# cryscan/bevy-hikari

Hardware: AMD Instinct MI355X
Metric: Mray/s (Cornell 1080p 2-bounce, whole job) + frame ms (higher is better)
Workload: dtype f32

## Files before the change

### bevy-hikari_amd/_ffi.py

```python
import ctypes as C
import os

HERE = os.path.dirname(os.path.abspath(__file__))
LIB_PATH = os.environ.get("HIKARI_HIP_LIB", os.path.join(HERE, "libhikari_hip.so"))

HK_OK = 0
HK_E_INVALID, HK_E_NO_DEVICE, HK_E_HIP, HK_E_NOT_READY, HK_E_NOMEM, HK_E_UNSUPPORTED = -1, -2, -3, -4, -5, -6

BUF_POSITION, BUF_NORMAL, BUF_DEPTH_GRADIENT, BUF_INSTANCE_MATERIAL, BUF_VELOCITY_UV, BUF_ALBEDO = range(6)
BUF_VARIANCE0, BUF_RENDER0, BUF_RESERVOIR0 = 6, 9, 12
BUF_DENOISE_INTERNAL0, BUF_DENOISE_INTERNAL_VARIANCE, BUF_DENOISE_RENDER0, BUF_TONE_MAPPED = 22, 26, 27, 30
(BUF_PREVIOUS_POSITION, BUF_PREVIOUS_VELOCITY_UV, BUF_PREVIOUS_TONE_MAPPED, BUF_UPSCALE_OUTPUT, BUF_TAA_OUTPUT, BUF_PREVIOUS_TAA_OUTPUT,
 BUF_UPSCALE_SHARPENED) = range(31, 38)
BUF_PARKED_TO0, BUF_PARKED_RECORD0, BUF_COUNT = 38, 41, 44
HISTORY_AUTO = 0xFFFF
(PASS_PREPASS, PASS_FULL_SCREEN_ALBEDO, PASS_DIRECT_LIT, PASS_DIRECT_EMISSIVE, PASS_INDIRECT, PASS_EMISSIVE_SPATIAL_REUSE,
 PASS_INDIRECT_SPATIAL_REUSE, PASS_DEMODULATION, PASS_DENOISE_L0, PASS_DENOISE_L1, PASS_DENOISE_L2, PASS_DENOISE_L3,
 PASS_TONE_MAPPING, PASS_SMAA_TU4X, PASS_SMAA_TU4X_EXTRAPOLATE, PASS_TAA_JASMINE, PASS_FSR_EASU, PASS_FSR_RCAS, PASS_COUNT) = range(19)
PASS_NAMES = ["prepass", "full_screen_albedo", "direct_lit", "direct_emissive", "indirect_lit_ambient", "emissive_spatial_reuse",
              "indirect_spatial_reuse", "demodulation", "denoise_l0", "denoise_l1", "denoise_l2", "denoise_l3", "tone_mapping",
              "smaa_tu4x", "smaa_tu4x_extrapolate", "taa_jasmine", "fsr_easu", "fsr_rcas"]
STAGE_TEMPORAL, STAGE_SPATIAL, STAGE_POST_PROCESS, STAGE_ANTIALIAS, STAGE_UPSCALE, STAGE_COUNT = range(6)
DEFAULT_CTX_FLAGS = int(os.environ.get("HIKARI_HIP_DEFAULT_CTX_FLAGS", "0"))
CTX_COUNT_RAYS, CTX_TIME_PASSES, CTX_PLAIN_DIVISION, CTX_SINGLE_STREAM, CTX_DETERMINISTIC_SCATTER, CTX_EXACT_TRAVERSAL = 1, 2, 4, 8, 16, 32
TREE_SAH, TREE_LBVH = 0, 1
CTX_WAVEFRONT, CTX_FUSED_INDIRECT = 64, 128
CTX_NO_WIDE_WALK = 256
CTX_COUNT_WALKS = 512
CTX_RACING_SCATTER = 1024
DEBUG_OPT_SPATIAL_WINDOW, DEBUG_OPT_FRAME_PIPELINE, DEBUG_OPT_WF_TIMELINE, DEBUG_OPT_FLAT_WALK, DEBUG_OPT_FLAT_ORDERINGS, DEBUG_OPT_TRACE_UPDATE = 0, 1, 2, 3, 4, 5
DEBUG_OPT_MAIN_PRIORITY, DEBUG_OPT_PREPASS_PIPELINE, DEBUG_OPT_MESH_REBUILD_ONE_WORKGROUP = 9, 10, 11
DEBUG_OPT_LOAD_DEVICE_LIMIT = 12
TIMING_TRACE_STAGES = 18
TRAVERSAL_WIDE = 0x100
FRAME_EXTERNAL_GBUFFER, FRAME_ANTIALIAS, FRAME_BALANCE_BANDS, FRAME_GATHER, FRAME_TIME_BAND = 1, 2, 4, 8, 16
TOPOLOGY_TRIANGLE_LIST, TOPOLOGY_TRIANGLE_STRIP = 0, 1
TAA_JASMINE, TAA_NONE = 0, 1
UPSCALE_FSR1, UPSCALE_SMAA_TU4X = 0, 1
NO_TEXTURE = 0xFFFFFFFF
ADDRESS_CLAMP_TO_EDGE, ADDRESS_REPEAT, ADDRESS_MIRROR_REPEAT = 0, 1, 2
TIMING_SLOTS = 24
FORMAT_RGBA16F, FORMAT_RGBA32F, FORMAT_RGBA8_UNORM_SRGB, FORMAT_BGRA8_UNORM_SRGB = range(4)
PRESENT_HDR, PRESENT_CLEAR = 1, 2
RAYS_CLOSEST, RAYS_ANY, RAYS_ATTRIBUTES, RAYS_STACKLESS = 0, 1, 2, 4
RAY_MISS, RAY_HIT, RAY_INVALID = 0, 1, 2
NO_INSTANCE = 0xFFFFFFFF

f32, u32, u64 = C.c_float, C.c_uint32, C.c_uint64


class HkVertex(C.Structure):
    _fields_ = [("position", f32 * 3), ("u", f32), ("normal", f32 * 3), ("v", f32)]


class HkPrimitiveVertex(C.Structure):
    _fields_ = [("position", f32 * 3), ("index", u32)]


class HkPrimitive(C.Structure):
    _fields_ = [("vertices", HkPrimitiveVertex * 3)]


class HkNode(C.Structure):
    _fields_ = [("min", f32 * 3), ("entry_index", u32), ("max", f32 * 3), ("exit_index", u32)]


class HkMeshIndex(C.Structure):
    _fields_ = [("vertex", u32), ("primitive", u32), ("node_offset", u32), ("node_count", u32)]


class HkInstance(C.Structure):
    _fields_ = [("min", f32 * 3), ("material", u32), ("max", f32 * 3), ("node_index", u32), ("model", f32 * 16),
                ("inverse_transpose_model", f32 * 16), ("mesh", HkMeshIndex)]


class HkMaterial(C.Structure):
    _fields_ = [("base_color", f32 * 4), ("base_color_texture", u32), ("_pad0", u32 * 3), ("emissive", f32 * 4),
                ("emissive_texture", u32), ("perceptual_roughness", f32), ("metallic", f32), ("metallic_roughness_texture", u32),
                ("reflectance", f32), ("normal_map_texture", u32), ("occlusion_texture", u32), ("_pad1", u32)]


class HkAliasEntry(C.Structure):
    _fields_ = [("prob", f32), ("index", u32)]


class HkEmissive(C.Structure):
    _fields_ = [("emissive", f32 * 4), ("position", f32 * 3), ("radius", f32), ("instance", u32), ("_pad0", u32),
                ("alias_table", u32 * 2), ("surface_area", f32), ("node_index", u32), ("_pad1", u32 * 2)]


class HkFrame(C.Structure):
    _fields_ = [("kernel", (f32 * 4) * 3), ("halton", (f32 * 4) * 8), ("clear_color", f32 * 4), ("number", u32),
                ("direct_validate_interval", u32), ("emissive_validate_interval", u32), ("indirect_bounces", u32),
                ("temporal_reuse", u32), ("emissive_spatial_reuse", u32), ("indirect_spatial_reuse", u32),
                ("max_temporal_reuse_count", u32), ("max_spatial_reuse_count", u32), ("max_reservoir_lifetime", f32),
                ("solar_angle", f32), ("max_indirect_luminance", f32), ("upscale_ratio", f32), ("_pad", u32 * 3)]


class HkView(C.Structure):
    _fields_ = [("view_proj", f32 * 16), ("inverse_view_proj", f32 * 16), ("view", f32 * 16), ("inverse_view", f32 * 16),
                ("projection", f32 * 16), ("inverse_projection", f32 * 16), ("world_position", f32 * 3), ("_pad0", f32),
                ("viewport", f32 * 4)]


class HkPreviousView(C.Structure):
    _fields_ = [("view_proj", f32 * 16), ("inverse_view_proj", f32 * 16)]


class HkLights(C.Structure):
    _fields_ = [("directional_color", f32 * 4), ("direction_to_light", f32 * 3), ("n_directional_lights", u32),
                ("ambient_color", f32 * 4)]


class HkSettings(C.Structure):
    _fields_ = [("direct_validate_interval", u32), ("emissive_validate_interval", u32), ("max_temporal_reuse_count", u32),
# ... 19 lines not shown
class HkRayHit(C.Structure):
    _fields_ = [("distance", f32), ("instance", u32), ("primitive", u32), ("material", u32), ("barycentric", f32 * 2), ("uv", f32 * 2),
                ("normal", f32 * 3), ("status", u32)]


class HkHaloOp(C.Structure):
    _fields_ = [("buffer", u32), ("peer", u32), ("row_begin", u32), ("row_end", u32), ("row_bytes", u64)]


class HkTransfer(C.Structure):
    _fields_ = [("buffer", u32), ("peer", u32), ("is_recv", u32), ("_pad", u32), ("offset", C.c_uint64), ("bytes", C.c_uint64)]


class HkMovedBox(C.Structure):
    _fields_ = [("min", f32 * 3), ("_pad0", f32), ("max", f32 * 3), ("_pad1", f32), ("previous_from_current", f32 * 16)]


class HkStats(C.Structure):
    _fields_ = [("rays_primary", u64), ("rays_tlas", u64), ("rays_blas", u64), ("frames", u64),
                ("pass_ms_total", C.c_double * TIMING_SLOTS), ("pass_launches", u64 * TIMING_SLOTS), ("last_frame_ms", f32),
                ("_pad", u32), ("scene_mesh_builds", u64), ("scene_instance_builds", u64),
                ("scene_async_instance_uploads", u64), ("scene_device_refits", u64), ("scene_device_tree_builds", u64),
                ("walk_node_steps", u64), ("walk_triangle_tests", u64), ("walk_instance_entries", u64), ("walk_closest_hits", u64), ("walk_top_node_steps", u64),
                ("wide_stack_lost", u64)]


assert C.sizeof(HkVertex) == 32 and C.sizeof(HkPrimitive) == 48 and C.sizeof(HkNode) == 32 and C.sizeof(HkInstance) == 176
assert C.sizeof(HkMaterial) == 80 and C.sizeof(HkEmissive) == 64 and C.sizeof(HkFrame) == 256 and C.sizeof(HkView) == 416
assert C.sizeof(HkPreviousView) == 128 and C.sizeof(HkAliasEntry) == 8
assert C.sizeof(HkRay) == 32 and C.sizeof(HkRayHit) == 48


class HikariError(RuntimeError):
    def __init__(self, code, fn, message):
        super().__init__(f"{fn} failed with code {code}: {message}")
        self.code = code


P = C.POINTER
_vp = C.c_void_p

_SIGNATURES = {
    "create": [C.c_int, u32, P(_vp)],
    "upload_meshes": [_vp, P(HkVertex), u32, P(HkPrimitive), u32, P(HkNode), u32],
    "upload_materials": [_vp, P(HkMaterial), u32],
    "upload_instances": [_vp, P(HkInstance), u32, P(HkNode), u32, P(HkEmissive), u32, P(HkNode), u32, P(HkAliasEntry), u32],
    "upload_previous_transforms": [_vp, P(f32), u32],
    "upload_noise": [_vp, _vp, C.c_size_t],
    "upload_textures": [_vp, P(HkImageDesc), u32],
    "resize": [_vp, u32, u32, f32],
    "set_view_options": [_vp, u32, u32, f32],
    "frame_begin": [_vp, P(HkFrame), P(HkView), P(HkPreviousView), P(HkLights)],
    "pass_run": [_vp, u32, u32, u32, u32],
    "frame_stage": [_vp, u32, P(HkSettings), u32],
    "frame_render": [_vp, P(HkFrame), P(HkView), P(HkPreviousView), P(HkLights), P(HkSettings), u32],
    "frame_wait": [_vp],
    "set_band": [_vp, u32, u32],
    "set_history_rows": [_vp, u32],
    "history_rows": [_vp, P(u32)],
    "scene_bounds": [_vp, P(f32), P(f32)],
    "set_band_bounds": [_vp, P(u32), u32],
    "row_costs": [_vp, P(u32), u32],
    "buffer_info": [_vp, u32, P(u32), P(u32), P(u32)],
    "read_buffer": [_vp, u32, _vp, C.c_size_t],
    "write_buffer": [_vp, u32, _vp, C.c_size_t],
    "device_ptr": [_vp, u32, P(_vp), P(C.c_size_t)],
    "get_stats": [_vp, P(HkStats)],
    "reset_stats": [_vp],
}
_DEBUG = {
    "debug_math": [_vp, u32, P(f32), P(f32), P(f32), C.c_size_t],
    "debug_read_trees": [_vp, P(HkNode), u32, P(HkNode), u32],
    "debug_read_mesh_nodes": [_vp, P(HkNode), u32, P(u32), P(u32)],
    "debug_last_load": [_vp, P(u32)],
    "debug_last_load_times": [_vp, P(C.c_double)],
    "debug_read_emitters": [_vp, P(f32), u32, P(u32), P(f32), u32, P(u32)],
    "debug_read_mesh_geometry": [_vp, P(HkMeshIndex), P(f32), P(f32), u32, P(f32), u32, P(f32), P(u32), P(u32)],
    "debug_comm_loopback": [_vp, u32, u32, u32, u32, u32],
    "debug_read_wf_timeline": [_vp, P(C.c_uint64), u32],
    "debug_set_option": [_vp, u32, C.c_int64],
    "debug_comm_lanes": [_vp, P(u32)],
    "debug_multi_serial": [C.c_int],
    "debug_spatial_windowed_launches": [_vp, P(C.c_uint64)],
    "debug_main_stream_priority": [_vp, P(u32)],
    "measure_hbm": [_vp, C.c_size_t, u32, P(C.c_double), P(C.c_double)],
    "measure_valu": [_vp, u32, P(C.c_double)],
    "measure_gather": [_vp, C.c_size_t, u32, u32, u32, u32, P(C.c_double), P(C.c_double)],
}
_PRODUCT_ONLY = {
    "device_count": [P(C.c_int)],
    "settings_default": [P(HkSettings)],
    "frame_from_settings": [P(HkSettings), u32, P(HkFrame)],
    "scaled_size": [u32, u32, f32, P(u32), P(u32)],
    "scene_builder_create": [P(_vp)],
    "scene_builder_add_mesh": [_vp, P(f32), P(f32), P(f32), u32, P(u32), u32, u32, P(u32)],
    "scene_builder_add_mesh_deferred": [_vp, P(f32), P(f32), P(f32), u32, P(u32), u32, u32, P(u32)],
    "scene_builder_pending_mesh_trees": [_vp, P(u32)],
    "scene_builder_build_pending_mesh_trees": [_vp],
    "scene_builder_add_material": [_vp, P(HkMaterial), P(u32)],
    "scene_builder_add_instance": [_vp, u32, u32, P(f32), P(u32)],
    "scene_builder_finish": [_vp],
    "scene_builder_finish_instances": [_vp],
    "scene_builder_remove_instance": [_vp, u32],
    "scene_builder_set_instance_material": [_vp, u32, u32],
    "scene_builder_set_instance_transform": [_vp, u32, P(f32)],
    "scene_builder_previous_transforms": [_vp, P(P(f32)), P(u32)],
    "scene_builder_vertices": [_vp, P(P(HkVertex)), P(u32)],
    "scene_builder_primitives": [_vp, P(P(HkPrimitive)), P(u32)],
    "scene_builder_asset_nodes": [_vp, P(P(HkNode)), P(u32)],
    "scene_builder_materials": [_vp, P(P(HkMaterial)), P(u32)],
    "scene_builder_instances": [_vp, P(P(HkInstance)), P(u32)],
    "scene_builder_instance_nodes": [_vp, P(P(HkNode)), P(u32)],
    "scene_builder_emissives": [_vp, P(P(HkEmissive)), P(u32)],
    "scene_builder_emissive_nodes": [_vp, P(P(HkNode)), P(u32)],
    "scene_builder_alias_table": [_vp, P(P(HkAliasEntry)), P(u32)],
    "scene_builder_set_mesh_vertices": [_vp, u32, P(f32), P(f32)],
    "scene_builder_rebuild_mesh_tree": [_vp, u32],
    "scene_builder_mesh_index": [_vp, u32, P(HkMeshIndex)],
    "upload_scene": [_vp, _vp],
    "upload_scene_instances": [_vp, _vp],
    "load_scene": [_vp, _vp, u32],
    "refit_scene_instances": [_vp, _vp, P(u32)],
    "rebuild_scene_trees": [_vp, u32],
    "update_scene_instances": [_vp, _vp, u32],
    "update_mesh_vertices": [_vp, P(HkMeshIndex), u32, P(f32), P(f32)],
    "set_mesh_skin": [_vp, P(HkMeshIndex), u32, P(f32), P(f32), P(C.c_uint16), P(f32)],
    "skin_mesh": [_vp, P(HkMeshIndex), P(f32), u32],
    "rebuild_mesh_tree": [_vp, P(HkMeshIndex), u32],
    "present": [_vp, P(HkSettings), u32, P(HkPresentTarget), u32, u32],
    "cast_rays": [_vp, P(HkRay), u32, u32, P(HkRayHit)],
    "cast_rays_device": [_vp, _vp, u32, u32, _vp],
    "band_rows": [u32, u32, u32, P(u32), P(u32)],
    "balanced_band_bounds": [P(u32), u32, u32, u32, u32, u32, f32, P(u32)],
    "balance_bands": [_vp, u32, P(u32), u32],
    "rebalanced_band_bounds": [P(u32), P(f32), u32, u32, P(f32), u32, u32, f32, P(u32)],
    "band_migration_plan": [u32, u32, f32, P(u32), P(u32), u32, u32, u32, P(HkSettings), P(HkHaloOp), P(u32)],
    "band_migration_schedule": [u32, u32, f32, P(u32), P(u32), u32, u32, u32, P(HkSettings), P(HkTransfer), P(u32)],
    "migrate_bands": [_vp, P(u32), u32, u32, P(HkSettings)],
    "band_time_ms": [_vp, P(f32)],
    "multi_migrate_bands": [_vp, P(u32), u32, u32, P(HkSettings)],
    "band_gather_schedule": [u32, u32, f32, u32, P(u32), u32, u32, u32, u32, P(HkTransfer), P(u32)],
    "comm_gather": [_vp, u32, u32],
    "multi_gather": [_vp, u32, u32],
    "get_band_bounds": [_vp, P(u32), u32],
    "get_band": [_vp, P(u32), P(u32)],
    "band_plan_bounds": [u32, u32, f32, P(u32), u32, u32, u32, u32, P(HkSettings), P(HkHaloOp), P(u32)],
    "band_schedule_bounds": [u32, u32, f32, P(u32), u32, u32, u32, u32, P(HkSettings), P(HkTransfer), P(u32)],
    "band_plan": [_vp, u32, P(HkSettings), P(HkHaloOp), P(u32)],
    "band_plan_for": [u32, u32, f32, u32, u32, u32, u32, P(HkSettings), P(HkHaloOp), P(u32)],
    "stream": [_vp, P(_vp)],
    "set_stream": [_vp, _vp],
    "set_timing_mask": [_vp, u32],
    "indirect_schedule": [_vp, P(u32)],
    "traversal_mode": [_vp, P(u32), P(u32)],
    "bvh_rethread": [P(HkNode), u32, u32, P(HkNode)],
    "band_schedule": [u32, u32, f32, u32, u32, u32, u32, P(HkSettings), P(HkTransfer), P(u32)],
    "comm_unique_id": [P(C.c_uint8)],
    "comm_available": [_vp],
    "comm_init": [_vp, u32, u32, P(C.c_uint8)],
    "comm_destroy": [_vp],
    "comm_set_history_rows": [_vp, u32],
    "history_rows_bound": [P(HkView), P(HkPreviousView), u32, P(f32), P(f32), P(HkMovedBox), u32, P(u32)],
    "comm_exchange": [_vp, u32, P(HkSettings)],
    "multi_create": [u32, P(C.c_int), u32, P(_vp)],
    "multi_context": [_vp, u32, P(_vp)],
    "multi_upload_scene": [_vp, _vp],
# ... 82 lines not shown
```

### bevy-hikari_amd/csrc/context.hip

```cpp
#include "hk_context.hpp"

using namespace hk;
using namespace hkd;

namespace hk {

void buffer_dims(const hk_ctx* c, uint32_t b, int* w, int* h) {
  if (buffer_is_full_size(b)) { *w = c->W; *h = c->H; return; }
  if (buffer_is_upscaled(b) && c->upscale_kind == HK_UPSCALE_SMAA_TU4X) { *w = c->UW; *h = c->UH; return; }
  if (b == HK_BUF_UPSCALE_OUTPUT) { *w = c->W; *h = c->H; return; }
  *w = c->RW;
  *h = c->RH;
}
size_t buffer_logical_bytes(const hk_ctx* c, uint32_t b) {
  int w, h;
  buffer_dims(c, b, &w, &h);
  return (size_t)w * h * buffer_bpp(b);
}

bool certify_uv_division(int size) {
  const float b = (float)size, c = 1.0f / b;
  for (int k = -64; k < size + 64; ++k) {
    const float x = (float)k + 0.5f, want = x / b, q = x * c, got = fmaf(fmaf(-q, b, x), c, q);
    if (memcmp(&want, &got, 4) != 0) return false;
  }
  return true;
}

#ifndef HK_PRE_BANDS
#define HK_PRE_BANDS 1
#endif
#ifndef HK_PRE_STREAM_HIGH
#define HK_PRE_STREAM_HIGH 0
#endif
#ifndef HK_MAIN_HIGH_PRIORITY_PIXELS
#define HK_MAIN_HIGH_PRIORITY_PIXELS ((size_t)6 << 20)
#endif
int pick_main_stream(hk_ctx* c, bool forced) {
  if (!c->own_stream || c->post_forked) return HK_OK;
  if (!forced && c->main_priority_decided) return HK_OK;
  const size_t px = (size_t)c->RW * (size_t)c->RH / (size_t)(c->band_count > 0 ? c->band_count : 1);
  if (px == 0) return HK_OK;
  c->main_priority_decided = true;
  const bool high = c->main_priority < 0 ? px <= HK_MAIN_HIGH_PRIORITY_PIXELS : c->main_priority != 0;
  if (high == c->own_stream_high) return HK_OK;
  const bool in_use = c->stream == c->own_stream;
  { const int rc = sync_all(c); if (rc) return rc; }
  HK_HIP(hipStreamSynchronize(c->own_stream));
  int least = 0, greatest = 0;
  hipStream_t fresh = nullptr;
  if (hipDeviceGetStreamPriorityRange(&least, &greatest) != hipSuccess || least == greatest ||
      hipStreamCreateWithPriority(&fresh, hipStreamNonBlocking, high ? greatest : least) != hipSuccess || !fresh) {
    (void)hipGetLastError();
    return HK_OK;
  }
  (void)hipStreamDestroy(c->own_stream);
  c->own_stream = fresh;
  c->own_stream_high = high;
  if (in_use) c->stream = fresh;
  if (high && c->side_stream && c->post_stream && !c->pre_stream) {
    if (hipStreamCreateWithPriority(&c->pre_stream, hipStreamNonBlocking, (HK_PRE_STREAM_HIGH || c->band_count > 1) ? greatest : least) != hipSuccess || hipEventCreateWithFlags(&c->pre_done, hipEventDisableTiming) != hipSuccess ||
        hipEventCreateWithFlags(&c->pre_scene_mark, hipEventDisableTiming) != hipSuccess) {
      (void)hipGetLastError();
      if (c->pre_stream) (void)hipStreamDestroy(c->pre_stream);
      c->pre_stream = nullptr;
    }
  }
  return HK_OK;
}
#ifndef HK_PREPASS_PIPELINE_RULE
#ifndef HK_PREPASS_PIPELINE_LDS_BANDS
#define HK_PREPASS_PIPELINE_LDS_BANDS 0
#endif
#define HK_PREPASS_PIPELINE_RULE                                                                                                     \
  ((size_t)c->scene.blob_f4 * 16 > HK_LDS_SCENE_BYTES ? (size_t)c->RW * (size_t)c->RH / (size_t)(c->band_count > 0 ? c->band_count : 1) <= ((size_t)3 << 20) \
                                                        : (HK_PREPASS_PIPELINE_LDS_BANDS && c->band_count > 1 && (size_t)c->RW * (size_t)c->RH / (size_t)c->band_count <= ((size_t)3 << 18)))
#endif
int free_screen(hk_ctx* c) {
  for (int k = 0; k < 3; ++k) {
    if (c->det_winner[k]) (void)hipFree(c->det_winner[k]);
    c->det_winner[k] = nullptr;
    c->det_lite_clean[k] = false;
  }
  for (uint32_t b = 0; b < HK_BUF_COUNT; ++b) {
    if (c->buf[b]) (void)hipFree(c->buf[b]);
    c->buf[b] = nullptr;
    c->buf_bytes[b] = 0;
  }
  for (int k = 0; k < 10; ++k) {
    if (c->tile_meta[k]) (void)hipFree(c->tile_meta[k]);
    c->tile_meta[k] = nullptr;
    c->tile_meta_zero[k] = false;
  }
  if (c->wf_mem) (void)hipFree(c->wf_mem);
  c->wf_mem = nullptr;
  if (c->wf.timeline) (void)hipFree(c->wf.timeline);
  c->wf = hkd::WfBuffers{};
  if (c->depth_plane) (void)hipFree(c->depth_plane);
  if (c->prev_depth_plane) (void)hipFree(c->prev_depth_plane);
  c->prev_depth_plane = nullptr;
  if (c->dn_g) (void)hipFree(c->dn_g);
  c->depth_plane = nullptr;
  c->dn_g = nullptr;
  for (void** q : {&c->albedo_twin, &c->depth_gradient_twin, &c->dn_g_twin, &c->normal_twin, &c->instance_material_twin, &c->render_twin[0], &c->render_twin[1], &c->render_twin[2], &c->variance_twin[0],
                   &c->variance_twin[1], &c->variance_twin[2]}) {
    if (*q) (void)hipFree(*q);
    *q = nullptr;
  }
  c->post_pending[0] = c->post_pending[1] = false;
  for (int k = 0; k < 2; ++k) {
    for (int l = 0; l < 4; ++l) {
      if (c->dn_extra[k][l]) (void)hipFree(c->dn_extra[k][l]);
      c->dn_extra[k][l] = nullptr;
    }
    if (c->dn_extra_var[k]) (void)hipFree(c->dn_extra_var[k]);
    c->dn_extra_var[k] = nullptr;
  }
  return HK_OK;
}

hipEvent_t get_event(hk_ctx* c) {
  if (!c->event_pool.empty()) {
    hipEvent_t e = c->event_pool.back();
    c->event_pool.pop_back();
    return e;
  }
  hipEvent_t e = nullptr;
  (void)hipEventCreate(&e);
  return e;
}

void drain_timers(hk_ctx* c) {
  for (TimedLaunch& t : c->pending) {
    float ms = 0.0f;
    if (hipEventElapsedTime(&ms, t.start, t.stop) == hipSuccess) {
      c->slot_ms[t.slot] += (double)ms;
      c->slot_launches[t.slot] += 1;
    }
    c->event_pool.push_back(t.start);
    c->event_pool.push_back(t.stop);
  }
  c->pending.clear();
  if (c->frame_timed) {
    float ms = 0.0f;
    if (hipEventElapsedTime(&ms, c->frame_start, c->frame_stop) == hipSuccess) c->last_frame_ms = ms;
    c->frame_timed = false;
  }
}

struct ScopedTimer {
  hk_ctx* c;
  bool on;
  TimedLaunch t{};
  bool attached;
  ScopedTimer(hk_ctx* ctx, uint32_t slot, bool attach = false) : c(ctx), on((ctx->timing_mask >> slot) & 1u), attached(attach) {
    if (on) {
      t.slot = slot;
      t.start = get_event(c);
      t.stop = get_event(c);
      if (!attached) (void)hipEventRecord(t.start, c->stream);
    }
  }
  ~ScopedTimer() {
    if (on) {
      if (!attached) (void)hipEventRecord(t.stop, c->stream);
      c->pending.push_back(t);
    }
  }
};

DFrame make_dframe(const hk_ctx* c) {
  DFrame f;
  memset(&f, 0, sizeof(f));
  const HkFrame& h = c->frame;
  for (int col = 0; col < 3; ++col)
    for (int row = 0; row < 3; ++row) f.kernel[col * 3 + row] = h.kernel[col][row];
  f.number = h.number;
  f.direct_validate_interval = h.direct_validate_interval;
  f.emissive_validate_interval = h.emissive_validate_interval;
  f.indirect_bounces = h.indirect_bounces;
  f.temporal_reuse = h.temporal_reuse;
  f.max_temporal_reuse_count = h.max_temporal_reuse_count;
  f.max_spatial_reuse_count = h.max_spatial_reuse_count;
  f.max_reservoir_lifetime = h.max_reservoir_lifetime;
  f.solar_angle = h.solar_angle;
  f.max_indirect_luminance = h.max_indirect_luminance;
  f.upscale_ratio = h.upscale_ratio;
  f.random_float_number = (float)hash_u32(h.number) / 4294967295.0f;
  f.number_golden = (float)h.number * 1.618033989f;
  f.cam_x = c->view.world_position[0]; f.cam_y = c->view.world_position[1]; f.cam_z = c->view.world_position[2];
  f.ortho_x = c->view.view_proj[2]; f.ortho_y = c->view.view_proj[6]; f.ortho_z = c->view.view_proj[10];
  f.is_ortho = c->view.projection[15] == 1.0f ? 1u : 0u;
  f.sun_r = c->lights.directional_color[0]; f.sun_g = c->lights.directional_color[1]; f.sun_b = c->lights.directional_color[2];
  f.sun_dx = c->lights.direction_to_light[0]; f.sun_dy = c->lights.direction_to_light[1]; f.sun_dz = c->lights.direction_to_light[2];
  f.amb_r = c->lights.ambient_color[0]; f.amb_g = c->lights.ambient_color[1]; f.amb_b = c->lights.ambient_color[2];
  f.clear_r = h.clear_color[0]; f.clear_g = h.clear_color[1]; f.clear_b = h.clear_color[2]; f.clear_a = h.clear_color[3];
  f.dw = c->W; f.dh = c->H; f.rw = c->RW; f.rh = c->RH;
  f.inv_dw = 1.0f / (float)c->W; f.inv_dh = 1.0f / (float)c->H; f.inv_rw = 1.0f / (float)c->RW; f.inv_rh = 1.0f / (float)c->RH;
  f.rcp_rw = 1.0 / (double)c->RW; f.rcp_rh = 1.0 / (double)c->RH;
  f.uv_fast = c->uv_fast ? 1u : 0u;
  return f;
}
GBuffer make_gbuffer(const hk_ctx* c) {
  GBuffer g;
  g.position = (float4*)c->buf[HK_BUF_POSITION];
  g.normal = (uint32_t*)c->buf[HK_BUF_NORMAL];
  g.depth_gradient = (float2*)c->buf[HK_BUF_DEPTH_GRADIENT];
  g.instance_material = (float2*)c->buf[HK_BUF_INSTANCE_MATERIAL];
  g.velocity_uv = (float4*)c->buf[HK_BUF_VELOCITY_UV];
  g.depth = c->depth_plane;
  g.dn_g = (float4*)c->dn_g;
  g.albedo_out = nullptr;
  return g;
}
bool parks_across_bands(const hk_ctx* c) { return c->band_count > 1 && c->history_now > 0; }
bool scatter_lite(const hk_ctx* c, int channel) {
  if (c->band_count > 1 || (c->flags & HK_CTX_RACING_SCATTER)) return false;
  if (c->flags & HK_CTX_DETERMINISTIC_SCATTER) return true;
  return channel == 2 ? c->frame.indirect_spatial_reuse != 0u : c->frame.emissive_spatial_reuse != 0u;
}
int ensure_parked(hk_ctx* c, uint32_t channels) {
  const size_t nr = (size_t)c->RW * c->RH;
  for (int k = 0; k < 3; ++k) {
    if (!((channels >> k) & 1u) || c->det_winner[k]) continue;
    int* winner = nullptr;
    void* plane[2] = {nullptr, nullptr};
    size_t plane_bytes[2] = {0, 0};
    hipError_t e = hipMalloc((void**)&winner, nr * sizeof(int));
    for (int j = 0; j < 2 && e == hipSuccess; ++j) {
      const uint32_t b = (j == 0 ? (uint32_t)HK_BUF_PARKED_TO0 : (uint32_t)HK_BUF_PARKED_RECORD0) + (uint32_t)k;
      plane_bytes[j] = nr * buffer_bpp(b);
      e = hipMalloc(&plane[j], plane_bytes[j]);
      if (e == hipSuccess) e = hipMemset(plane[j], j == 0 ? 0xFF : 0, plane_bytes[j]);
    }
    if (e == hipSuccess) e = hipDeviceSynchronize();
    if (e != hipSuccess) {
      if (winner) (void)hipFree(winner);
      for (void* q : plane)
        if (q) (void)hipFree(q);
      set_error("allocating the parked-store planes failed: %s", hipGetErrorString(e));
      return HK_E_HIP;
    }
    c->det_winner[k] = winner;
    for (int j = 0; j < 2; ++j) {
      const uint32_t b = (j == 0 ? (uint32_t)HK_BUF_PARKED_TO0 : (uint32_t)HK_BUF_PARKED_RECORD0) + (uint32_t)k;
      c->buf[b] = plane[j];
      c->buf_bytes[b] = plane_bytes[j];
    }
  }
  return HK_OK;
}
void scene_bounds(const hk_ctx* c, float mn[3], float mx[3]) {
  for (int k = 0; k < 3; ++k) { mn[k] = INFINITY; mx[k] = -INFINITY; }
  for (const HkInstance& in : c->instances)
    for (int k = 0; k < 3; ++k) {
      mn[k] = std::min(mn[k], in.min[k]);
      mx[k] = std::max(mx[k], in.max[k]);
    }
}
int derive_history_rows(const hk_ctx* c, uint32_t* rows) {
  *rows = 0;
  if (c->instances.empty()) return HK_OK;
  std::vector<HkMovedBox> moved;
  const size_t ni = c->instances.size();
  if (c->prev_models.size() == 16 * ni)
    for (size_t i = 0; i < ni; ++i) {
      const HkInstance& in = c->instances[i];
      const float* pm = &c->prev_models[16 * i];
      if (memcmp(pm, in.model, 64) == 0) continue;
      HkMovedBox b{};
      memcpy(b.min, in.min, 12);
      memcpy(b.max, in.max, 12);
      for (int col = 0; col < 4; ++col)
        for (int row = 0; row < 4; ++row) {
          double s = 0.0;
          for (int k = 0; k < 4; ++k) s += (double)pm[4 * k + row] * (double)in.inverse_transpose_model[4 * k + col];
          b.previous_from_current[4 * col + row] = (float)s;
        }
      moved.push_back(b);
    }
  if (moved.empty() && memcmp(c->view.view_proj, c->pview.view_proj, 64) == 0) return HK_OK;
  float mn[3], mx[3];
  scene_bounds(c, mn, mx);
  return hk_history_rows_bound(&c->view, &c->pview, (uint32_t)c->RH, mn, mx, moved.empty() ? nullptr : moved.data(), (uint32_t)moved.size(), rows);
}
LightTargets make_light_targets(const hk_ctx* c, int channel) {
  static const int T[3] = {0, 2, 6}, S[3] = {4, 4, 8};
  const uint32_t cur = c->frame.number % 2u, prev = 1u - cur;
  LightTargets t;
  t.previous = (const PackedReservoir*)c->buf[HK_BUF_RESERVOIR0 + cur + T[channel]];
  t.current = (PackedReservoir*)c->buf[HK_BUF_RESERVOIR0 + prev + T[channel]];
  t.previous_spatial = (PackedReservoir*)c->buf[HK_BUF_RESERVOIR0 + cur + S[channel]];
  t.spatial = (PackedReservoir*)c->buf[HK_BUF_RESERVOIR0 + prev + S[channel]];
  t.variance = (float*)c->buf[HK_BUF_VARIANCE0 + channel];
  t.render = (uint2*)c->buf[HK_BUF_RENDER0 + channel];
  const bool parked = c->det_winner[channel] && (scatter_lite(c, channel) || parks_across_bands(c));
  t.det_lite = parked && !parks_across_bands(c) ? 1 : 0;
// ... 2 lines not shown
  t.det_pending = parked ? (PackedReservoir*)c->buf[HK_BUF_PARKED_RECORD0 + channel] : nullptr;
  t.m_current = t.m_spatial = t.m_previous_spatial = nullptr;
  t.serial = 0;
  t.tiles_x = c->tiles_x;
  t.rw = c->RW;
  return t;
}
int attach_tile_meta(hk_ctx* c, LightTargets& t, int channel, bool spatial_pass, int y0, int y1) {
  if (!c->tile_meta[0]) return HK_OK;
  static const int T[3] = {0, 2, 6}, S[3] = {4, 4, 8};
  const int cur = (int)(c->frame.number % 2u), prev = 1 - cur;
  const int k_current = prev + T[channel], k_spatial = prev + S[channel], k_previous_spatial = cur + S[channel];
  const bool maintain = c->band_count == 1 && (y0 % 8) == 0 && ((y1 % 8) == 0 || y1 == c->RH);
  const size_t mb = (size_t)c->tiles_x * c->tiles_y * sizeof(TileMeta);
  const int written[3] = {spatial_pass ? -1 : k_current, k_spatial, spatial_pass ? -1 : k_previous_spatial};
  for (int k : written) {
    if (k < 0) continue;
    if (maintain) {
      c->tile_meta_zero[k] = false;
    } else if (!c->tile_meta_zero[k]) {
      HK_HIP(hipMemsetAsync(c->tile_meta[k], 0, mb, c->stream));
      c->tile_meta_zero[k] = true;
    }
  }
  if (!maintain) return HK_OK;
  t.m_current = c->tile_meta[k_current];
  t.m_spatial = c->tile_meta[k_spatial];
  t.m_previous_spatial = c->tile_meta[k_previous_spatial];
  t.serial = ++c->elide_serial;
  return HK_OK;
}

int ready(hk_ctx* c) {
  HK_REQUIRE(c, HK_E_INVALID, "ctx is NULL");
  HK_REQUIRE(c->W > 0, HK_E_NOT_READY, "hk_resize has not been called");
  HK_REQUIRE(c->have_frame, HK_E_NOT_READY, "hk_frame_begin has not been called");
  HK_REQUIRE(c->have_noise, HK_E_NOT_READY, "noise textures not uploaded");
  HK_HIP(hipSetDevice(c->device));
  const int rc = finalize_scene(c);
  return rc ? rc : flush_deform(c);
}

struct Jitter { float x, y; };
Jitter prepass_jitter(const hk_ctx* c) {
  Jitter j{0.0f, 0.0f};
  if (c->taa == HK_TAA_NONE) return j;
  const uint32_t n = c->frame.number;
  const uint32_t index = (c->upscale_kind == HK_UPSCALE_SMAA_TU4X) ? ((n >> 1u) & 15u) : (n & 15u);
  const float* h = c->frame.halton[index >> 1u];
  const float hx = (index & 1u) == 0u ? h[0] : h[2], hy = (index & 1u) == 0u ? h[1] : h[3];
  j.x = 2.0f * hx * (1.0f / c->view.viewport[2]);
  j.y = -(2.0f * hy * (1.0f / c->view.viewport[3]));
  return j;
}

void full_rows_for(const hk_ctx* c, int ry0, int ry1, int* fy0, int* fy1) {
  if (c->RH == c->H) {
    *fy0 = ry0;
    *fy1 = ry1;
    return;
  }
  *fy0 = std::max(0, (int)floorf((float)ry0 * (float)c->H / (float)c->RH) - 1);
  *fy1 = std::min(c->H, (int)ceilf((float)ry1 * (float)c->H / (float)c->RH) + 1);
}

void* dn_internal(hk_ctx* c, uint32_t nch, uint32_t ch, int level) {
  return ch + 1 == nch ? c->buf[HK_BUF_DENOISE_INTERNAL0 + level] : c->dn_extra[ch][level];
}
float* dn_variance(hk_ctx* c, uint32_t nch, uint32_t ch) {
  return ch + 1 == nch ? (float*)c->buf[HK_BUF_DENOISE_INTERNAL_VARIANCE] : c->dn_extra_var[ch];
}
int run_demodulation_fused(hk_ctx* c, uint32_t nch, int y0, int y1) {
  if (y1 <= y0) return HK_OK;
  const DFrame fr = make_dframe(c);
  ScopedTimer timer(c, HK_PASS_DEMODULATION);
  DemodTargets d{};
  d.albedo = (const uint2*)c->buf[HK_BUF_ALBEDO];
  for (uint32_t ch = 0; ch < nch; ++ch) {
    d.variance[ch] = (const float*)c->buf[HK_BUF_VARIANCE0 + ch];
    d.render[ch] = (const uint2*)c->buf[HK_BUF_RENDER0 + ch];
    d.output[ch] = (uint2*)dn_internal(c, nch, ch, 0);
    d.internal_variance[ch] = dn_variance(c, nch, ch);
  }
  launch_demodulation(c->stream, (int)nch, fr, d, y0, y1);
  HK_HIP(hipGetLastError());
  return HK_OK;
}
int run_denoise_fused(hk_ctx* c, uint32_t nch, int level, int y0, int y1, bool with_tone_mapping = false) {
  if (y1 <= y0) return HK_OK;
  const DFrame fr = make_dframe(c);
  ScopedTimer timer(c, HK_PASS_DENOISE_L0 + (uint32_t)level);
  DenoiseTargets d{};
  d.albedo = (const uint2*)c->buf[HK_BUF_ALBEDO];
  d.dn_g = (const float4*)c->dn_g;
  d.depth = c->depth_plane;
  d.depth_gradient = (const float2*)c->buf[HK_BUF_DEPTH_GRADIENT];
  for (uint32_t ch = 0; ch < nch; ++ch) {
    d.input[ch] = (const uint2*)dn_internal(c, nch, ch, level);
    d.output[ch] = level == 3 ? (uint2*)c->buf[HK_BUF_DENOISE_RENDER0 + ch] : (uint2*)dn_internal(c, nch, ch, level + 1);
    d.internal_variance[ch] = dn_variance(c, nch, ch);
  }
  if (with_tone_mapping && level == 3 && nch == (c->frame.indirect_bounces != 0u ? 3u : 2u)) {
    d.tone_mapped = (uint2*)c->buf[HK_BUF_TONE_MAPPED];
    memcpy(d.clear_color, c->frame.clear_color, sizeof(d.clear_color));
  }
  launch_denoise(c->stream, level, (int)nch, 0, fr, d, y0, y1);
  HK_HIP(hipGetLastError());
  return HK_OK;
}

bool use_wavefront(const hk_ctx* c) {
  if (c->frame.indirect_bounces < 2u || c->frame.indirect_bounces > 60u || (c->flags & HK_CTX_COUNT_RAYS)) return false;
  if (c->flags & HK_CTX_FUSED_INDIRECT) return false;
  if (c->flags & HK_CTX_WAVEFRONT) return true;
  return (size_t)c->scene.blob_f4 * 16 > HK_LDS_SCENE_BYTES;
}
static bool wide_allowed(const hk_ctx* c) {
  return !(c->flags & HK_CTX_NO_WIDE_WALK) && c->threaded && !c->scene.flat_mode && (size_t)c->scene.blob_f4 * 16 > HK_LDS_SCENE_BYTES;
}
bool use_wide(const hk_ctx* c) { return wide_allowed(c); }
int ensure_wide(hk_ctx* c, bool with_spill) {
  const size_t tlas_slots = c->instance_nodes.size(), blas_slots = c->asset_nodes.size();
  if (tlas_slots == 0 || blas_slots == 0) return HK_OK;
  if (tlas_slots > c->wide_tlas_slots) {
    if (c->wide_tlas) { HK_HIP(hipStreamSynchronize(c->stream)); (void)hipFree(c->wide_tlas); c->wide_tlas = nullptr; }
    HK_HIP(hipMalloc((void**)&c->wide_tlas, (tlas_slots + tlas_slots / 2 + 16) * 128));
    c->wide_tlas_slots = tlas_slots + tlas_slots / 2 + 16;
    c->wide_tlas_dirty = true;
  }
  if (blas_slots > c->wide_blas_slots) {
    if (c->wide_blas) { HK_HIP(hipStreamSynchronize(c->stream)); (void)hipFree(c->wide_blas); c->wide_blas = nullptr; }
    HK_HIP(hipMalloc((void**)&c->wide_blas, blas_slots * 128));
    c->wide_blas_slots = blas_slots;
    c->wide_blas_dirty = true;
  }
  const size_t n_inst = c->instances.size(), n_prim = c->primitives.size();
  if (n_inst > c->wide_rank_instances) {
    if (c->wide_tlas_rank) { HK_HIP(hipStreamSynchronize(c->stream)); (void)hipFree(c->wide_tlas_rank); c->wide_tlas_rank = nullptr; }
    HK_HIP(hipMalloc((void**)&c->wide_tlas_rank, (n_inst + n_inst / 2 + 16) * sizeof(uint32_t)));
    HK_HIP(hipMemsetAsync(c->wide_tlas_rank, 0xFF, (n_inst + n_inst / 2 + 16) * sizeof(uint32_t), c->stream));
    c->wide_rank_instances = n_inst + n_inst / 2 + 16;
    c->wide_tlas_dirty = true;
  }
  if (n_prim > c->wide_rank_primitives) {
    if (c->wide_blas_rank) { HK_HIP(hipStreamSynchronize(c->stream)); (void)hipFree(c->wide_blas_rank); c->wide_blas_rank = nullptr; }
    HK_HIP(hipMalloc((void**)&c->wide_blas_rank, std::max<size_t>(n_prim, 1) * sizeof(uint32_t)));
    HK_HIP(hipMemsetAsync(c->wide_blas_rank, 0xFF, std::max<size_t>(n_prim, 1) * sizeof(uint32_t), c->stream));
    c->wide_rank_primitives = n_prim;
    c->wide_blas_dirty = true;
  }
  if (!c->compute_units) {
    hipDeviceProp_t prop;
    HK_HIP(hipGetDeviceProperties(&prop, c->device));
    c->compute_units = prop.multiProcessorCount;
  }
  const size_t lanes = with_spill ? wide_trace_lanes(c->compute_units) : 0;
  if (lanes > c->wide_spill_lanes) {
    if (c->wide_spill) { HK_HIP(hipStreamSynchronize(c->stream)); (void)hipFree(c->wide_spill); c->wide_spill = nullptr; }
    HK_HIP(hipMalloc((void**)&c->wide_spill, lanes * wide_spill_entries() * sizeof(uint32_t)));
    c->wide_spill_lanes = lanes;
  }
  if (c->wide_blas_dirty || c->wide_mesh_check) {
    if (c->wide_blas_dirty) c->wide_meshes.clear();
    std::vector<std::pair<uint32_t, uint32_t>> meshes;
    std::vector<std::pair<std::pair<uint32_t, uint32_t>, uint32_t>> first_primitive;
    for (const HkInstance& in : c->instances) {
      meshes.emplace_back(in.mesh.node_offset, in.mesh.node_count);
      first_primitive.emplace_back(std::make_pair(in.mesh.node_offset, in.mesh.node_count), in.mesh.primitive);
    }
    std::sort(meshes.begin(), meshes.end());
    meshes.erase(std::unique(meshes.begin(), meshes.end()), meshes.end());
    std::sort(first_primitive.begin(), first_primitive.end());
    first_primitive.erase(std::unique(first_primitive.begin(), first_primitive.end()), first_primitive.end());
    for (size_t k = 0; k + 1 < first_primitive.size(); ++k)
      HK_REQUIRE(first_primitive[k].first != first_primitive[k + 1].first, HK_E_INVALID, "two instances share the mesh nodes [%u, +%u) but not the mesh primitives (%u / %u)",
                 first_primitive[k].first.first, first_primitive[k].first.second, first_primitive[k].second, first_primitive[k + 1].second);
    for (const auto& m : meshes) {
      if (std::binary_search(c->wide_meshes.begin(), c->wide_meshes.end(), m)) continue;
      HK_REQUIRE((size_t)m.first + m.second <= blas_slots, HK_E_INVALID, "an instance's mesh nodes lie outside the uploaded mesh nodes");
      const uint32_t prim0 = std::lower_bound(first_primitive.begin(), first_primitive.end(), std::make_pair(m, 0u))->second;
      HK_REQUIRE((size_t)prim0 + (m.second + 2u) / 3u <= n_prim, HK_E_INVALID, "an instance's mesh primitives lie outside the uploaded primitives");
      launch_build_wide(c->stream, c->scene.nodes + 2u * ((size_t)c->scene.blas_base + m.first), m.second, c->wide_blas + 8u * (size_t)m.first, c->wide_blas_rank + prim0);
    }
    HK_HIP(hipGetLastError());
    std::vector<std::pair<uint32_t, uint32_t>> all;
    std::set_union(c->wide_meshes.begin(), c->wide_meshes.end(), meshes.begin(), meshes.end(), std::back_inserter(all));
    c->wide_meshes.swap(all);
    c->wide_blas_dirty = c->wide_mesh_check = false;
// ... 51 lines not shown
  if ((tl_twin || count_twin) && !w.timeline) HK_HIP(hipMalloc((void**)&w.timeline, 64 * 32 * sizeof(unsigned long long)));
  w.timeline_mode = count_twin ? 2u : (tl_twin ? 1u : 0u);
  return HK_OK;
}

int join_side(hk_ctx* c) {
  if (!c->forked) return HK_OK;
  HK_HIP(hipEventRecord(c->join_event, c->side_stream));
  HK_HIP(hipStreamWaitEvent(c->stream, c->join_event, 0));
  c->forked = false;
  c->side_state[0] = c->side_state[1] = 0;
  return HK_OK;
}
int join_post(hk_ctx* c) {
  for (int k = 0; k < 2; ++k)
    if (c->post_pending[k]) {
      HK_HIP(hipStreamWaitEvent(c->stream, c->post_done[k], 0));
      c->post_pending[k] = false;
    }
  return HK_OK;
}
int join_post_parity(hk_ctx* c, uint32_t parity) {
  if (!c->post_pending[parity & 1u]) return HK_OK;
  HK_HIP(hipStreamWaitEvent(c->stream, c->post_done[parity & 1u], 0));
  c->post_pending[parity & 1u] = false;
  return HK_OK;
}
int join_all(hk_ctx* c) {
  int rc = join_side(c);
  if (!rc) rc = join_post(c);
  if (!rc && c->comm) rc = comm_join(c, -1);
  return rc;
}
#define HK_FRAME_INTERNAL_LATE_JOIN 0x80000000u
int post_begin(hk_ctx* c, const HkSettings* st, bool* pipelined) {
  *pipelined = false;
  int rc;
  if (st->denoise && c->derived_dirty) {
    launch_derive_planes(c->stream, make_gbuffer(c), c->depth_plane, c->dn_g, c->W, 0, c->H);
    c->derived_dirty = false;
  }
  const uint32_t post_bits = (1u << HK_PASS_DEMODULATION) | (1u << HK_PASS_DENOISE_L0) | (1u << HK_PASS_DENOISE_L1) | (1u << HK_PASS_DENOISE_L2) | (1u << HK_PASS_DENOISE_L3);
  if (!(st->denoise && c->post_stream && c->frame_pipeline && !(c->timing_mask & post_bits) && c->albedo_twin && c->render_twin[0])) {
    if ((rc = join_side(c))) return rc;
    return join_post(c);
  }
  if (c->forked) {
    HK_HIP(hipEventRecord(c->side_done, c->side_stream));
    HK_HIP(hipStreamWaitEvent(c->post_stream, c->side_done, 0));
    for (int k = 0; k < 2; ++k)
      if (c->side_state[k] == 1) {
        c->side_state[k] = 2;
        c->side_cover[k] = (uint8_t)(c->mapped_parity & 1u);
      }
  }
  HK_HIP(hipEventRecord(c->post_fork, c->stream));
  HK_HIP(hipStreamWaitEvent(c->post_stream, c->post_fork, 0));
  c->post_saved_main = c->stream;
  c->stream = c->post_stream;
  *pipelined = true;
  return HK_OK;
}
int post_end(hk_ctx* c, bool pipelined) {
  c->post_forked = false;
  if (!pipelined) return HK_OK;
  const uint32_t parity = c->mapped_parity & 1u;
  const hipError_t e = hipEventRecord(c->post_done[parity], c->post_stream);
  c->stream = c->post_saved_main;
  HK_REQUIRE(e == hipSuccess, HK_E_HIP, "hipEventRecord failed: %s", hipGetErrorString(e));
  c->post_pending[parity] = true;
  return HK_OK;
}
int run_pass(hk_ctx* c, uint32_t pass, uint32_t arg, int y0, int y1);
int run_pass_on_side(hk_ctx* c, uint32_t pass, uint32_t arg, int y0, int y1) {
  hipStream_t main_stream = c->stream;
  c->stream = c->side_stream;
  const int rc = (y1 > y0) ? run_pass(c, pass, arg, y0, y1) : HK_OK;
  c->stream = main_stream;
  return rc;
}

int run_pass(hk_ctx* c, uint32_t pass, uint32_t arg, int y0, int y1) {
  const DFrame fr = make_dframe(c);
  const GBuffer g = make_gbuffer(c);
  unsigned long long* counters = (c->flags & HK_CTX_COUNT_RAYS) ? c->d_counters : nullptr;
  if (c->derived_dirty && pass != HK_PASS_PREPASS) {
    launch_derive_planes(c->stream, g, c->depth_plane, c->dn_g, c->W, 0, c->H);
    c->derived_dirty = false;
  }
  ScopedTimer timer(c, pass, pass == HK_PASS_INDIRECT || pass == HK_PASS_INDIRECT_SPATIAL_REUSE || pass == HK_PASS_EMISSIVE_SPATIAL_REUSE);
  switch (pass) {
    case HK_PASS_PREPASS: {
      Jitter j = prepass_jitter(c);
      hkd::WideTrees wide{};
      { const int rc_ = wide_for_fused(c, &wide); if (rc_) return rc_; }
      launch_prepass(c->stream, c->scene, fr, c->view.inverse_view_proj, c->view.view_proj, c->pview.view_proj, c->d_prev_models, j.x, j.y, g, y0, y1, counters, &wide);
      break;
    }
    case HK_PASS_FULL_SCREEN_ALBEDO: launch_albedo(c->stream, c->scene, fr, g, c->buf[HK_BUF_ALBEDO], y0, y1); break;
    case HK_PASS_DIRECT_LIT:
    case HK_PASS_DIRECT_EMISSIVE:
    case HK_PASS_INDIRECT: {
      const int channel = pass == HK_PASS_DIRECT_LIT ? 0 : (pass == HK_PASS_DIRECT_EMISSIVE ? 1 : 2);
      const bool across = parks_across_bands(c);
      if (across || scatter_lite(c, channel)) { const int rc_ = ensure_parked(c, across ? 7u : 1u << channel); if (rc_) return rc_; }
      LightTargets t = make_light_targets(c, channel);
      { const int rc_ = attach_tile_meta(c, t, channel, false, y0, y1); if (rc_) return rc_; }
      const size_t px = (size_t)c->RW * c->RH;
      if (t.det_winner && t.det_lite) {
        if (!c->det_lite_clean[channel]) {
          HK_HIP(hipMemsetAsync(t.det_winner, 0xFF, px * sizeof(int), c->stream));
          HK_HIP(hipMemsetAsync(t.det_to, 0xFF, px * sizeof(int), c->stream));
          c->det_lite_clean[channel] = true;
        }
      } else {
        c->det_lite_clean[channel] = false;
        if (t.det_winner) {
          HK_HIP(hipMemsetAsync(t.det_winner, 0xFF, px * sizeof(int), c->stream));
          if (across) HK_HIP(hipMemsetAsync(t.det_to + (size_t)y0 * c->RW, 0xFF, (size_t)(y1 - y0) * c->RW * sizeof(int), c->stream));
          else HK_HIP(hipMemsetAsync(t.det_to, 0xFF, px * sizeof(int), c->stream));
        }
      }
      if (pass == HK_PASS_INDIRECT && use_wavefront(c)) {
        { const int rc_ = ensure_wavefront(c); if (rc_) return rc_; }
        hkd::WideTrees wide{};
        if (use_wide(c)) {
          { const int rc_ = ensure_wide(c, true); if (rc_) return rc_; }
          wide.tlas = c->wide_tlas;
          wide.blas = c->wide_blas;
          wide.tlas_rank = c->wide_tlas_rank;
          wide.blas_rank = c->wide_blas_rank;
          wide.tlas_count = c->scene.tlas_count;
          wide.spill = c->wide_spill;
          wide.lost = c->d_counters + 8;
        }
        std::vector<hipEvent_t> trace_events;
        if ((c->timing_mask >> HK_TIMING_TRACE_STAGES) & 1u)
          for (uint32_t k = 0; k < 2u * (c->frame.indirect_bounces + 1u); ++k) trace_events.push_back(get_event(c));
        launch_indirect_wavefront(c->stream, c->scene, fr, g, t, c->wf, y0, y1, c->compute_units, timer.on ? timer.t.start : nullptr,
                                  timer.on ? timer.t.stop : nullptr, &wide, trace_events.empty() ? nullptr : trace_events.data());
        for (size_t k = 0; k + 1 < trace_events.size(); k += 2) c->pending.push_back(TimedLaunch{HK_TIMING_TRACE_STAGES, trace_events[k], trace_events[k + 1]});
      } else if (pass == HK_PASS_INDIRECT)
        launch_indirect(c->stream, c->frame.indirect_bounces >= 2u, c->scene, fr, g, t, y0, y1, counters, timer.on ? timer.t.start : nullptr,
                        timer.on ? timer.t.stop : nullptr);
      else
        launch_direct(c->stream, pass == HK_PASS_DIRECT_EMISSIVE, c->scene, fr, g, t, y0, y1, counters);
      if (t.det_winner && t.det_lite) launch_resolve_scatter_lite(c->stream, t, fr, c->depth_plane, pass == HK_PASS_INDIRECT, y0, y1);
      else if (t.det_winner && !across) launch_resolve_scatter(c->stream, t, 0, (int)px, 0, 0);
      break;
    }
    case HK_PASS_EMISSIVE_SPATIAL_REUSE:
    case HK_PASS_INDIRECT_SPATIAL_REUSE: {
      const int channel = pass == HK_PASS_EMISSIVE_SPATIAL_REUSE ? 1 : 2;
      LightTargets t = make_light_targets(c, channel);
      { const int rc_ = attach_tile_meta(c, t, channel, true, y0, y1); if (rc_) return rc_; }
      if (launch_spatial(c->stream, channel == 1, c->scene, fr, g, t, y0, y1, c->spatial_window, timer.on ? timer.t.start : nullptr, timer.on ? timer.t.stop : nullptr))
        c->spatial_windowed_launches += 1;
      break;
    }
    case HK_PASS_DEMODULATION: {
      HK_REQUIRE(arg < 3, HK_E_INVALID, "channel out of range");
      DemodTargets d{};
      d.albedo = (const uint2*)c->buf[HK_BUF_ALBEDO];
      d.variance[0] = (const float*)c->buf[HK_BUF_VARIANCE0 + arg];
      d.render[0] = (const uint2*)c->buf[HK_BUF_RENDER0 + arg];
      d.output[0] = (uint2*)c->buf[HK_BUF_DENOISE_INTERNAL0];
      d.internal_variance[0] = (float*)c->buf[HK_BUF_DENOISE_INTERNAL_VARIANCE];
      launch_demodulation(c->stream, 1, fr, d, y0, y1);
      break;
    }
    case HK_PASS_DENOISE_L0: case HK_PASS_DENOISE_L1: case HK_PASS_DENOISE_L2: case HK_PASS_DENOISE_L3: {
      HK_REQUIRE(arg < 3, HK_E_INVALID, "channel out of range");
// ... 134 lines not shown
    if (!(flags & (HK_CTX_DETERMINISTIC_SCATTER | HK_CTX_COUNT_RAYS | HK_CTX_TIME_PASSES))) {
      if (hipStreamCreateWithFlags(&c->post_stream, hipStreamNonBlocking) != hipSuccess || hipEventCreateWithFlags(&c->post_fork, hipEventDisableTiming) != hipSuccess ||
          hipEventCreateWithFlags(&c->post_done[0], hipEventDisableTiming) != hipSuccess || hipEventCreateWithFlags(&c->post_done[1], hipEventDisableTiming) != hipSuccess) {
        set_error("cannot create the post-process stream");
        hk_destroy(c);
        return HK_E_HIP;
      }
    }
  }
  *out = c;
  return HK_OK;
}

void hk_destroy(hk_ctx* c) {
  if (!c) return;
  (void)hipSetDevice(c->device);
  (void)join_all(c);
  if (c->stream) (void)hipStreamSynchronize(c->stream);
  comm_release(c);
  drain_timers(c);
  for (hipEvent_t e : c->event_pool) (void)hipEventDestroy(e);
  for (hipEvent_t e : c->band_ev)
    if (e) (void)hipEventDestroy(e);
  if (c->frame_start) (void)hipEventDestroy(c->frame_start);
  if (c->frame_stop) (void)hipEventDestroy(c->frame_stop);
  free_screen(c);
  if (c->scene_mem) (void)hipFree(c->scene_mem);
  for (int k = 0; k < 2; ++k) {
    if (c->staging[k]) (void)hipHostFree(c->staging[k]);
    if (c->staging_done[k]) (void)hipEventDestroy(c->staging_done[k]);
  }
  if (c->query_staging) (void)hipHostFree(c->query_staging);
  if (c->query_device) (void)hipFree(c->query_device);
  free_refit(c);
  free_deform(c);
  for (void* q : {(void*)c->wide_tlas, (void*)c->wide_blas, (void*)c->wide_spill, (void*)c->wide_tlas_rank, (void*)c->wide_blas_rank})
    if (q) (void)hipFree(q);
  c->d_tex_data.release();
  c->d_noise.release();
  if (c->d_counters) (void)hipFree(c->d_counters);
  if (c->side_stream) (void)hipStreamDestroy(c->side_stream);
  if (c->post_stream) (void)hipStreamDestroy(c->post_stream);
  if (c->post_fork) (void)hipEventDestroy(c->post_fork);
  for (int k = 0; k < 2; ++k)
    if (c->post_done[k]) (void)hipEventDestroy(c->post_done[k]);
  if (c->fork_event) (void)hipEventDestroy(c->fork_event);
  if (c->join_event) (void)hipEventDestroy(c->join_event);
  if (c->side_done) (void)hipEventDestroy(c->side_done);
  if (c->pre_stream) { (void)hipStreamSynchronize(c->pre_stream); (void)hipStreamDestroy(c->pre_stream); }
  if (c->pre_done) (void)hipEventDestroy(c->pre_done);
  if (c->pre_scene_mark) (void)hipEventDestroy(c->pre_scene_mark);
  if (c->own_stream) (void)hipStreamDestroy(c->own_stream);
  delete c;
}
int hk_debug_read_wf_timeline(hk_ctx* c, unsigned long long* out, uint32_t n) {
  HK_REQUIRE(c && out && n == 64u * 32u, HK_E_INVALID, "bad argument");
  HK_REQUIRE(c->wf.timeline, HK_E_NOT_READY, "no timeline: set HK_WF_TIMELINE=1 (or create the context with HK_CTX_COUNT_WALKS) before the first frame of a scene beyond the LDS copy");
  HK_HIP(hipSetDevice(c->device));
  { const int rc = sync_all(c); if (rc) return rc; }
  HK_HIP(hipMemcpy(out, c->wf.timeline, n * sizeof(unsigned long long), hipMemcpyDeviceToHost));
  int khz = 0;
  HK_HIP(hipDeviceGetAttribute(&khz, hipDeviceAttributeWallClockRate, c->device));
  out[n - 1] = (unsigned long long)khz;
  return HK_OK;
}

int hk_debug_set_option(hk_ctx* c, uint32_t option, int64_t value) {
  HK_REQUIRE(c, HK_E_INVALID, "ctx is NULL");
  HK_HIP(hipSetDevice(c->device));
  { const int rc = sync_all(c); if (rc) return rc; }
  switch (option) {
    case HK_DEBUG_OPT_SPATIAL_WINDOW: c->spatial_window = value < 0 ? -1 : (value ? 1 : 0); break;
    case HK_DEBUG_OPT_FRAME_PIPELINE: c->frame_pipeline = value != 0; break;
    case HK_DEBUG_OPT_WF_TIMELINE:
      c->wf_timeline = value != 0;
      if (c->wf_mem) { (void)hipFree(c->wf_mem); c->wf_mem = nullptr; }
      break;
    case HK_DEBUG_OPT_FLAT_WALK: c->flat_walk = value != 0; c->dynamic_dirty = true; break;
    case HK_DEBUG_OPT_FLAT_ORDERINGS: c->flat_orderings = (int)std::max<int64_t>(0, std::min<int64_t>(8, value)); c->dynamic_dirty = true; break;
    case HK_DEBUG_OPT_TRACE_UPDATE: c->trace_update = value != 0; break;
    case HK_DEBUG_OPT_MESH_REBUILD_ONE_WORKGROUP: c->mesh_rebuild_one_workgroup = value != 0; break;
    case HK_DEBUG_OPT_LOAD_DEVICE_LIMIT: c->load_device_limit = value <= 0 ? HK_MESH_REBUILD_MAX_TRIANGLES : (uint32_t)std::min<int64_t>(value, HK_MESH_REBUILD_MAX_TRIANGLES); break;
    case HK_DEBUG_OPT_PREPASS_PIPELINE: c->prepass_pipeline = value < 0 ? -1 : (value ? 1 : 0); break;
    case HK_DEBUG_OPT_MAIN_PRIORITY: c->main_priority = value < 0 ? -1 : (value ? 1 : 0); return pick_main_stream(c, true);
    default: HK_REQUIRE(false, HK_E_INVALID, "unknown option %u", option);
  }
  return HK_OK;
}

int hk_debug_main_stream_priority(hk_ctx* c, uint32_t* out) {
  HK_REQUIRE(c && out, HK_E_INVALID, "bad argument");
  *out = (c->own_stream_high ? 1u : 0u) | (c->main_priority_decided ? 2u : 0u) | (c->pre_stream ? 4u : 0u) | ((uint32_t)std::min<uint64_t>(c->prepasses_pipelined, 0xFFFFFu) << 8);
  return HK_OK;
}

int hk_debug_spatial_windowed_launches(hk_ctx* c, uint64_t* out) {
  HK_REQUIRE(c && out, HK_E_INVALID, "bad argument");
  *out = c->spatial_windowed_launches;
  return HK_OK;
}

static int resize_resources(hk_ctx* c, uint32_t width, uint32_t height, float upscale_ratio);

int hk_resize(hk_ctx* c, uint32_t width, uint32_t height, float upscale_ratio) {
  HK_REQUIRE(c && width && height && width <= 16384u && height <= 16384u, HK_E_INVALID, "bad size %u x %u (1..16384)", width, height);
  const int rc = resize_resources(c, width, height, upscale_ratio);
  if (rc) {
    free_screen(c);
    c->W = c->H = c->RW = c->RH = c->UW = c->UH = 0;
  }
  return rc;
}

static int resize_resources(hk_ctx* c, uint32_t width, uint32_t height, float upscale_ratio) {
  HK_HIP(hipSetDevice(c->device));
  { const int rc_ = sync_all(c); if (rc_) return rc_; }
  free_screen(c);
  if (!c->band_bounds.empty()) {
    c->band_bounds.clear();
    c->bounds_generation += 1;
  }
  uint32_t rw, rh;
  int rc = hk_scaled_size(width, height, upscale_ratio, &rw, &rh);
  if (rc) return rc;
  c->W = (int)width; c->H = (int)height; c->RW = (int)rw; c->RH = (int)rh;
  c->ratio = upscale_ratio < 1.0f ? 1.0f : (upscale_ratio > 2.0f ? 2.0f : upscale_ratio);
  {
    const float scale2 = (1.0f / c->ratio) * 2.0f;
    c->UW = (int)ceilf((float)width * scale2);
    c->UH = (int)ceilf((float)height * scale2);
    c->mapped_parity = 0;
    c->pre_chain_ok = false;
  }
  for (uint32_t b = 0; b < HK_BUF_PARKED_TO0; ++b) {
    size_t n = buffer_is_full_size(b) ? (size_t)c->W * c->H : (buffer_is_upscaled(b) ? (size_t)c->UW * c->UH : (size_t)c->RW * c->RH);
    size_t bytes = n * buffer_bpp(b);
    HK_HIP(hipMalloc(&c->buf[b], bytes));
    HK_HIP(hipMemset(c->buf[b], 0, bytes));
    c->buf_bytes[b] = bytes;
  }
  const size_t nf = (size_t)c->W * c->H, nr = (size_t)c->RW * c->RH;
  {
    c->tiles_x = (c->RW + 7) / 8;
    c->tiles_y = (c->RH + 7) / 8;
    const size_t mb = (size_t)c->tiles_x * c->tiles_y * sizeof(TileMeta);
    for (int k = 0; k < 10; ++k) {
      HK_HIP(hipMalloc((void**)&c->tile_meta[k], mb));
      HK_HIP(hipMemset(c->tile_meta[k], 0, mb));
      c->tile_meta_zero[k] = true;
    }
  }
  HK_HIP(hipMalloc((void**)&c->depth_plane, nf * 4));
  HK_HIP(hipMemset(c->depth_plane, 0, nf * 4));
  HK_HIP(hipMalloc((void**)&c->prev_depth_plane, nf * 4));
  HK_HIP(hipMemset(c->prev_depth_plane, 0, nf * 4));
  HK_HIP(hipMalloc(&c->dn_g, nf * 16));
  HK_HIP(hipMemset(c->dn_g, 0, nf * 16));
  if (c->post_stream) {
    HK_HIP(hipMalloc(&c->albedo_twin, c->buf_bytes[HK_BUF_ALBEDO]));
    HK_HIP(hipMemset(c->albedo_twin, 0, c->buf_bytes[HK_BUF_ALBEDO]));
    HK_HIP(hipMalloc(&c->depth_gradient_twin, c->buf_bytes[HK_BUF_DEPTH_GRADIENT]));
    HK_HIP(hipMemset(c->depth_gradient_twin, 0, c->buf_bytes[HK_BUF_DEPTH_GRADIENT]));
    HK_HIP(hipMalloc(&c->dn_g_twin, nf * 16));
    HK_HIP(hipMemset(c->dn_g_twin, 0, nf * 16));
    HK_HIP(hipMalloc(&c->normal_twin, c->buf_bytes[HK_BUF_NORMAL]));
    HK_HIP(hipMemset(c->normal_twin, 0, c->buf_bytes[HK_BUF_NORMAL]));
    HK_HIP(hipMalloc(&c->instance_material_twin, c->buf_bytes[HK_BUF_INSTANCE_MATERIAL]));
    HK_HIP(hipMemset(c->instance_material_twin, 0, c->buf_bytes[HK_BUF_INSTANCE_MATERIAL]));
    for (int ch = 0; ch < 3; ++ch) {
      HK_HIP(hipMalloc(&c->render_twin[ch], c->buf_bytes[HK_BUF_RENDER0 + ch]));
      HK_HIP(hipMemset(c->render_twin[ch], 0, c->buf_bytes[HK_BUF_RENDER0 + ch]));
      HK_HIP(hipMalloc(&c->variance_twin[ch], c->buf_bytes[HK_BUF_VARIANCE0 + ch]));
      HK_HIP(hipMemset(c->variance_twin[ch], 0, c->buf_bytes[HK_BUF_VARIANCE0 + ch]));
    }
  }
  for (int k = 0; k < 2; ++k) {
    for (int l = 0; l < 4; ++l) {
      HK_HIP(hipMalloc(&c->dn_extra[k][l], nr * 8));
      HK_HIP(hipMemset(c->dn_extra[k][l], 0, nr * 8));
    }
    HK_HIP(hipMalloc((void**)&c->dn_extra_var[k], nr * 4));
    HK_HIP(hipMemset(c->dn_extra_var[k], 0, nr * 4));
  }
  c->derived_dirty = false;
  c->uv_fast = !(c->flags & HK_CTX_PLAIN_DIVISION) && certify_uv_division(c->W) && certify_uv_division(c->H) && certify_uv_division(c->RW) && certify_uv_division(c->RH);
  HK_HIP(hipDeviceSynchronize());
  return HK_OK;
}

int hk_set_view_options(hk_ctx* c, uint32_t taa, uint32_t upscale_kind, float upscale_sharpness) {
  HK_REQUIRE(c && taa <= HK_TAA_NONE && upscale_kind <= HK_UPSCALE_SMAA_TU4X, HK_E_INVALID, "bad argument");
  c->upscale_sharpness = upscale_sharpness;
  c->taa = taa;
  c->upscale_kind = upscale_kind;
  return HK_OK;
}

int hk_frame_begin(hk_ctx* c, const HkFrame* f, const HkView* v, const HkPreviousView* pv, const HkLights* l) {
  HK_REQUIRE(c && f && v && pv && l, HK_E_INVALID, "NULL argument");
  HK_REQUIRE(f->direct_validate_interval > 0 && f->emissive_validate_interval > 0, HK_E_INVALID, "validate intervals must be > 0");
  if (!c->main_priority_decided) { const int rc = pick_main_stream(c, false); if (rc) return rc; }
  c->frame = *f;
  c->view = *v;
  c->pview = *pv;
  c->lights = *l;
  c->have_frame = true;
  if ((f->number & 1u) != c->mapped_parity) {
    std::swap(c->buf[HK_BUF_POSITION], c->buf[HK_BUF_PREVIOUS_POSITION]);
    std::swap(c->depth_plane, c->prev_depth_plane);
    std::swap(c->buf[HK_BUF_VELOCITY_UV], c->buf[HK_BUF_PREVIOUS_VELOCITY_UV]);
    std::swap(c->buf[HK_BUF_TONE_MAPPED], c->buf[HK_BUF_PREVIOUS_TONE_MAPPED]);
    std::swap(c->buf[HK_BUF_TAA_OUTPUT], c->buf[HK_BUF_PREVIOUS_TAA_OUTPUT]);
    if (c->albedo_twin) {
      std::swap(c->buf[HK_BUF_ALBEDO], c->albedo_twin);
      std::swap(c->buf[HK_BUF_DEPTH_GRADIENT], c->depth_gradient_twin);
      std::swap(c->dn_g, c->dn_g_twin);
      std::swap(c->buf[HK_BUF_NORMAL], c->normal_twin);
      std::swap(c->buf[HK_BUF_INSTANCE_MATERIAL], c->instance_material_twin);
      for (int ch = 0; ch < 3; ++ch) {
        std::swap(c->buf[HK_BUF_RENDER0 + ch], c->render_twin[ch]);
        std::swap(c->buf[HK_BUF_VARIANCE0 + ch], c->variance_twin[ch]);
      }
    }
    c->mapped_parity = f->number & 1u;
  }
  if (c->comm) { const int rc = comm_join(c, (int)(f->number & 1u)); if (rc) return rc; }
  c->history_now = 0;
  if (c->band_count > 1 && c->RH > 0) {
    if (c->history_rows != HK_HISTORY_AUTO) {
      c->history_now = std::min(c->history_rows, (uint32_t)c->RH);
    } else {
      const int rc = derive_history_rows(c, &c->history_now);
      if (rc) return rc;
    }
    if (parks_across_bands(c)) { const int rc = ensure_parked(c, 7u); if (rc) return rc; }
  }
  return HK_OK;
}

int hk_set_history_rows(hk_ctx* c, uint32_t rows) {
  HK_REQUIRE(c && rows <= HK_HISTORY_AUTO, HK_E_INVALID, "bad argument");
  c->history_rows = rows;
  return HK_OK;
}
int hk_history_rows(hk_ctx* c, uint32_t* rows) {
  HK_REQUIRE(c && rows, HK_E_INVALID, "bad argument");
  *rows = c->history_now;
  return HK_OK;
}
int hk_scene_bounds(hk_ctx* c, float mn[3], float mx[3]) {
  HK_REQUIRE(c && mn && mx, HK_E_INVALID, "bad argument");
  HK_REQUIRE(c->have_instances, HK_E_NOT_READY, "no scene uploaded");
  scene_bounds(c, mn, mx);
  return HK_OK;
}

int hk_pass_run(hk_ctx* c, uint32_t pass, uint32_t arg, uint32_t row_begin, uint32_t row_end) {
  int rc = ready(c);
  if (rc) return rc;
  if ((rc = join_all(c))) return rc;
  const bool full_grid = pass == HK_PASS_PREPASS || pass == HK_PASS_FULL_SCREEN_ALBEDO;
  int rows = full_grid ? c->H : c->RH;
  if (pass == HK_PASS_TAA_JASMINE) { int w; buffer_dims(c, HK_BUF_TAA_OUTPUT, &w, &rows); }
  if (pass == HK_PASS_FSR_EASU || pass == HK_PASS_FSR_RCAS) rows = c->H;
  const int y0 = (int)row_begin, y1 = row_end == 0 ? rows : (int)row_end;
  HK_REQUIRE(y0 >= 0 && y1 <= rows && y0 <= y1, HK_E_INVALID, "row range [%d,%d) outside 0..%d", y0, y1, rows);
  return run_pass(c, pass, arg, y0, y1);
}

int hk_set_band(hk_ctx* c, uint32_t band_index, uint32_t band_count) {
  HK_REQUIRE(c && band_count > 0 && band_index < band_count, HK_E_INVALID, "bad band");
  if (band_count != c->band_count && !c->band_bounds.empty()) {
    c->band_bounds.clear();
    c->bounds_generation += 1;
  }
  c->band_index = band_index;
  c->band_count = band_count;
  return HK_OK;
}

int hk_set_band_bounds(hk_ctx* c, const uint32_t* bounds, uint32_t n_bounds) {
  HK_REQUIRE(c, HK_E_INVALID, "ctx is NULL");
  if (!bounds || n_bounds == 0) {
    if (!c->band_bounds.empty()) c->bounds_generation += 1;
    c->band_bounds.clear();
    return HK_OK;
  }
  HK_REQUIRE(c->RH > 0, HK_E_NOT_READY, "hk_resize has not been called");
  HK_REQUIRE(n_bounds == c->band_count + 1, HK_E_INVALID, "need band_count + 1 = %u boundaries (hk_set_band first), got %u", c->band_count + 1, n_bounds);
  HK_REQUIRE(band_bounds_valid(bounds, c->band_count, (uint32_t)c->RH), HK_E_INVALID,
             "band bounds must run 0 = b[0] < b[1] < ... < b[%u] = %d (scaled render rows)", c->band_count, c->RH);
  c->band_bounds.assign(bounds, bounds + n_bounds);
  c->bounds_generation += 1;
  return HK_OK;
}

int hk_get_band(hk_ctx* c, uint32_t* band_index, uint32_t* band_count) {
  HK_REQUIRE(c, HK_E_INVALID, "ctx is NULL");
  if (band_index) *band_index = c->band_index;
  if (band_count) *band_count = c->band_count;
  return HK_OK;
}
int hk_get_band_bounds(hk_ctx* c, uint32_t* bounds, uint32_t n_bounds) {
  HK_REQUIRE(c && bounds, HK_E_INVALID, "NULL argument");
  HK_REQUIRE(c->RH > 0, HK_E_NOT_READY, "hk_resize has not been called");
  HK_REQUIRE(n_bounds == c->band_count + 1, HK_E_INVALID, "need band_count + 1 = %u entries", c->band_count + 1);
  const uint32_t* explicit_split = c->band_bounds.size() == (size_t)c->band_count + 1 ? c->band_bounds.data() : nullptr;
  for (uint32_t i = 0; i < c->band_count; ++i) {
    uint32_t b0, b1;
    band_rows_in(explicit_split, (uint32_t)c->RH, (uint32_t)c->RH, i, c->band_count, &b0, &b1);
    bounds[i] = b0;
    bounds[i + 1] = b1;
  }
  return HK_OK;
}

int hk_row_costs(hk_ctx* c, uint32_t* out, uint32_t n_rows) {
  HK_REQUIRE(c && out, HK_E_INVALID, "NULL argument");
  HK_REQUIRE(c->H > 0 && c->depth_plane, HK_E_NOT_READY, "hk_resize has not been called");
  HK_REQUIRE(n_rows == (uint32_t)c->H, HK_E_INVALID, "need one counter per full-size row: %d", c->H);
  HK_HIP(hipSetDevice(c->device));
  { const int rc_ = sync_all(c); if (rc_) return rc_; }
  uint32_t* d = nullptr;
  HK_HIP(hipMalloc((void**)&d, (size_t)n_rows * 4));
  launch_count_geometry_rows(c->stream, c->depth_plane, c->W, c->H, d);
  hipError_t e = hipStreamSynchronize(c->stream);
  if (e == hipSuccess) e = hipMemcpy(out, d, (size_t)n_rows * 4, hipMemcpyDeviceToHost);
  (void)hipFree(d);
  HK_REQUIRE(e == hipSuccess, HK_E_HIP, "hk_row_costs failed: %s", hipGetErrorString(e));
  return HK_OK;
}

int hk_balance_bands(hk_ctx* c, uint32_t min_rows, uint32_t* bounds_out, uint32_t n_bounds) {
  int rc = ready(c);
  if (rc) return rc;
  HK_REQUIRE(c->have_frame, HK_E_NOT_READY, "hk_frame_begin has not been called");
  HK_REQUIRE(!bounds_out || n_bounds == c->band_count + 1, HK_E_INVALID, "need band_count + 1 = %u boundaries", c->band_count + 1);
  std::vector<uint32_t> bounds(c->band_count + 1);
  if (c->band_count > 1) {
    if ((rc = hk_pass_run(c, HK_PASS_PREPASS, 0, 0, 0))) return rc;
    std::vector<uint32_t> cost((size_t)c->H);
    if ((rc = hk_row_costs(c, cost.data(), (uint32_t)c->H))) return rc;
    if ((rc = hk_balanced_band_bounds(cost.data(), (uint32_t)c->H, (uint32_t)c->W, (uint32_t)c->RH, c->band_count,
                                      std::max(1u, std::min(min_rows ? min_rows : 8u, (uint32_t)c->RH / c->band_count)) ,
                                      (size_t)c->scene.blob_f4 * 16 > HK_LDS_SCENE_BYTES ? 1.0f / 16.0f : 0.25f, bounds.data()))) return rc;
    if ((rc = hk_set_band_bounds(c, bounds.data(), c->band_count + 1))) return rc;
  } else {
    bounds[0] = 0u;
    bounds[1] = (uint32_t)c->RH;
  }
  if (bounds_out) std::copy(bounds.begin(), bounds.end(), bounds_out);
  return HK_OK;
}

int hk_band_time_ms(hk_ctx* c, float* ms) {
  HK_REQUIRE(c && ms, HK_E_INVALID, "bad argument");
  HK_REQUIRE(c->band_timed, HK_E_NOT_READY, "no frame has been rendered with HK_FRAME_TIME_BAND");
  HK_HIP(hipSetDevice(c->device));
  HK_HIP(hipEventSynchronize(c->band_ev[3]));
  float a = 0.0f, b = 0.0f;
  HK_HIP(hipEventElapsedTime(&a, c->band_ev[0], c->band_ev[1]));
  HK_HIP(hipEventElapsedTime(&b, c->band_ev[2], c->band_ev[3]));
  *ms = a + b;
  return HK_OK;
}

int hk_migrate_bands(hk_ctx* c, const uint32_t* new_bounds, uint32_t n_bounds, uint32_t next_frame_number, const HkSettings* st) {
  HK_REQUIRE(c && st, HK_E_INVALID, "NULL argument");
  HK_REQUIRE(c->RH > 0, HK_E_NOT_READY, "hk_resize has not been called");
  HK_REQUIRE(!new_bounds || n_bounds == c->band_count + 1, HK_E_INVALID, "need band_count + 1 = %u boundaries", c->band_count + 1);
  HK_REQUIRE(band_bounds_valid(new_bounds, c->band_count, (uint32_t)c->RH), HK_E_INVALID, "band bounds must run 0 = b[0] < b[1] < ... < b[%u] = %d", c->band_count, c->RH);
  HK_HIP(hipSetDevice(c->device));
  int rc = join_all(c);
  if (rc) return rc;
  const uint32_t* old_bounds = c->band_bounds.size() == (size_t)c->band_count + 1 ? c->band_bounds.data() : nullptr;
  if (c->band_count > 1 && (rc = comm_migrate(c, old_bounds, new_bounds, next_frame_number, st))) return rc;
  return hk_set_band_bounds(c, new_bounds, new_bounds ? n_bounds : 0u);
}

int hk_band_plan(hk_ctx* c, uint32_t stage, const HkSettings* st, HkHaloOp* ops, uint32_t* n_ops) {
  HK_REQUIRE(c && c->W > 0, HK_E_NOT_READY, "hk_resize has not been called");
  HK_REQUIRE(c->have_frame, HK_E_NOT_READY, "hk_frame_begin has not been called");
  const uint32_t* bounds = c->band_bounds.size() == (size_t)c->band_count + 1 ? c->band_bounds.data() : nullptr;
  return hk_band_plan_bounds((uint32_t)c->W, (uint32_t)c->H, c->ratio, bounds, c->band_index, c->band_count, stage, c->frame.number, st, ops, n_ops);
}

int hk_frame_stage(hk_ctx* c, uint32_t stage, const HkSettings* st, uint32_t flags) {
  int rc = ready(c);
  if (rc) return rc;
  HK_REQUIRE(st, HK_E_INVALID, "settings is NULL");
  HK_REQUIRE(c->band_count <= (uint32_t)c->RH, HK_E_INVALID, "more bands than rows");
  HK_REQUIRE(st->taa <= HK_TAA_NONE && st->upscale_kind <= HK_UPSCALE_SMAA_TU4X, HK_E_INVALID, "bad taa / upscale_kind in settings");
  HK_REQUIRE(!(flags & HK_FRAME_INTERNAL_LATE_JOIN) || c->in_frame_render, HK_E_INVALID, "unknown frame flag");
  HK_REQUIRE(st->indirect_bounces == c->frame.indirect_bounces && (st->temporal_reuse != 0u) == (c->frame.temporal_reuse != 0u) &&
                 (st->emissive_spatial_reuse != 0u) == (c->frame.emissive_spatial_reuse != 0u) &&
                 (st->indirect_spatial_reuse != 0u) == (c->frame.indirect_spatial_reuse != 0u),
             HK_E_INVALID, "HkSettings disagrees with the HkFrame given to hk_frame_begin (indirect_bounces / reuse flags)");
  c->taa = st->taa;
  c->upscale_kind = st->upscale_kind;
  c->upscale_sharpness = st->upscale_sharpness;
  uint32_t ub0, ub1;
  const uint32_t* bounds = c->band_bounds.size() == (size_t)c->band_count + 1 ? c->band_bounds.data() : nullptr;
  HK_REQUIRE(band_bounds_valid(bounds, c->band_count, (uint32_t)c->RH), HK_E_INVALID, "the band boundaries do not fit the current render size (hk_set_band_bounds after hk_resize)");
  band_rows_in(bounds, (uint32_t)c->RH, (uint32_t)c->RH, c->band_index, c->band_count, &ub0, &ub1);
  const int b0 = (int)ub0, b1 = (int)ub1;
  auto clampr = [&](int v) { return std::min(std::max(v, 0), c->RH); };
  const Aprons ap = band_aprons(st);
  const int den = (int)ap.denoise, sp = (int)ap.spatial;
#define HK_RUN(pass, arg, y0, y1)                    \
  do {                                               \
    int a_ = (y0), b_ = (y1);                        \
    if (b_ > a_ && (rc = run_pass(c, pass, arg, a_, b_))) return rc; \
  } while (0)
  if (stage == HK_STAGE_TEMPORAL) {
    {
      const uint32_t p_ = c->mapped_parity & 1u;
      const bool covered = c->side_state[p_] == 2 && c->side_cover[p_] == p_;
      if (c->forked && (!c->normal_twin || (flags & HK_FRAME_EXTERNAL_GBUFFER) || (c->side_state[p_] != 0 && !covered)) && (rc = join_side(c))) return rc;
    }
    int f0, f1;
    full_rows_for(c, clampr(b0 - den - sp), clampr(b1 + den + sp), &f0, &f1);
    const uint32_t parity = c->mapped_parity & 1u;
    const bool wide_clean = !wide_allowed(c) || (!c->wide_tlas_dirty && !c->wide_blas_dirty && !c->wide_mesh_check);
    const bool pre_wanted = c->prepass_pipeline < 0 ? HK_PREPASS_PIPELINE_RULE : c->prepass_pipeline != 0;
    const bool pre_pipelined = pre_wanted && c->pre_stream && c->stream == c->own_stream && c->normal_twin && c->pre_chain_ok && c->pre_last_parity != parity &&
                               !(flags & (HK_FRAME_EXTERNAL_GBUFFER | HK_FRAME_ANTIALIAS | HK_FRAME_TIME_BAND)) && (c->band_count == 1 || HK_PRE_BANDS) && !c->timing_mask && !(c->flags & HK_CTX_COUNT_RAYS) &&
                               wide_clean && !c->derived_dirty && c->scene_epoch == c->pre_seen_epoch && c->post_pending[parity] && f1 > f0 &&
                               (c->side_state[parity] == 0 || (c->side_state[parity] == 2 && c->side_cover[parity] == parity));
    const bool scene_written = c->scene_epoch != c->pre_seen_epoch || !wide_clean;
    c->pre_seen_epoch = c->scene_epoch;
    if (pre_pipelined) {
      if (c->pre_scene_marked) HK_HIP(hipStreamWaitEvent(c->pre_stream, c->pre_scene_mark, 0));
      HK_HIP(hipStreamWaitEvent(c->pre_stream, c->post_done[parity], 0));
      c->post_pending[parity] = false;
    } else if ((flags & HK_FRAME_EXTERNAL_GBUFFER) ? (rc = join_post(c)) : (rc = join_post_parity(c, c->mapped_parity))) {
      return rc;
    }
    bool albedo_done = false;
    if (c->timing_mask) (void)hipEventRecord(c->frame_start, c->stream);
    if (!(flags & HK_FRAME_EXTERNAL_GBUFFER)) {
      if (f1 > f0) {
        const DFrame fr = make_dframe(c);
        GBuffer g = make_gbuffer(c);
        g.albedo_out = (uint2*)c->buf[HK_BUF_ALBEDO];
        unsigned long long* counters = (c->flags & HK_CTX_COUNT_RAYS) ? c->d_counters : nullptr;
        const Jitter j = prepass_jitter(c);
        hkd::WideTrees wide{};
        if ((rc = wide_for_fused(c, &wide))) return rc;
        {
          ScopedTimer timer(c, HK_PASS_PREPASS);
          launch_prepass(pre_pipelined ? c->pre_stream : c->stream, c->scene, fr, c->view.inverse_view_proj, c->view.view_proj, c->pview.view_proj, c->d_prev_models, j.x, j.y, g, f0, f1,
                         counters, &wide);
        }
        HK_HIP(hipGetLastError());
        if (pre_pipelined) {
          HK_HIP(hipEventRecord(c->pre_done, c->pre_stream));
          HK_HIP(hipStreamWaitEvent(c->stream, c->pre_done, 0));
          c->prepasses_pipelined += 1;
        } else if (c->pre_stream && scene_written) {
          HK_HIP(hipEventRecord(c->pre_scene_mark, c->stream));
          c->pre_scene_marked = true;
        }
        albedo_done = true;
      }
    } else if (f1 > f0) {
      launch_derive_planes(c->stream, make_gbuffer(c), c->depth_plane, c->dn_g, c->W, f0, f1);
      c->derived_dirty = false;
    }
    int a0, a1;
    full_rows_for(c, clampr(b0 - den), clampr(b1 + den), &a0, &a1);
    if (!albedo_done) HK_RUN(HK_PASS_FULL_SCREEN_ALBEDO, 0, a0, a1);
    if (c->side_stream && b1 > b0) {
      HK_HIP(hipEventRecord(c->fork_event, c->stream));
      HK_HIP(hipStreamWaitEvent(c->side_stream, c->fork_event, 0));
      c->forked = true;
      c->side_state[c->mapped_parity & 1u] = 1;
      if ((rc = run_pass_on_side(c, HK_PASS_DIRECT_LIT, 0, b0, b1))) return rc;
      if ((rc = run_pass_on_side(c, HK_PASS_DIRECT_EMISSIVE, 0, b0, b1))) return rc;
      HK_RUN(HK_PASS_INDIRECT, 0, b0, b1);
      if (c->band_count > 1 && st->emissive_spatial_reuse && (rc = join_side(c))) return rc;
    } else {
      HK_RUN(HK_PASS_DIRECT_LIT, 0, b0, b1);
      HK_RUN(HK_PASS_DIRECT_EMISSIVE, 0, b0, b1);
      HK_RUN(HK_PASS_INDIRECT, 0, b0, b1);
    }
    c->pre_chain_ok = !(flags & (HK_FRAME_EXTERNAL_GBUFFER | HK_FRAME_ANTIALIAS));
    c->pre_last_parity = parity;
  } else if (stage == HK_STAGE_SPATIAL) {
    if (parks_across_bands(c) && c->det_winner[0]) {
      const int reach = 2 * (int)c->history_now, r0 = clampr(b0 - reach), r1 = clampr(b1 + reach);
      if ((rc = join_side(c))) return rc;
      for (int channel = 0; channel < 3; ++channel) {
        const bool exchanged = channel == 2 ? st->indirect_spatial_reuse != 0 : st->emissive_spatial_reuse != 0;
        const LightTargets t = make_light_targets(c, channel);
        if (!t.det_winner) continue;
        if (exchanged) launch_resolve_scatter(c->stream, t, r0 * c->RW, r1 * c->RW, b0 * c->RW, b1 * c->RW);
        else launch_resolve_scatter(c->stream, t, b0 * c->RW, b1 * c->RW, 0, 0);
      }
      HK_HIP(hipGetLastError());
    }
    if (st->emissive_spatial_reuse) {
      if (c->forked) {
        if ((rc = run_pass_on_side(c, HK_PASS_EMISSIVE_SPATIAL_REUSE, 0, b0, b1))) return rc;
      } else {
        HK_RUN(HK_PASS_EMISSIVE_SPATIAL_REUSE, 0, b0, b1);
      }
    }
    if (st->indirect_spatial_reuse) HK_RUN(HK_PASS_INDIRECT_SPATIAL_REUSE, 0, b0, b1);
    if ((c->band_count > 1 && !(flags & HK_FRAME_INTERNAL_LATE_JOIN)) && (rc = join_side(c))) return rc;
  } else if (stage == HK_STAGE_POST_PROCESS) {
    bool pipelined = c->post_forked;
    if (!pipelined && (rc = post_begin(c, st, &pipelined))) return rc;
    if (st->denoise) {
      const uint32_t nch = st->indirect_bounces == 0 ? 2u : 3u;
      rc = run_demodulation_fused(c, nch, clampr(b0 - 15), clampr(b1 + 15));
      if (!rc) rc = run_denoise_fused(c, nch, 0, clampr(b0 - 7), clampr(b1 + 7));
      if (!rc) rc = run_denoise_fused(c, nch, 1, clampr(b0 - 3), clampr(b1 + 3));
      if (!rc) rc = run_denoise_fused(c, nch, 2, clampr(b0 - 1), clampr(b1 + 1));
      if (!rc) rc = run_denoise_fused(c, nch, 3, b0, b1, true);
      if (c->timing_mask) {
        (void)hipEventRecord(c->frame_stop, c->stream);
        c->frame_timed = true;
      }
      const int rc2 = post_end(c, pipelined);
      if (rc) return rc;
      if (rc2) return rc2;
    } else {
      if ((rc = join_side(c))) return rc;
      HK_RUN(HK_PASS_TONE_MAPPING, 0u, b0, b1);
      if (c->timing_mask) {
        (void)hipEventRecord(c->frame_stop, c->stream);
        c->frame_timed = true;
      }
    }
    c->frames += 1;
  } else if (stage == HK_STAGE_ANTIALIAS) {
    if ((rc = join_post(c))) return rc;
    const bool smaa = st->upscale_kind == HK_UPSCALE_SMAA_TU4X;
    if (smaa) {
      HK_RUN(HK_PASS_SMAA_TU4X, 0, clampr(b0 - 2), clampr(b1 + 2));
      HK_RUN(HK_PASS_SMAA_TU4X_EXTRAPOLATE, 0, clampr(b0 - 1), clampr(b1 + 1));
    }
    if (st->taa == HK_TAA_JASMINE) {
      int w, h;
      buffer_dims(c, HK_BUF_TAA_OUTPUT, &w, &h);
      const int scale = smaa ? 2 : 1;
      HK_RUN(HK_PASS_TAA_JASMINE, 0, std::min(h, scale * b0), b1 == c->RH ? h : std::min(h, scale * b1));
    }
  } else if (stage == HK_STAGE_UPSCALE) {
    if ((rc = join_post(c))) return rc;
    if (st->upscale_kind == HK_UPSCALE_FSR1) {
      uint32_t w0, w1;
      band_rows_in(bounds, (uint32_t)c->RH, (uint32_t)c->H, c->band_index, c->band_count, &w0, &w1);
      HK_RUN(HK_PASS_FSR_EASU, 0, std::max((int)w0 - 1, 0), std::min((int)w1 + 1, c->H));
      HK_RUN(HK_PASS_FSR_RCAS, 0, (int)w0, (int)w1);
    }
  } else {
    HK_REQUIRE(false, HK_E_INVALID, "unknown stage %u", stage);
  }
#undef HK_RUN
  return HK_OK;
}

int hk_frame_render(hk_ctx* c, const HkFrame* f, const HkView* v, const HkPreviousView* pv, const HkLights* l, const HkSettings* st, uint32_t flags) {
  int rc = hk_frame_begin(c, f, v, pv, l);
  if (rc) return rc;
  HK_REQUIRE(st, HK_E_INVALID, "settings is NULL");
// ... 113 lines not shown
    if (derives) c->scene_epoch += 1;
    wide.tlas = c->wide_tlas;
    wide.blas = c->wide_blas;
    wide.tlas_rank = c->wide_tlas_rank;
    wide.blas_rank = c->wide_blas_rank;
    wide.tlas_count = c->scene.tlas_count;
    wide.spill = c->wide_spill;
    wide.lost = c->d_counters + 8;
  }
  launch_cast_rays(c->stream, c->scene, &wide, c->wide_spill_lanes, d_rays, n, flags, d_hits);
  HK_HIP(hipGetLastError());
  return HK_OK;
}
int hk_cast_rays_device(hk_ctx* c, const void* d_rays, uint32_t n, uint32_t flags, void* d_hits) {
  int rc = cast_rays_checked(c, d_rays, n, flags, d_hits);
  if (rc || !n) return rc;
  HK_REQUIRE(((uintptr_t)d_rays % 16) == 0 && ((uintptr_t)d_hits % 16) == 0, HK_E_INVALID, "d_rays and d_hits must be aligned to 16 bytes");
  HK_HIP(hipSetDevice(c->device));
  return cast_rays_enqueue(c, d_rays, n, flags, d_hits);
}
int hk_cast_rays(hk_ctx* c, const HkRay* rays, uint32_t n, uint32_t flags, HkRayHit* hits) {
  int rc = cast_rays_checked(c, rays, n, flags, hits);
  if (rc || !n) return rc;
  HK_HIP(hipSetDevice(c->device));
  const size_t chunk = std::min<size_t>(n, (size_t)1 << 18);
  const size_t per_ray = sizeof(HkRay) + sizeof(HkRayHit);
  if (chunk > c->query_capacity) {
    HK_HIP(hipStreamSynchronize(c->stream));
    if (c->query_staging) (void)hipHostFree(c->query_staging);
    if (c->query_device) (void)hipFree(c->query_device);
    c->query_staging = c->query_device = nullptr;
    c->query_capacity = 0;
    HK_HIP(hipHostMalloc((void**)&c->query_staging, chunk * per_ray, hipHostMallocDefault));
    HK_HIP(hipMalloc((void**)&c->query_device, chunk * per_ray));
    c->query_capacity = chunk;
  }
  uint8_t* const h_rays = c->query_staging;
  uint8_t* const h_hits = c->query_staging + c->query_capacity * sizeof(HkRay);
  uint8_t* const d_rays = c->query_device;
  uint8_t* const d_hits = c->query_device + c->query_capacity * sizeof(HkRay);
  for (size_t done = 0; done < n; done += chunk) {
    const size_t m = std::min<size_t>(chunk, n - done);
    memcpy(h_rays, rays + done, m * sizeof(HkRay));
    HK_HIP(hipMemcpyAsync(d_rays, h_rays, m * sizeof(HkRay), hipMemcpyHostToDevice, c->stream));
    if ((rc = cast_rays_enqueue(c, d_rays, (uint32_t)m, flags, d_hits))) return rc;
    HK_HIP(hipMemcpyAsync(h_hits, d_hits, m * sizeof(HkRayHit), hipMemcpyDeviceToHost, c->stream));
    HK_HIP(hipStreamSynchronize(c->stream));
    memcpy(hits + done, h_hits, m * sizeof(HkRayHit));
  }
  return HK_OK;
}

int hk_buffer_info(hk_ctx* c, uint32_t buffer, uint32_t* w, uint32_t* h, uint32_t* bpp) {
  HK_REQUIRE(c && buffer < HK_BUF_COUNT && buffer_bpp(buffer), HK_E_INVALID, "bad buffer id");
  int bw, bh;
  buffer_dims(c, buffer, &bw, &bh);
  if (w) *w = (uint32_t)bw;
  if (h) *h = (uint32_t)bh;
  if (bpp) *bpp = buffer_bpp(buffer);
  return HK_OK;
}
int hk_read_buffer(hk_ctx* c, uint32_t buffer, void* dst, size_t bytes) {
  HK_REQUIRE(c && dst && buffer < HK_BUF_COUNT && c->buf[buffer], HK_E_INVALID, "bad argument");
  HK_REQUIRE(bytes == buffer_logical_bytes(c, buffer), HK_E_INVALID, "size mismatch: buffer has %zu bytes", buffer_logical_bytes(c, buffer));
  HK_HIP(hipSetDevice(c->device));
  { int rc_ = join_all(c); if (rc_) return rc_; }
  HK_HIP(hipStreamSynchronize(c->stream));
  HK_HIP(hipMemcpy(dst, c->buf[buffer], bytes, hipMemcpyDeviceToHost));
  return HK_OK;
}
int hk_write_buffer(hk_ctx* c, uint32_t buffer, const void* src, size_t bytes) {
  HK_REQUIRE(c && src && buffer < HK_BUF_COUNT && c->buf[buffer], HK_E_INVALID, "bad argument");
  HK_REQUIRE(bytes == buffer_logical_bytes(c, buffer), HK_E_INVALID, "size mismatch: buffer has %zu bytes", buffer_logical_bytes(c, buffer));
  HK_HIP(hipSetDevice(c->device));
  { int rc_ = join_all(c); if (rc_) return rc_; }
  HK_HIP(hipStreamSynchronize(c->stream));
  HK_HIP(hipMemcpy(c->buf[buffer], src, bytes, hipMemcpyHostToDevice));
  if (buffer >= HK_BUF_RESERVOIR0 && buffer < HK_BUF_RESERVOIR0 + 10 && c->tile_meta[buffer - HK_BUF_RESERVOIR0]) {
    const uint32_t k = buffer - HK_BUF_RESERVOIR0;
    HK_HIP(hipMemset(c->tile_meta[k], 0, (size_t)c->tiles_x * c->tiles_y * sizeof(TileMeta)));
    c->tile_meta_zero[k] = true;
  }
  if (buffer == HK_BUF_POSITION || buffer == HK_BUF_NORMAL || buffer == HK_BUF_INSTANCE_MATERIAL) c->derived_dirty = true;
  return HK_OK;
}
int hk_device_ptr(hk_ctx* c, uint32_t buffer, void** ptr, size_t* bytes) {
  HK_REQUIRE(c && ptr && buffer < HK_BUF_COUNT && c->buf[buffer], HK_E_INVALID, "bad argument");
  *ptr = c->buf[buffer];
  if (bytes) *bytes = c->buf_bytes[buffer];
  return HK_OK;
}
int hk_set_stream(hk_ctx* c, void* s) {
  HK_REQUIRE(c, HK_E_INVALID, "ctx is NULL");
  HK_HIP(hipSetDevice(c->device));
  { int rc = join_all(c); if (rc) return rc; }
  HK_HIP(hipStreamSynchronize(c->stream));
  drain_timers(c);
  c->stream = s ? (hipStream_t)s : c->own_stream;
  return HK_OK;
}
int hk_stream(hk_ctx* c, void** s) {
  HK_REQUIRE(c && s, HK_E_INVALID, "bad argument");
  *s = (void*)c->stream;
  return HK_OK;
}
int hk_set_timing_mask(hk_ctx* c, uint32_t mask) {
  HK_REQUIRE(c, HK_E_INVALID, "ctx is NULL");
  c->timing_mask = mask;
  return HK_OK;
}
int hk_get_stats(hk_ctx* c, HkStats* out) {
  HK_REQUIRE(c && out, HK_E_INVALID, "bad argument");
  HK_HIP(hipSetDevice(c->device));
  { int rc = join_all(c); if (rc) return rc; }
  HK_HIP(hipStreamSynchronize(c->stream));
  drain_timers(c);
  memset(out, 0, sizeof(*out));
  unsigned long long h[9] = {};
  HK_HIP(hipMemcpy(h, c->d_counters, sizeof(h), hipMemcpyDeviceToHost));
  out->rays_primary = h[0];
  out->rays_tlas = h[1];
  out->rays_blas = h[2];
  out->walk_node_steps = h[3];
  out->walk_triangle_tests = h[4];
  out->walk_instance_entries = h[5];
  out->walk_closest_hits = h[6];
  out->walk_top_node_steps = h[7];
  out->wide_stack_lost = h[8];
  out->frames = c->frames;
  out->last_frame_ms = c->last_frame_ms;
  out->scene_mesh_builds = c->static_rebuilds;
  out->scene_instance_builds = c->dynamic_rebuilds;
  out->scene_async_instance_uploads = c->async_instance_uploads;
  out->scene_device_refits = c->device_refits;
  out->scene_device_tree_builds = c->device_tree_builds;
  for (int i = 0; i < HK_TIMING_SLOTS; ++i) {
    out->pass_ms_total[i] = c->slot_ms[i];
    out->pass_launches[i] = c->slot_launches[i];
  }
  return HK_OK;
}
int hk_indirect_schedule(hk_ctx* c, uint32_t* out) {
  HK_REQUIRE(c && out, HK_E_INVALID, "NULL argument");
  HK_REQUIRE(c->have_frame, HK_E_NOT_READY, "hk_frame_begin has not been called");
  HK_HIP(hipSetDevice(c->device));
  { const int rc = finalize_scene(c); if (rc) return rc; }
  *out = use_wavefront(c) ? 1u : 0u;
  return HK_OK;
}

int hk_traversal_mode(hk_ctx* c, uint32_t* out, uint32_t* orderings) {
  HK_REQUIRE(c && out, HK_E_INVALID, "NULL argument");
  HK_HIP(hipSetDevice(c->device));
  { const int rc = finalize_scene(c); if (rc) return rc; }
  HK_REQUIRE(c->scene_mem, HK_E_NOT_READY, "no scene uploaded");
  *out = c->scene.flat_mode ? HK_TRAVERSAL_ONE_LEVEL : c->threaded ? (HK_TRAVERSAL_THREADED | (wide_allowed(c) ? HK_TRAVERSAL_WIDE : 0u)) : HK_TRAVERSAL_REFERENCE;
  if (orderings) *orderings = c->scene.flat_mode ? c->scene.flat_mask + 1u : c->threaded ? 8u : 1u;
  return HK_OK;
}

int hk_reset_stats(hk_ctx* c) {
  HK_REQUIRE(c, HK_E_INVALID, "ctx is NULL");
  HK_HIP(hipSetDevice(c->device));
  { const int rc_ = sync_all(c); if (rc_) return rc_; }
  drain_timers(c);
  HK_HIP(hipMemset(c->d_counters, 0, 9 * sizeof(unsigned long long)));
  c->frames = 0;
  for (int i = 0; i < HK_TIMING_SLOTS; ++i) {
    c->slot_ms[i] = 0.0;
    c->slot_launches[i] = 0;
  }
// ... 4 lines not shown
```

### bevy-hikari_amd/csrc/hk_context.hpp

```cpp
#pragma once
#include <hip/hip_runtime.h>
#include <math.h>
#include <stdlib.h>
#include <string.h>

#include <algorithm>
#include <iterator>
#include <chrono>
#include <new>
#include <thread>
#include <utility>
#include <vector>

#include "hk_internal.hpp"
#include "hk_kernels.hpp"

#define HK_HIP(expr)                                                                     \
  do {                                                                                   \
    hipError_t e_ = (expr);                                                              \
    if (e_ != hipSuccess) {                                                              \
      ::hk::set_error("%s failed: %s (%s:%d)", #expr, hipGetErrorString(e_), __FILE__, __LINE__); \
      return HK_E_HIP;                                                                   \
    }                                                                                    \
  } while (0)
// ... 68 lines not shown
struct DynOffsets { size_t tlas, instances, prev_models, light_lo, light_hi, emissives, alias, materials, tex_info, srgb_lut, flat; uint32_t flat_count, flat_orderings; };

struct hk_ctx {
  int device = 0;
  uint32_t flags = 0;
  hipStream_t stream = nullptr;
  hipStream_t own_stream = nullptr;
  bool own_stream_high = false;
  bool main_priority_decided = false;
  hipStream_t pre_stream = nullptr;
  hipEvent_t pre_done = nullptr, pre_scene_mark = nullptr;
  bool pre_scene_marked = false;
  int prepass_pipeline = -1;
  uint64_t scene_epoch = 0, pre_seen_epoch = 0;
  bool pre_chain_ok = false;
  uint32_t pre_last_parity = 0;
  uint64_t prepasses_pipelined = 0;
  int main_priority = -1;
  hipStream_t side_stream = nullptr;
  hipEvent_t fork_event = nullptr, join_event = nullptr;
  bool forked = false;
  hipEvent_t side_done = nullptr;
  uint8_t side_state[2] = {0, 0};
  uint8_t side_cover[2] = {0, 0};
  void* normal_twin = nullptr;
  void* instance_material_twin = nullptr;
  hipStream_t post_stream = nullptr;
  hipEvent_t post_fork = nullptr;
  hipEvent_t post_done[2] = {nullptr, nullptr};
  bool post_pending[2] = {false, false};
  bool post_forked = false;
  hipStream_t post_saved_main = nullptr;
  void* albedo_twin = nullptr;
  void* depth_gradient_twin = nullptr;
  void* dn_g_twin = nullptr;
  void* render_twin[3] = {nullptr, nullptr, nullptr};
  void* variance_twin[3] = {nullptr, nullptr, nullptr};
  int spatial_window = -1;
  uint64_t spatial_windowed_launches = 0;
  bool frame_pipeline = true;
  bool wf_timeline = false;
  bool flat_walk = true;
  int flat_orderings = 0;
  bool trace_update = false;
  bool in_frame_render = false;

  std::vector<HkVertex> vertices;
  std::vector<HkPrimitive> primitives;
  std::vector<HkNode> asset_nodes;
  std::vector<HkMaterial> materials;
  std::vector<HkInstance> instances;
  std::vector<HkNode> instance_nodes;
  std::vector<HkEmissive> emissives;
  std::vector<HkNode> emissive_nodes;
  std::vector<HkAliasEntry> alias_table;
  struct HostTexture { std::vector<uint32_t> texels; uint32_t w, h, flags; };
  std::vector<HostTexture> textures;
  bool have_meshes = false, have_materials = false, have_instances = false, have_noise = false;
  bool mesh_dirty = true, dynamic_dirty = true, textures_dirty = true;
  std::vector<float> prev_models;
  std::vector<int64_t> node_prim_offset;

  uint8_t* scene_mem = nullptr;
  size_t dyn_capacity = 0, static_bytes = 0;
  bool two_slots = false;
  int slot = 0;
  Blob dyn_blob;
  std::vector<float4> tlas_tmp;
  bool trees_pending_on_device = false;
  bool threaded = false;
  uint8_t* staging[2] = {nullptr, nullptr};
  size_t staging_bytes[2] = {0, 0};
  hipEvent_t staging_done[2] = {nullptr, nullptr};
  bool staging_pending[2] = {false, false};
  uint64_t async_instance_uploads = 0;
  size_t st_nodes = 0, st_v0 = 0, st_v1 = 0, st_v2 = 0, st_vn = 0, st_vuv = 0;
  uint64_t static_rebuilds = 0, dynamic_rebuilds = 0;
  int* det_winner[3] = {nullptr, nullptr, nullptr};
  bool det_lite_clean[3] = {false, false, false};
  TileMeta* tile_meta[10] = {};
  bool tile_meta_zero[10] = {};
  int tiles_x = 0, tiles_y = 0;
  uint32_t elide_serial = 0;
  DynOffsets dyn_off{};
  float4 *rf_inst_lo = nullptr, *rf_inst_hi = nullptr, *rf_prev_models = nullptr;
  uint32_t* rf_emissive_of_instance = nullptr;
  float* rf_alias_scratch = nullptr;
  size_t rf_instances = 0, rf_alias = 0;
  bool rf_ready = false;
  hkd::RefitUpdate* rf_updates[2] = {nullptr, nullptr};
  size_t rf_updates_cap[2] = {0, 0};
  hipEvent_t rf_done[2] = {nullptr, nullptr};
  bool rf_pending[2] = {false, false};
  int rf_k = 0;
  std::vector<uint32_t> rf_last_moved;
  bool mirrors_stale = false;
  std::vector<struct DeformMesh*> deform;
  struct DeformStage { uint8_t* p = nullptr; size_t cap = 0; hipEvent_t done = nullptr; bool pending = false; };
  std::vector<DeformStage> df_stage;
  bool deform_pending = false;
  bool meshes_deformed = false;
  uint64_t instances_generation = 0;
  uint64_t device_refits = 0, device_tree_builds = 0;
  void* lbvh_scratch = nullptr;
  size_t lbvh_scratch_cap = 0;
  std::vector<std::pair<uint32_t, uint32_t>> load_pending_ranges;
  uint32_t load_device_limit = HK_MESH_REBUILD_MAX_TRIANGLES;
  uint32_t last_load[4] = {0, 0, 0, 0};
  double last_load_ms[5] = {0, 0, 0, 0, 0};
  bool mesh_rebuild_one_workgroup = false;
  const float4* d_prev_models = nullptr;
  DevArray<uint32_t> d_noise;
  DevArray<uint32_t> d_tex_data;
  DScene scene{};

  int W = 0, H = 0, RW = 0, RH = 0;
  int UW = 0, UH = 0;
  bool uv_fast = false;
  uint32_t mapped_parity = 0;
  float ratio = 1.0f;
  void* buf[HK_BUF_COUNT] = {};
  size_t buf_bytes[HK_BUF_COUNT] = {};
  float* depth_plane = nullptr;
  float* prev_depth_plane = nullptr;
  void* dn_g = nullptr;
  void* dn_extra[2][4] = {};
  float* dn_extra_var[2] = {};
  bool derived_dirty = false;
  void* wf_mem = nullptr;
  hkd::WfBuffers wf{};
  float4* wide_tlas = nullptr;
  float4* wide_blas = nullptr;
  uint32_t* wide_spill = nullptr;
  uint32_t* wide_tlas_rank = nullptr;
  uint32_t* wide_blas_rank = nullptr;
  size_t wide_rank_instances = 0, wide_rank_primitives = 0;
  size_t wide_tlas_slots = 0, wide_blas_slots = 0, wide_spill_lanes = 0;
  bool wide_tlas_dirty = true, wide_blas_dirty = true;
  bool wide_mesh_check = true;
  std::vector<std::pair<uint32_t, uint32_t>> wide_meshes;
  int compute_units = 0;

  HkFrame frame{};
  HkView view{};
  HkPreviousView pview{};
  HkLights lights{};
  bool have_frame = false;
  uint32_t taa = HK_TAA_JASMINE, upscale_kind = HK_UPSCALE_SMAA_TU4X;
  float upscale_sharpness = 0.0f;

  uint32_t band_index = 0, band_count = 1;
  std::vector<uint32_t> band_bounds;
  uint32_t bounds_generation = 0;
  void* comm = nullptr;
  uint32_t history_rows = HK_HISTORY_AUTO;
  uint32_t history_now = 0;
  hipEvent_t band_ev[4] = {nullptr, nullptr, nullptr, nullptr};
  bool band_timed = false;

  uint8_t* query_staging = nullptr;
  uint8_t* query_device = nullptr;
  size_t query_capacity = 0;

  unsigned long long* d_counters = nullptr;
  uint64_t frames = 0;
  uint32_t timing_mask = 0;
// ... 26 lines not shown
```

### bevy-hikari_amd/csrc/hk_kernels.hpp

```cpp
#pragma once
#include <hip/hip_runtime.h>

#include "../../include/hikari_hip.h"
#include "hk_device.hpp"

namespace hkd {

struct GBuffer {
  float4* __restrict__ position;
  uint32_t* __restrict__ normal;
  float2* __restrict__ depth_gradient;
  float2* __restrict__ instance_material;
  float4* __restrict__ velocity_uv;
  float* __restrict__ depth;
  float4* __restrict__ dn_g;
  uint2* __restrict__ albedo_out;
};
struct TileMeta {
  unsigned long long id, src;
  uint32_t valid, poison, pad0, pad1;
};
struct LightTargets {
  const PackedReservoir* __restrict__ previous;
  PackedReservoir* current;
  PackedReservoir* previous_spatial;
  PackedReservoir* spatial;
  float* variance;
  uint2* render;
  int* det_winner;
  int* det_to;
  PackedReservoir* det_pending;
  int det_lite;
  TileMeta* m_current;
  TileMeta* m_spatial;
  TileMeta* m_previous_spatial;
  uint32_t serial;
  int tiles_x;
  int rw;
};
struct WfBuffers {
  uint32_t* ctr;
  uint32_t* pixel;
  float4* state;
  float4 *cr0, *cr1;
  float4 *sr0, *sr1;
  uint32_t* sr2;
  float4* ch0;
  uint32_t* ch1;
  uint32_t* sh;
  uint32_t* alive[2];
  uint32_t* shadow[2];
  uint32_t cap;
  unsigned long long* timeline;
  uint32_t timeline_mode;
};
struct WideTrees {
  const float4* tlas;
  const float4* blas;
  const uint32_t* tlas_rank;
  const uint32_t* blas_rank;
  uint32_t tlas_count;
  unsigned long long* lost;
  uint32_t* spill;
};
struct RefitUpdate {
  uint32_t instance;
  uint32_t moved;
  float model[16];
  float aabb_center[3], aabb_half[3];
};
struct MeshTree {
  uint32_t n;
  uint32_t *parent, *left, *right, *first, *last;
  uint32_t *leaf_parent, *leaf_shape;
  uint32_t* arrived;
  uint8_t* swap;
  float4 *node_lo, *node_hi;
  float4 *tri_lo, *tri_hi;
};
struct ForestMesh {
  uint32_t tri_begin, n_tris;
  uint32_t primitive;
  uint32_t node_offset;
};
struct RefitScene {
  DInstance* instances;
  float4* prev_models;
  float4 *inst_lo, *inst_hi;
  const uint32_t* emissive_of_instance;
  DEmissive* emissives;
  float2* alias;
  float* alias_scratch;
  const float4* materials;
  const float4 *tri_v0, *tri_v1, *tri_v2;
};
struct DemodTargets {
  const uint2* __restrict__ albedo;
  const float* variance[3];
  const uint2* render[3];
  uint2* output[3];
  float* internal_variance[3];
};
struct DenoiseTargets {
  const uint2* __restrict__ albedo;
  const float4* __restrict__ dn_g;
  const float* __restrict__ depth;
  const float2* __restrict__ depth_gradient;
  const uint2* input[3];
  uint2* output[3];
  const float* internal_variance[3];
  uint2* tone_mapped;
  float clear_color[4];
};

__device__ __forceinline__ float4 denoise_geometry(uint32_t packed_normal, float instance) {
  const f3 n = normalize(xyz(unpack4x8snorm(packed_normal)));
  return make_float4(n.x, n.y, n.z, instance);
}

struct Pixel { int x, y; bool valid; };

__device__ __forceinline__ unsigned long long record_id(const PackedReservoir& p) {
  const uint32_t w[16] = {p.radiance.x, p.radiance.y, p.random.x, p.random.y, f2u(p.visible_position.x), f2u(p.visible_position.y), f2u(p.visible_position.z),
                          f2u(p.visible_position.w), f2u(p.sample_position.x), f2u(p.sample_position.y), f2u(p.sample_position.z), f2u(p.sample_position.w),
                          p.visible_normal, p.sample_normal, p.reservoir.x, p.reservoir.y};
  unsigned long long h = 0x9E3779B97F4A7C15ull;
#pragma unroll
  for (int k = 0; k < 16; ++k) {
    h ^= (unsigned long long)w[k] + 0x9E3779B97F4A7C15ull + (h << 6) + (h >> 2);
    h *= 0xBF58476D1CE4E5B9ull;
    h ^= h >> 29;
  }
  return h | 1ull;
}
__device__ __forceinline__ bool wave_leader() { return (int)__lane_id() == __ffsll((long long)__ballot(1)) - 1; }
__device__ __forceinline__ int wave_tile(const Pixel& px, int tiles_x) {
  const int lane = threadIdx.x & 63;
  return ((px.y - (lane >> 3)) >> 3) * tiles_x + ((px.x - (lane & 7)) >> 3);
}
__device__ __forceinline__ bool tile_holds(const TileMeta* m, int tile, unsigned long long id) {
  const TileMeta v = m[tile];
  return v.valid > v.poison && v.id == id;
}
__device__ __forceinline__ void tile_mark(TileMeta* m, int tile, unsigned long long id, unsigned long long src, uint32_t serial) {
  if (wave_leader()) {
    m[tile].id = id;
    m[tile].src = src;
    m[tile].valid = serial;
  }
}
__device__ __forceinline__ void tile_unknown(TileMeta* m, int tile) {
  if (wave_leader()) m[tile].valid = 0u;
}

constexpr int HK_TILE_LDS_UINT4 = 4 * 65;
__device__ __forceinline__ void store_packed_tile(uint4* lds, PackedReservoir* __restrict__ buf, int width, const Pixel& px, const PackedReservoir& p, bool write) {
  const int lane = threadIdx.x & 63;
  const unsigned long long wmask = __ballot(write);
  if (wmask == 0ull) return;
  lds[0 * 65 + lane] = make_uint4(p.radiance.x, p.radiance.y, p.random.x, p.random.y);
  lds[1 * 65 + lane] = make_uint4(f2u(p.visible_position.x), f2u(p.visible_position.y), f2u(p.visible_position.z), f2u(p.visible_position.w));
  lds[2 * 65 + lane] = make_uint4(f2u(p.sample_position.x), f2u(p.sample_position.y), f2u(p.sample_position.z), f2u(p.sample_position.w));
  lds[3 * 65 + lane] = make_uint4(p.visible_normal, p.sample_normal, p.reservoir.x, p.reservoir.y);
  __builtin_amdgcn_wave_barrier();
  const int tile_x0 = px.x - (lane & 7), tile_y0 = px.y - (lane >> 3);
#pragma unroll
  for (int k = 0; k < 4; ++k) {
    const int m = k * 64 + lane, record = m >> 2, part = m & 3;
    const uint4 v = lds[part * 65 + record];
    if ((wmask >> record) & 1ull) {
      const int x = tile_x0 + (record & 7), y = tile_y0 + (record >> 3);
      reinterpret_cast<uint4*>(buf + (x + width * y))[part] = v;
    }
  }
  __builtin_amdgcn_wave_barrier();
}

template <bool XCD_BANDS = true>
__device__ __forceinline__ Pixel pixel_of_thread(int width, int row_begin, int row_end) {
  const int tiles_x = (width + 15) >> 4;
  const uint32_t nb = gridDim.x;
  uint32_t b = blockIdx.x;
  const uint32_t per = nb >> 3;
  if ((XCD_BANDS || nb < 2048u) && per > 0 && b < per * 8u) b = (b & 7u) * per + (b >> 3);
  const int tile_x = (int)(b % (uint32_t)tiles_x), tile_y = (int)(b / (uint32_t)tiles_x);
  const int wave = threadIdx.x >> 6, lane = threadIdx.x & 63;
  Pixel p;
  p.x = tile_x * 16 + (wave & 1) * 8 + (lane & 7);
  p.y = row_begin + tile_y * 16 + (wave >> 1) * 8 + (lane >> 3);
  p.valid = p.x < width && p.y < row_end;
  return p;
}

template <int W, bool XCD_BANDS>
__device__ __forceinline__ Pixel pixel_of_thread_rows(int width, int row_begin, int row_end) {
  constexpr int H = 64 / W;
  const int tiles_x = (width + W - 1) / W;
  uint32_t b = blockIdx.x;
  const uint32_t nb = gridDim.x, per = nb >> 3;
  if (XCD_BANDS && per > 0 && b < per * 8u) b = (b & 7u) * per + (b >> 3);
  const int tile_x = (int)(b % (uint32_t)tiles_x), tile_y = (int)(b / (uint32_t)tiles_x);
  const int wave = threadIdx.x >> 6, lane = threadIdx.x & 63;
  Pixel p;
  p.x = tile_x * W + (lane & (W - 1));
  p.y = row_begin + tile_y * (4 * H) + wave * H + (lane / W);
  p.valid = p.x < width && p.y < row_end;
  return p;
}

}

#define HK_LDS_SCENE_BYTES 32768u

namespace hk {
static inline dim3 grid_for_rows(int wave_width, int width, int rows) {
  int wg_rows = 4 * (64 / wave_width);
  int tiles_x = (width + wave_width - 1) / wave_width, tiles_y = (rows + wg_rows - 1) / wg_rows;
  return dim3((unsigned)(tiles_x * tiles_y), 1, 1);
}
static inline dim3 grid_for(int width, int rows) {
  int tiles_x = (width + 15) / 16, tiles_y = (rows + 15) / 16;
// ... 70 lines not shown
```

### bevy-hikari_amd/csrc/kernels.hip

```cpp
#include <hip/hip_runtime.h>
#include <hip/hip_ext.h>

#include <cmath>

#include "hk_device.hpp"
#include "hk_kernels.hpp"
#include "hk_light.hpp"
#include "hk_prepass.hpp"
#include "hk_wide.hpp"

namespace hkd {

__global__ __launch_bounds__(256) void k_join_winners(LightTargets t, int p0, int p1, int own0, int own1) {
  const int i = p0 + (int)(blockIdx.x * 256u + threadIdx.x);
  if (i >= p1 || (i >= own0 && i < own1)) return;
  const int to = t.det_to[i];
  if (to >= 0) atomicMax(&t.det_winner[to], i);
}
__global__ __launch_bounds__(256) void k_resolve_scatter(LightTargets t, int p0, int p1) {
  const int i = p0 + (int)(blockIdx.x * 256u + threadIdx.x);
  if (i >= p1) return;
  const int to = t.det_to[i];
  if (to >= 0 && t.det_winner[to] == i) store_packed(t.previous_spatial, to, load_packed(t.det_pending, i));
}

__device__ __forceinline__ bool lite_is_background(const DFrame& fr, const float* __restrict__ depth_plane, int pixel, bool indirect) {
  if (indirect && fr.indirect_bounces == 0u) return true;
  const int y = pixel / fr.rw, x = pixel - y * fr.rw;
  int dcx, dcy;
  jittered_deferred_coords(fr, coords_to_uv(fr, x, y), &dcx, &dcy);
  const float depth = in_bounds(dcx, dcy, fr.dw, fr.dh) ? depth_plane[dcx + fr.dw * dcy] : 0.0f;
  return depth < HK_F32_EPSILON;
}
__global__ __launch_bounds__(256) void k_resolve_scatter_lite(LightTargets t, DFrame fr, const float* __restrict__ depth_plane, int indirect, int p0, int p1) {
  const int p = p0 + (int)(blockIdx.x * 256u + threadIdx.x);
  if (p >= p1) return;
  const int to = t.det_to[p];
  if (to < 0 || to == p || t.det_winner[to] != p) return;
  if (lite_is_background(fr, depth_plane, p, indirect != 0)) return;
  t.det_winner[to] = -1;
  const bool owner_stored = lite_is_background(fr, depth_plane, to, indirect != 0) || t.det_to[to] == to;
  if (owner_stored && to > p) return;
  store_packed(t.previous_spatial, to, load_packed(t.det_pending, p));
  if (t.m_previous_spatial) {
    const int ty = to / t.rw, tx = to - ty * t.rw;
    atomicMax(&t.m_previous_spatial[(ty >> 3) * t.tiles_x + (tx >> 3)].poison, t.serial);
  }
}

#ifndef HK_PREPASS_WIDE_WAVES
#define HK_PREPASS_WIDE_WAVES 5
#endif
#ifndef HK_PREPASS_FLAT_WAVES
#define HK_PREPASS_FLAT_WAVES 5
#endif
template <bool COUNT, int LDS>
__global__ __launch_bounds__(256, (LDS == 4 ? HK_PREPASS_WIDE_WAVES : (LDS == 2 ? HK_PREPASS_FLAT_WAVES : 1))) void k_prepass(DScene gsc, DFrame fr, PrepassParams pp, GBuffer g, int row_begin, int row_end,
                                                  unsigned long long* counters) {
  const DScene sc = stage_scene<LDS>(gsc);
  const Pixel px = pixel_of_thread<false>(fr.dw, row_begin, row_end);
  RayCounters rc{0, 0};
  uint32_t primary = 0;
  __shared__ uint32_t wide_lds[LDS == 4 ? HK_WIDE_LDS_STACK * 256u : 1u];
  if (px.valid) {
    Ray ray = primary_ray(fr, pp, (float)px.x, (float)px.y);
    Hit hit;
#pragma unroll 1
    for (int attempt = 0;; ++attempt) {
      if (LDS == 4) {
        WideStackPrivate<HK_WIDE_LDS_STACK, 96u> stack;
        stack.lds = wide_lds;
        stack.lost = pp.wide.lost;
        hit = traverse_top_wide<COUNT>(sc, pp.wide, ray, HK_F32_MAX, 0.0f, HK_DONT_EXCLUDE, stack, rc);
      } else {
        hit = traverse_top(sc, ray, HK_F32_MAX, 0.0f, HK_DONT_EXCLUDE, rc);
      }
      if (attempt != 0 || !clip_at_near_plane(fr, pp, (float)px.x, (float)px.y, ray, hit)) break;
    }
    rc.tlas = 0;
    primary = 1;
    rc.hits += hit.instance_index != HK_U32_MAX ? 1u : 0u;
    prepass_store(sc, fr, pp, g, px.x, px.y, ray, hit);
  }
  flush_counters<COUNT>(rc, primary, counters);
}

__global__ __launch_bounds__(256) void k_full_screen_albedo(DScene sc, DFrame fr, GBuffer g, uint2* __restrict__ albedo, int row_begin, int row_end) {
  const Pixel px = pixel_of_thread(fr.dw, row_begin, row_end);
  if (!px.valid) return;
  const int idx = px.x + fr.dw * px.y;
  const float4 position_depth = g.position[idx];
  if (position_depth.w < HK_F32_EPSILON) {
    albedo[idx] = make_uint2(0u, 0u);
    return;
  }
  const f3 normal = xyz(unpack4x8snorm(g.normal[idx]));
  const uint32_t material = f32_to_u32(g.instance_material[idx].y);
  const float4 velocity_uv = g.velocity_uv[idx];
  Surface surface = retreive_surface(sc, material, F2(velocity_uv.z, velocity_uv.w));
  f3 view_direction = calculate_view(fr, xyz(position_depth));
  albedo[idx] = pack_f16x4(F4(env_brdf(view_direction, normal, surface), 1.0f));
}

#ifndef HK_DIRECT_GLOBAL_WAVES
#define HK_DIRECT_GLOBAL_WAVES 4
#endif
#ifndef HK_DIRECT_FLAT_WAVES
#define HK_DIRECT_FLAT_WAVES 4
#endif
template <bool EMISSIVE_LIT, bool COUNT, int LDS>
__global__ __launch_bounds__(256, (LDS == 0 ? HK_DIRECT_GLOBAL_WAVES : (LDS == 2 ? HK_DIRECT_FLAT_WAVES : 1))) void k_direct_lit(DScene gsc, DFrame fr, GBuffer g, LightTargets t, int row_begin, int row_end,
                                                     unsigned long long* counters) {
  const DScene sc = stage_scene<LDS>(gsc);
  const Pixel px = pixel_of_thread<false>(fr.rw, row_begin, row_end);
  RayCounters rc{0, 0};
  __shared__ uint4 tile_lds[4][HK_TILE_LDS_UINT4];
  PackedReservoir out = pack_reservoir(zero_reservoir());
  bool write_current = false, background = false;
  if (px.valid) {
    const int x = px.x, y = px.y;
    const int index = x + fr.rw * y;
    const f2 uv = coords_to_uv(fr, x, y);
    Sample s = zero_sample();
    int dcx, dcy;
    jittered_deferred_coords(fr, uv, &dcx, &dcy);
    const bool din = in_bounds(dcx, dcy, fr.dw, fr.dh);
    const int didx = dcx + fr.dw * dcy;
    const float4 position_depth = din ? g.position[didx] : make_float4(0, 0, 0, 0);
    const f3 position = xyz(position_depth);
    const float depth = position_depth.w;

    if (depth < HK_F32_EPSILON) {
      Reservoir r = zero_reservoir();
      set_reservoir(r, s, 0.0f);
      out = pack_reservoir(r);
      write_current = true;
      background = true;
      t.variance[index] = 0.0f;
      t.render[index] = make_uint2(0u, 0u);
    } else {
      const f3 normal = xyz(unpack4x8snorm(g.normal[didx]));
      const float2 imf = g.instance_material[didx];
      const uint32_t im_x = f32_to_u32(imf.x), im_y = f32_to_u32(imf.y);
      const float4 velocity_uv = g.velocity_uv[didx];

      s.random = noise_fetch(sc, x, y, fr.number);
      s.random = fract(s.random + fr.number_golden);
      s.visible_position = F4(position, depth);
      s.visible_normal = normal;
      s.visible_instance = im_x;

      Ray ray;
      ray.origin = F3(0, 0, 0); ray.direction = F3(0, 0, 0); ray.inv_direction = F3(0, 0, 0);
      HitInfo info = empty_hit_info(F3(0, 0, 0), F3(0, 0, 0));
      info.position = F4(0, 0, 0, 0); info.instance_index = 0u; info.material_index = 0u;

      const f2 previous_uv = jittered_deferred_uv(fr, uv, 0.25f) - F2(velocity_uv.x, velocity_uv.y);
      Reservoir r = load_reservoir_uv(t.previous, previous_uv, fr.rw, fr.rh);
      if (t.det_lite) t.det_to[index] = -1;
      const bool prev_on_screen = fabsf(previous_uv.x - 0.5f) <= 0.5f && fabsf(previous_uv.y - 0.5f) <= 0.5f;
      const int previous_index = f32_to_i32(previous_uv.x * (float)fr.rw) + fr.rw * f32_to_i32(previous_uv.y * (float)fr.rh);

      if (!check_previous_reservoir(r, s) && prev_on_screen) store_previous_spatial(t, index, previous_index, pack_reservoir(r));

      const uint32_t validate_interval = EMISSIVE_LIT ? fr.emissive_validate_interval : fr.direct_validate_interval;
      const uint32_t select_light_instance = EMISSIVE_LIT ? im_x : HK_DONT_SAMPLE_EMISSIVE;
      const bool validation_frame = (fr.number % validate_interval) == 0u;

      if (!validation_frame || r.count < 4.0f) {
        LightCandidate candidate = select_light_candidate(sc, fr, s.random, xyz(s.visible_position), s.visible_normal, select_light_instance, info, rc);
        ray.origin = position + normal * HK_RAY_BIAS;
        ray.direction = candidate.direction;
        ray.inv_direction = 1.0f / ray.direction;
        bool trace_condition = dot(candidate.direction, normal) > 0.0f;
        trace_condition = trace_condition && candidate.p > 0.0f;
        if (EMISSIVE_LIT) trace_condition = trace_condition && candidate.emissive_instance != HK_DONT_SAMPLE_EMISSIVE;
        if (trace_condition) {
          Hit hit = traverse_top<true>(sc, ray, candidate.max_distance, candidate.min_distance, candidate.emissive_instance, rc);
          occlude_hit_info(ray, hit, info);
          s.radiance = EMISSIVE_LIT ? input_radiance(sc, fr, ray, info, false, candidate.emissive_instance, false)
                                    : input_radiance(sc, fr, ray, info, true, HK_DONT_SAMPLE_EMISSIVE, false);
        }
        s.sample_position = info.position;
        s.sample_normal = info.normal;
        float w_new = (candidate.p > 0.0f) ? luminance(xyz(s.radiance)) / candidate.p : 0.0f;
        temporal_restir(r, s, w_new, fr.max_temporal_reuse_count);
      }

      if (validation_frame) {
        LightCandidate candidate = select_light_candidate(sc, fr, r.s.random, xyz(r.s.visible_position), r.s.visible_normal, select_light_instance, info, rc);
        ray.origin = xyz(s.visible_position) + s.visible_normal * HK_RAY_BIAS;
        ray.direction = normalize(xyz(r.s.sample_position) - xyz(s.visible_position));
        ray.inv_direction = 1.0f / ray.direction;
        f4 validate_radiance = F4(0, 0, 0, 0);
        bool trace_condition = dot(candidate.direction, r.s.visible_normal) > 0.0f;
        trace_condition = trace_condition && candidate.p > 0.0f;
        if (EMISSIVE_LIT) trace_condition = trace_condition && candidate.emissive_instance != HK_DONT_SAMPLE_EMISSIVE;
        if (trace_condition) {
          Hit hit = traverse_top<true>(sc, ray, candidate.max_distance, candidate.min_distance, candidate.emissive_instance, rc);
          occlude_hit_info(ray, hit, info);
          validate_radiance = EMISSIVE_LIT ? input_radiance(sc, fr, ray, info, false, candidate.emissive_instance, false)
                                           : input_radiance(sc, fr, ray, info, true, HK_DONT_SAMPLE_EMISSIVE, false);
        }
        if (r.count >= 4.0f) {
          s.random = r.s.random;
          s.sample_position = info.position;
          s.sample_normal = info.normal;
          s.radiance = validate_radiance;
        }
        float luminance_ratio = luminance(xyz(validate_radiance)) / fmax_(luminance(xyz(r.s.radiance)), 0.0001f);
        if (luminance_ratio > 1.25f || luminance_ratio < 0.8f) {
// ... 108 lines not shown
};
__device__ __forceinline__ bool bounce_step(const DScene& sc, const DFrame& fr, uint32_t n, PathState& p, RayCounters& rc, SecTimer& tm) {
  HK_SEC(tm, 1);
  f4 rand_sample = sample_cosine_hemisphere(F2(p.random.x, p.random.y));
  Ray ray;
  ray.origin = p.position + p.normal * HK_RAY_BIAS;
  ray.direction = mul(normal_basis(p.normal), xyz(rand_sample));
  ray.inv_direction = 1.0f / ray.direction;

  HK_SEC(tm, 2);
  HK_ABLATE_WALK(sc, ray, HK_F32_MAX, 0.0f, HK_DONT_EXCLUDE, rc);
  Hit hit = traverse_top(sc, ray, HK_F32_MAX, 0.0f, HK_DONT_EXCLUDE, rc);
  HK_SEC(tm, 3);
  rc.hits += hit.instance_index != HK_U32_MAX ? 1u : 0u;
  HitInfo info = hit_info(sc, ray, hit);
  if (n == 0u) {
    p.first_position = info.position;
    p.first_normal = info.normal;
    p.pdf = rand_sample.w;
  }
  const f3 sample_position = xyz(info.position);
  const f3 sample_normal = info.normal;

  if (hit.instance_index != HK_U32_MAX) {
    f3 out_radiance = F3(0, 0, 0);
    Surface surface = retreive_surface(sc, info.material_index, info.uv);
    surface.roughness = 1.0f;
    const uint32_t info_instance = info.instance_index;
    HK_SEC(tm, 4);
    LightCandidate candidate = select_light_candidate(sc, fr, p.random, sample_position, sample_normal, info_instance, info, rc);
    HK_SEC(tm, 5);
    const bool sample_directional = (candidate.emissive_instance == HK_DONT_SAMPLE_EMISSIVE);
    const f3 bounce_view_direction = normalize(p.position - sample_position);

    const f3 next_transport = p.transport * env_brdf(bounce_view_direction, sample_normal, surface);
    if (dot(candidate.direction, sample_normal) > 0.0f && candidate.p > 0.0f) {
      ray.origin = sample_position + sample_normal * HK_RAY_BIAS;
      ray.direction = candidate.direction;
      ray.inv_direction = 1.0f / ray.direction;
      const f4 in_clear = input_radiance(sc, fr, ray, info, sample_directional, candidate.emissive_instance, false);
      f3 add[2];
#pragma unroll
      for (int o = 0; o < 2; ++o) {
        const f4 in_radiance = o == 0 ? in_clear : F4(0.0f, 0.0f, 0.0f, 1.0f);
        out_radiance = shading(fr, bounce_view_direction, sample_normal, ray.direction, surface, in_radiance);
        out_radiance = out_radiance / candidate.p;
        if (n > 0u) out_radiance = (rand_sample.w < 0.01f) ? F3(0, 0, 0) : out_radiance / rand_sample.w;
        float out_luminance = luminance(out_radiance);
        if (out_luminance > fr.max_indirect_luminance) out_radiance = out_radiance * fr.max_indirect_luminance / out_luminance;
        add[o] = p.transport * out_radiance;
      }
      HK_SEC(tm, 6);
      HK_ABLATE_WALK(sc, ray, candidate.max_distance, candidate.min_distance, candidate.emissive_instance, rc);
      hit = traverse_top(sc, ray, candidate.max_distance, candidate.min_distance, candidate.emissive_instance, rc);
      HK_SEC(tm, 7);
      p.radiance = p.radiance + F4(hit.instance_index != HK_U32_MAX ? add[1] : add[0], 1.0f);
    }
    p.transport = next_transport;
    p.random = fract(p.random + fr.number_golden);
    p.position = sample_position;
    p.normal = sample_normal;
    return true;
  }
  f3 out_radiance = xyz(input_radiance(sc, fr, ray, info, false, HK_DONT_SAMPLE_EMISSIVE, true));
  p.radiance = p.radiance + F4(p.transport * out_radiance, 0.0f);
  return false;
}

#ifndef HK_INDIRECT_FLAT_WAVES
#define HK_INDIRECT_FLAT_WAVES 5
#endif
template <bool MULTIPLE_BOUNCES, bool COUNT, int LDS>
__global__ __launch_bounds__(256, (LDS == 2 && MULTIPLE_BOUNCES ? HK_INDIRECT_FLAT_WAVES : 4)) void k_indirect(DScene gsc, DFrame fr, GBuffer g, LightTargets t, int row_begin, int row_end,
                                                   unsigned long long* counters) {
  const DScene sc = stage_scene<LDS>(gsc);
  const Pixel px = pixel_of_thread<false>(fr.rw, row_begin, row_end);
  RayCounters rc{0, 0};
  SecTimer tm;
  tm.start();
  if (px.valid) {
    const int x = px.x, y = px.y;
    const int index = x + fr.rw * y;
    const f2 uv = coords_to_uv(fr, x, y);
    int dcx, dcy;
    jittered_deferred_coords(fr, uv, &dcx, &dcy);
    const bool din = in_bounds(dcx, dcy, fr.dw, fr.dh);
    const int didx = dcx + fr.dw * dcy;
    const float4 position_depth = din ? g.position[didx] : make_float4(0, 0, 0, 0);
    const f3 position = xyz(position_depth);
    const float depth = position_depth.w;

    Sample s = zero_sample();
    Reservoir r = zero_reservoir();

    const bool background = fr.indirect_bounces == 0u || depth < HK_F32_EPSILON;
    const bool all_background = __ballot(!background) == 0ull;
    const int tile = wave_tile(px, t.tiles_x);
    if (background) {
      const PackedReservoir pr = pack_reservoir(r);
      bool skip_current = false, skip_spatial = false, skip_previous_spatial = false;
      if (t.m_current && all_background) {
        const unsigned long long id = record_id(pr);
        skip_current = tile_holds(t.m_current, tile, id);
        skip_spatial = tile_holds(t.m_spatial, tile, id);
        skip_previous_spatial = tile_holds(t.m_previous_spatial, tile, id);
        if (!skip_current) tile_mark(t.m_current, tile, id, 0ull, t.serial);
        if (!skip_spatial) tile_mark(t.m_spatial, tile, id, 0ull, t.serial);
        if (!skip_previous_spatial) tile_mark(t.m_previous_spatial, tile, id, 0ull, t.serial);
      }
      if (!skip_current) store_packed(t.current, index, pr);
      if (!skip_spatial) store_packed(t.spatial, index, pr);
      if (!skip_previous_spatial) store_previous_spatial(t, index, index, pr);
      t.variance[index] = 0.0f;
      t.render[index] = make_uint2(0u, 0u);
    } else {
      const f3 normal = normalize(xyz(unpack4x8snorm(g.normal[didx])));
      const float2 imf = g.instance_material[didx];
      const uint32_t im_x = f32_to_u32(imf.x), im_y = f32_to_u32(imf.y);
      const float4 velocity_uv = g.velocity_uv[didx];

      s.random = noise_fetch(sc, x, y, fr.number);
      s.random = fract(s.random + fr.number_golden);
      s.visible_position = F4(position, depth);
      s.visible_normal = normal;
      s.visible_instance = im_x;

      Ray ray;
      float pdf = 0.0f;
      Surface surface;

      if (MULTIPLE_BOUNCES) {
        PathState p;
        p.random = s.random;
        p.position = xyz(s.visible_position);
        p.normal = s.visible_normal;
        p.transport = F3(1.0f, 1.0f, 1.0f);
        p.radiance = s.radiance;
        p.first_position = s.sample_position;
        p.first_normal = s.sample_normal;
        p.pdf = 0.0f;
        for (uint32_t n = 0u; n < fr.indirect_bounces && (p.transport.x > 0.01f || p.transport.y > 0.01f || p.transport.z > 0.01f); n += 1u) {
          if (!bounce_step(sc, fr, n, p, rc, tm)) break;
        }
        s.radiance = p.radiance;
        s.sample_position = p.first_position;
        s.sample_normal = p.first_normal;
        pdf = p.pdf;
        {
          int didx2 = didx, x2 = x, y2 = y;
          asm volatile("" : "+v"(didx2), "+v"(x2), "+v"(y2));
          const float4 pd2 = g.position[didx2];
          const float2 imf2 = g.instance_material[didx2];
          Sample s2 = zero_sample();
          s2.random = noise_fetch(sc, x2, y2, fr.number);
          s2.random = fract(s2.random + fr.number_golden);
          s2.visible_position = F4(pd2);
          s2.visible_normal = normalize(xyz(unpack4x8snorm(g.normal[didx2])));
          s2.visible_instance = f32_to_u32(imf2.x);
          s2.radiance = s.radiance;
          s2.sample_position = s.sample_position;
          s2.sample_normal = s.sample_normal;
          HK_SEC(tm, 8);
          indirect_temporal_tail(sc, fr, t, x2 + fr.rw * y2, coords_to_uv(fr, x2, y2), xyz(F4(pd2)), g.velocity_uv[didx2], f32_to_u32(imf2.y), s2, pdf);
        }
      } else {
        f4 rand_sample = sample_cosine_hemisphere(F2(s.random.x, s.random.y));
        ray.origin = xyz(s.visible_position) + s.visible_normal * HK_RAY_BIAS;
        ray.direction = mul(normal_basis(s.visible_normal), xyz(rand_sample));
        ray.inv_direction = 1.0f / ray.direction;
        Hit hit = traverse_top(sc, ray, HK_F32_MAX, 0.0f, HK_DONT_EXCLUDE, rc);
        rc.hits += hit.instance_index != HK_U32_MAX ? 1u : 0u;
// ... 61 lines not shown
    if constexpr (WINDOWED) {
      const unsigned lx = (unsigned)(x - x0), ly = (unsigned)(y - y0);
      if (lx < (unsigned)HK_SPATIAL_TILE_W && ly < (unsigned)HK_SPATIAL_TILE_W) return tile[ly * (unsigned)HK_SPATIAL_TILE_W + lx];
    }
    return plane[x + dw * y];
  }
};
template <bool WINDOWED>
HKD uint32_t spatial_tap_reaches(const DFrame& fr, const DepthWindow<WINDOWED>& g, const SpatialTaps& taps, const SpatialPixel& me, uint32_t i, int* out_x, int* out_y) {
  const float angle = HK_TAU * fract((float)i * HK_GOLDEN_RATIO + me.rot + fr.random_float_number);
  const float radius = taps.radius[i - 1u];
  float sn, cs;
  sincos_(angle, &sn, &cs);
  const f2 offset = radius * F2(cs, sn);

  const int scx = f32_to_i32(offset.x + (float)me.x), scy = f32_to_i32(offset.y + (float)me.y);
  *out_x = scx;
  *out_y = scy;
  const f2 sample_uv = coords_to_uv(fr, scx, scy);
  if (sample_uv.x < 0.0f || sample_uv.y < 0.0f || sample_uv.x > 1.0f || sample_uv.y > 1.0f) return 1u;
  int sdx, sdy;
  jittered_deferred_coords(fr, sample_uv, &sdx, &sdy);
  const float sample_depth = g.at(sdx, sdy);

  const float depth_ratio = me.depth / sample_depth;
  if (depth_ratio < 0.9f || depth_ratio > 1.1f) return 2u;

  const float tap_interval = taps.tap_interval[i - 1u];
  const uint32_t tap_count = taps.tap_count[i - 1u];
  bool occluded = false;
  const f2 dir = normalize(offset);
  float march_depth[6];
#pragma unroll
  for (uint32_t j = 1u; j <= 6u; j += 1u) {
    march_depth[j - 1u] = 0.0f;
    if (j <= tap_count) {
      const float tap_dist = (float)j * tap_interval;
      const f2 tap_offset = tap_dist * dir;
      const f2 tap_uv = me.uv + F2(quotient_by_reciprocal(tap_offset.x, fr.rcp_rw), quotient_by_reciprocal(tap_offset.y, fr.rcp_rh));
      int tdx, tdy;
      jittered_deferred_coords(fr, tap_uv, &tdx, &tdy);
      march_depth[j - 1u] = g.at(tdx, tdy);
    }
  }
#pragma unroll
  for (uint32_t j = 1u; j <= 6u; j += 1u) {
    if (j <= tap_count) {
      const float ref_depth = mix(me.depth, sample_depth, taps.march_frac[i - 1u][j - 1u]);
      if (march_depth[j - 1u] > ref_depth + 0.00001f) occluded = true;
    }
  }
  return occluded ? 5u : 0u;
}
template <bool EMISSIVE_LIT>
HKD uint32_t spatial_tap_merge(const ShadingSite& site, const Sample& s, Reservoir& r, const PackedReservoir& record) {
  const Reservoir q = unpack_reservoir(record);
  const bool normal_miss = dot(s.visible_normal, q.s.visible_normal) < 0.866f;
  if (q.count < HK_F32_EPSILON || normal_miss) return 3u;

  const f3 to_sample = xyz(q.s.sample_position) - xyz(s.visible_position);
  const float to_sample_length = sqrtf(dot(to_sample, to_sample));
  const f3 sample_direction = to_sample * (1.0f / to_sample_length);
  if (dot(sample_direction, s.visible_normal) < 0.0f) return 4u;

  const float jacobian = (q.s.sample_position.w > 0.5f) ? compute_jacobian_shared(q.s, sample_direction, to_sample_length) : 1.0f;
  if (EMISSIVE_LIT) {
    merge_reservoir(r, q, luminance(xyz(q.s.radiance)) / jacobian);
  } else {
    f3 out_radiance = shade(site, sample_direction, q.s.radiance);
    merge_reservoir(r, q, luminance(out_radiance) / jacobian);
  }
  return 0u;
}
#ifndef HK_SPATIAL_WGS
#define HK_SPATIAL_WGS 4
#endif
template <bool EMISSIVE_LIT, bool WINDOWED>
__global__ __launch_bounds__(256, HK_SPATIAL_WGS) void k_spatial_reuse(DScene sc, DFrame fr, GBuffer g, LightTargets t, SpatialTaps taps, int row_begin, int row_end) {
  const Pixel px = pixel_of_thread<false>(fr.rw, row_begin, row_end);
  if (!WINDOWED && !px.valid) return;
  constexpr uint32_t SPATIAL_REUSE_COUNT = EMISSIVE_LIT ? 8u : 16u;
  const int x = px.x, y = px.y;
  const int index = x + fr.rw * y;
  const f2 uv = coords_to_uv(fr, x, y);
  int dcx, dcy;
  jittered_deferred_coords(fr, uv, &dcx, &dcy);
  const bool din = in_bounds(dcx, dcy, fr.dw, fr.dh) && px.valid;
  const int didx = dcx + fr.dw * dcy;
  const float4 position_depth = din ? g.position[didx] : make_float4(0, 0, 0, 0);
  const f3 position = xyz(position_depth);
  const float depth = position_depth.w;
  __shared__ float depth_tile[WINDOWED ? HK_SPATIAL_TILE_W * HK_SPATIAL_TILE_W : 1];
  DepthWindow<WINDOWED> window{g.depth, depth_tile, 0, 0, fr.dw, fr.dh};
  if constexpr (WINDOWED) {
    const int lane = threadIdx.x & 63, wave = threadIdx.x >> 6;
    const int block_x0 = x - (lane & 7) - (wave & 1) * 8, block_y0 = y - (lane >> 3) - (wave >> 1) * 8;
    window.x0 = (int)floorf((float)(block_x0 - HK_SPATIAL_TILE_REACH) * (float)fr.dw / (float)fr.rw);
    window.y0 = (int)floorf((float)(block_y0 - HK_SPATIAL_TILE_REACH) * (float)fr.dh / (float)fr.rh);
    if (__syncthreads_or(px.valid && !(depth < HK_F32_EPSILON))) {
      for (int k = (int)threadIdx.x; k < HK_SPATIAL_TILE_W * HK_SPATIAL_TILE_W; k += 256) {
        const int ly = k / HK_SPATIAL_TILE_W, lx = k - ly * HK_SPATIAL_TILE_W;
        const int gx = window.x0 + lx, gy = window.y0 + ly;
        depth_tile[k] = in_bounds(gx, gy, fr.dw, fr.dh) ? g.depth[gx + fr.dw * gy] : 0.0f;
      }
      __syncthreads();
    }
    if (!px.valid) return;
  }

  const bool background = depth < HK_F32_EPSILON;
  const bool all_background = __ballot(!background) == 0ull;
  const int tile = wave_tile(px, t.tiles_x);
  unsigned long long input_id = 0ull;
  if (t.m_current && all_background) {
    const TileMeta in = t.m_current[tile];
    if (in.valid > in.poison) {
      input_id = in.id;
      const TileMeta have = t.m_spatial[tile];
      if (have.valid > have.poison && have.src == input_id) {
        t.render[index] = make_uint2(0u, 0u);
        return;
      }
    }
  }
  Reservoir r = unpack_reservoir(load_packed(t.current, index));
  if (background) {
    const PackedReservoir pr = pack_reservoir(r);
    store_packed(t.spatial, index, pr);
    if (t.m_spatial) {
      if (all_background && input_id != 0ull) tile_mark(t.m_spatial, tile, record_id(pr), input_id, t.serial);
      else tile_unknown(t.m_spatial, tile);
    }
    t.render[index] = make_uint2(0u, 0u);
    return;
  }
  const uint32_t im_y = f32_to_u32(g.instance_material[didx].y);
  const float4 velocity_uv = g.velocity_uv[didx];
  const Surface surface = retreive_surface(sc, im_y, F2(velocity_uv.z, velocity_uv.w));
  const bool use_spatial_variance = r.count <= 4.0f;
  const f2 previous_uv = jittered_deferred_uv(fr, uv, 0.25f) - F2(velocity_uv.x, velocity_uv.y);

  Reservoir q = r;
  const Sample s = q.s;
  const float max_lifetime = (fr.max_reservoir_lifetime <= 1.0f) ? HK_F32_MAX : fr.max_reservoir_lifetime;
  if (r.lifetime <= max_lifetime) r = load_reservoir_uv(t.previous_spatial, previous_uv, fr.rw, fr.rh);

  const f3 view_direction = calculate_view(fr, position);
  const ShadingSite site = make_site(fr, view_direction, s.visible_normal, surface);
  if (EMISSIVE_LIT) {
    merge_reservoir(r, q, luminance(xyz(q.s.radiance)));
  } else {
    f3 out_radiance = shade(site, normalize(xyz(s.sample_position) - xyz(s.visible_position)), s.radiance);
    merge_reservoir(r, q, luminance(out_radiance));
  }
  r.s.visible_position = s.visible_position;
  r.s.visible_normal = s.visible_normal;

  const float rot = dot(s.random, F4(1.0f, 1.0f, 1.0f, 1.0f));
#ifdef HK_PROFILE_SECTIONS
  struct TapStats {
    uint32_t n[6] = {0u, 0u, 0u, 0u, 0u, 0u};
    __device__ ~TapStats() {
      for (int k = 0; k < 6; ++k)
        if (n[k]) atomicAdd(&g_sections[10 + k], (unsigned long long)n[k]);
    }
  } taps_;
#define HK_TAP(k) (taps_.n[k] += 1u)
#else
#define HK_TAP(k) ((void)0)
#endif
  const SpatialPixel me{x, y, uv, depth, rot};
  __shared__ uint32_t kept[WINDOWED ? 16u * 256u : 1u];
// ... 266 lines not shown
```

### bevy-hikari_amd/csrc/kernels_denoise.hip

```cpp
#include <hip/hip_runtime.h>

#include "hk_device.hpp"
#include "hk_kernels.hpp"

#ifndef HK_DENOISE_W
#define HK_DENOISE_W 64
#endif

namespace hkd {

__global__ __launch_bounds__(256) void k_derive_planes(GBuffer g, float* __restrict__ depth_plane, float4* __restrict__ dn_g, int width, int row_begin,
                                                       int row_end) {
  const Pixel px = pixel_of_thread(width, row_begin, row_end);
  if (!px.valid) return;
  const int idx = px.x + width * px.y;
  const float depth = g.position[idx].w;
  depth_plane[idx] = depth;
  dn_g[idx] = denoise_geometry(g.normal[idx], g.instance_material[idx].x);
}

__global__ __launch_bounds__(256) void k_count_geometry_rows(const float* __restrict__ depth, int width, uint32_t* __restrict__ out) {
  __shared__ uint32_t partial[4];
  const int y = (int)blockIdx.x;
  uint32_t n = 0;
  for (int x = (int)threadIdx.x; x < width; x += 256) n += !(depth[(size_t)y * width + x] < HK_F32_EPSILON) ? 1u : 0u;
  for (int off = 32; off > 0; off >>= 1) n += __shfl_down(n, off);
  if ((threadIdx.x & 63) == 0) partial[threadIdx.x >> 6] = n;
  __syncthreads();
  if (threadIdx.x == 0) out[y] = partial[0] + partial[1] + partial[2] + partial[3];
}

template <int NCH>
__global__ __launch_bounds__(256) void k_demodulation(DFrame fr, DemodTargets d, int row_begin, int row_end) {
  const Pixel px = pixel_of_thread_rows<64, true>(fr.rw, row_begin, row_end);
  if (!px.valid) return;
  const int x = px.x, y = px.y, index = x + fr.rw * y;
  const f2 uv = coords_to_uv(fr, x, y);
  const f2 deferred_uv = jittered_deferred_uv(fr, uv, 0.5f);
  int ax, ay, rx, ry;
  nearest_coords(deferred_uv, fr.dw, fr.dh, &ax, &ay);
  const f3 albedo = xyz(unpack_f16x4(d.albedo[ax + fr.dw * ay]));
  nearest_coords(uv, fr.rw, fr.rh, &rx, &ry);
  uint2 render_in[NCH];
#pragma unroll
  for (int ch = 0; ch < NCH; ++ch) render_in[ch] = d.render[ch][rx + fr.rw * ry];
  float tap_variance[9][NCH];
  bool tap_inside[9];
#pragma unroll
  for (int ox = -1; ox <= 1; ++ox) {
#pragma unroll
    for (int oy = -1; oy <= 1; ++oy) {
      const int k = (ox + 1) * 3 + (oy + 1);
      const f2 sample_uv = uv + F2((float)ox * fr.inv_rw, (float)oy * fr.inv_rh);
      tap_inside[k] = !(sample_uv.x < 0.0f || sample_uv.y < 0.0f || sample_uv.x > 1.0f || sample_uv.y > 1.0f);
      int sx, sy;
      nearest_coords(sample_uv, fr.rw, fr.rh, &sx, &sy);
      const int at = tap_inside[k] ? sx + fr.rw * sy : index;
#pragma unroll
      for (int ch = 0; ch < NCH; ++ch) tap_variance[k][ch] = d.variance[ch][at];
    }
  }
#pragma unroll
  for (int ch = 0; ch < NCH; ++ch) {
    f3 irradiance = xyz(unpack_f16x4(render_in[ch]));
    const f3 qd = irradiance / albedo;
    irradiance = F3(albedo.x < 0.01f ? 0.0f : qd.x, albedo.y < 0.01f ? 0.0f : qd.y, albedo.z < 0.01f ? 0.0f : qd.z);
    d.output[ch][index] = pack_f16x4(F4(irradiance, 1.0f));
  }
  float sum_variance[NCH];
#pragma unroll
  for (int ch = 0; ch < NCH; ++ch) sum_variance[ch] = 0.0f;
#pragma unroll
  for (int ox = -1; ox <= 1; ++ox) {
#pragma unroll
    for (int oy = -1; oy <= 1; ++oy) {
      const int k = (ox + 1) * 3 + (oy + 1);
#pragma unroll
      for (int ch = 0; ch < NCH; ++ch) {
        const float variance = tap_variance[k][ch];
        const float with_tap = sum_variance[ch] + fr.kernel[(oy + 1) * 3 + (ox + 1)] * fmax_(variance, 0.0f);
        sum_variance[ch] = (tap_inside[k] && !(variance > HK_F32_MAX)) ? with_tap : sum_variance[ch];
      }
    }
  }
#pragma unroll
  for (int ch = 0; ch < NCH; ++ch) d.internal_variance[ch][index] = sum_variance[ch];
}

__device__ __forceinline__ bool nan_or_above_max(f3 v) { return !(v.x <= HK_F32_MAX) || !(v.y <= HK_F32_MAX) || !(v.z <= HK_F32_MAX); }

#ifndef HK_DENOISE_WAVES
#define HK_DENOISE_WAVES 8
#endif
template <int LEVEL, int NCH, int FFMASK>
__global__ __launch_bounds__(256, HK_DENOISE_WAVES) void k_denoise(DFrame fr, DenoiseTargets d, int row_begin, int row_end) {
  const Pixel px = pixel_of_thread_rows<HK_DENOISE_W, false>(fr.rw, row_begin, row_end);
  if (!px.valid) return;
  constexpr int STEP = 8 >> LEVEL;
  const int x = px.x, y = px.y, index = x + fr.rw * y;
  int col_texel[3], row_texel[3];
  bool col_inside[3], row_inside[3];
#pragma unroll
  for (int a = 0; a < 3; ++a) {
    const f2 tap_uv = coords_to_uv(fr, x + (a - 1) * STEP, y + (a - 1) * STEP);
    col_inside[a] = !(tap_uv.x < 0.0f || tap_uv.x > 1.0f);
    row_inside[a] = !(tap_uv.y < 0.0f || tap_uv.y > 1.0f);
    nearest_coords(jittered_deferred_uv(fr, tap_uv, 0.5f), fr.dw, fr.dh, &col_texel[a], &row_texel[a]);
  }
  const int dx = col_texel[1], dy = row_texel[1];
  const int didx = dx + fr.dw * dy;
  const float4 gc = d.dn_g[didx];
  const float depth = d.depth[didx];
  if (depth < HK_F32_EPSILON) {
#pragma unroll
    for (int ch = 0; ch < NCH; ++ch) d.output[ch][index] = make_uint2(0u, 0u);
    if (LEVEL == 3 && d.tone_mapped) d.tone_mapped[index] = pack_f16x4(F4(d.clear_color[0], d.clear_color[1], d.clear_color[2], d.clear_color[3]));
    return;
  }
  const float2 dg = d.depth_gradient[didx];
  const f2 depth_gradient = F2(dg.x, dg.y);
  const f3 normal = F3(gc.x, gc.y, gc.z);
  const float instance = gc.w;

  constexpr int OX[8] = {-1, 0, 1, -1, 1, -1, 0, 1};
  constexpr int OY[8] = {-1, -1, -1, 0, 0, 1, 1, 1};
  bool tap_inside[8];
  float w_geometry[8];
#pragma unroll
  for (int k = 0; k < 8; ++k) {
    const int ox = OX[k], oy = OY[k];
    tap_inside[k] = col_inside[ox + 1] && row_inside[oy + 1];
    w_geometry[k] = 0.0f;
    if (tap_inside[k]) {
      const int gx = col_texel[ox + 1], gy = row_texel[oy + 1];
      const float4 gs = d.dn_g[gx + fr.dw * gy];
      const float sample_depth = d.depth[gx + fr.dw * gy];
      const f3 sample_normal = F3(gs.x, gs.y, gs.z);
      const float w_normal = pow16_(fmax_(0.0f, dot(normal, sample_normal)));
      const float w_depth = exp_nonpositive_((-fabsf(depth - sample_depth)) / (fabsf(dot(depth_gradient, F2((float)ox, (float)oy))) + 0.01f));
      const float w_instance = fmax_(0.0f, 1.0f - fabsf(instance - gs.w));
      w_geometry[k] = w_normal * w_depth * w_instance;
    }
  }
  f4 albedo = F4(0, 0, 0, 0), tone_sum = F4(0, 0, 0, 0);
  if (LEVEL == 3) albedo = unpack_f16x4(d.albedo[didx]);
#pragma unroll
  for (int ch = 0; ch < NCH; ++ch) {
    const float variance = d.internal_variance[ch][index];
    const uint2 centre = d.input[ch][index];
    f3 irradiance = xyz(unpack_f16x4(centre));
    f3 sum_irradiance = irradiance * fr.kernel[4];
    float sum_w = fr.kernel[4];
    if (nan_or_above_max(irradiance)) {
      irradiance = F3(0, 0, 0);
      sum_irradiance = F3(0, 0, 0);
      sum_w = 0.0f;
    }
    const float lum = luminance(irradiance);
    const float lum_denominator = 4.0f * pow_quarter_(variance) + 0.001f;
    const double inv_lum_denominator = 1.0 / (double)lum_denominator;
    uint2 tap[8];
#pragma unroll
    for (int k = 0; k < 8; ++k) tap[k] = tap_inside[k] ? d.input[ch][index + OX[k] * STEP + fr.rw * (OY[k] * STEP)] : make_uint2(0u, 0u);
    float ff_moment_1 = 0.0f, ff_moment_2 = 0.0f, ff_count = 0.0f;
    bool black = (centre.x | (centre.y & 0xFFFFu)) == 0u && lum_denominator == lum_denominator;
#pragma unroll
    for (int k = 0; k < 8; ++k) black = black && (tap[k].x | (tap[k].y & 0xFFFFu)) == 0u;
    if (__ballot(!black) == 0ull) {
#pragma unroll
      for (int k = 0; k < 8; ++k) {
        if (!tap_inside[k]) continue;
        const float w = clamp_(w_geometry[k] * 1.0f, 0.0f, 1.0f) * fr.kernel[(OY[k] + 1) * 3 + (OX[k] + 1)];
        const float zw = 0.0f * w;
        sum_irradiance = sum_irradiance + F3(zw, zw, zw);
        sum_w += w;
      }
    } else {
#pragma unroll
      for (int k = 0; k < 8; ++k) {
        if (!tap_inside[k]) continue;
        const f3 irr = xyz(unpack_f16x4(tap[k]));
        if (nan_or_above_max(irr)) continue;
// ... 80 lines not shown
```

### bevy-hikari_amd/plugin.py

```python
import ctypes as C
import dataclasses
import json
import math
import os
from dataclasses import dataclass, field
from typing import Optional

import numpy as np

from . import _ffi as F

ASSETS = os.path.join(os.path.dirname(os.path.abspath(__file__)), "assets")

WORKGROUP_SIZE = 8
NOISE_TEXTURE_COUNT = 16


class graph:
    NAME = "hikari"

    class node:
        PREPASS = "hikari_prepass"
        LIGHT = "hikari_light"
        POST_PROCESS = "hikari_post_process"
# ... 740 lines not shown
            return False, repr(err)

    def comm_unique_id(self):
        ident = (C.c_uint8 * 128)()
        self.api.call("comm_unique_id", ident)
        return bytes(ident)

    def comm_init(self, rank, n_ranks, ident):
        buf = (C.c_uint8 * 128).from_buffer_copy(ident)
        self.api.call("comm_init", self.ctx, rank, n_ranks, buf)

    def comm_set_history_rows(self, rows):
        self.set_history_rows(rows)

    def set_history_rows(self, rows=F.HISTORY_AUTO):
        self.api.call("set_history_rows", self.ctx, int(rows))

    def history_rows(self):
        n = F.u32(0)
        self.api.call("history_rows", self.ctx, C.byref(n))
        return n.value

    def scene_bounds(self):
        mn, mx = (F.f32 * 3)(), (F.f32 * 3)()
        self.api.call("scene_bounds", self.ctx, mn, mx)
        return list(mn), list(mx)

    def comm_gather(self, buffer, root=0):
        self.api.call("comm_gather", self.ctx, buffer, root)

    def debug_comm_loopback(self, src_buffer, dst_buffer, row_begin, row_end, overlapped=False):
        self.api.call("debug_comm_loopback", self.ctx, src_buffer, dst_buffer, row_begin, row_end, 1 if overlapped else 0)

    def comm_destroy(self):
        self.api.call("comm_destroy", self.ctx)

    def stats(self):
        s = F.HkStats()
        self.api.call("get_stats", self.ctx, C.byref(s))
        return s

    def reset_stats(self):
        self.api.call("reset_stats", self.ctx)

    def stream(self):
        h = C.c_void_p()
        self.api.call("stream", self.ctx, C.byref(h))
        return h.value or 0

    def set_stream(self, hip_stream_ptr):
        self.api.call("set_stream", self.ctx, C.c_void_p(hip_stream_ptr))

    def set_timing_mask(self, mask):
        self.api.call("set_timing_mask", self.ctx, mask)

    def indirect_schedule(self):
        v = C.c_uint32()
        self.api.call("indirect_schedule", self.ctx, C.byref(v))
        return "wavefront" if v.value else "fused"

    def traversal_mode(self):
        v, n = C.c_uint32(), C.c_uint32()
        self.api.call("traversal_mode", self.ctx, C.byref(v), C.byref(n))
        return ("reference", "threaded", "one-level")[v.value & 0xFF], n.value

    def wide_walk(self):
        v = C.c_uint32()
        self.api.call("traversal_mode", self.ctx, C.byref(v), None)
        return bool(v.value & 0x100)

    def set_debug_option(self, option, value):
        self.api.call("debug_set_option", self.ctx, option, int(value))

    def main_stream_priority(self):
        v = F.u32()
        self.api.call("debug_main_stream_priority", self.ctx, C.byref(v))
        return bool(v.value & 1), bool(v.value & 2)

    def prepasses_pipelined(self):
        v = F.u32()
        self.api.call("debug_main_stream_priority", self.ctx, C.byref(v))
        return int(v.value >> 8)

    def spatial_windowed_launches(self):
        n = C.c_uint64()
        self.api.call("debug_spatial_windowed_launches", self.ctx, C.byref(n))
        return int(n.value)

    def measure_hbm(self, bytes_per_array=1 << 30, reps=8):
        cp, tr = C.c_double(), C.c_double()
        self.api.call("measure_hbm", self.ctx, bytes_per_array, reps, C.byref(cp), C.byref(tr))
        return cp.value, tr.value

    def measure_gather(self, footprint_bytes, bytes_per_step=32, waves_per_simd=7, steps=512, workgroups=0):
        a, b = C.c_double(), C.c_double()
        self.api.call("measure_gather", self.ctx, int(footprint_bytes), bytes_per_step, waves_per_simd, steps, workgroups, C.byref(a), C.byref(b))
        return a.value, b.value

    def measure_valu(self, iters=2048):
        r = (C.c_double * 4)()
        self.api.call("measure_valu", self.ctx, iters, r)
        return {1 << k: r[k] for k in range(4)}

    def debug_math(self, op, x, y=None):
        return debug_math_call(self.api, self.ctx, op, x, y)


def debug_math_call(api, ctx, op, x, y=None):
    op = int(op)
    x = np.ascontiguousarray(x, dtype=np.float32)
    width = 16 if 16 <= op <= 19 or 35 <= op <= 52 else 1
    n, rest = divmod(x.size, width)
    if rest:
        raise ValueError(f"debug_math op {op} reads {width} floats of x per item, got {x.size}")
    yy = None if y is None else np.ascontiguousarray(y, dtype=np.float32)
    ywidth = 4 if 46 <= op <= 49 else 1
    if ywidth == 4 and yy is None:
        raise ValueError(f"debug_math op {op} takes its vector in y")
    if yy is not None and yy.size != ywidth * n:
        raise ValueError(f"debug_math op {op} reads {ywidth} floats of y per item: {ywidth * n} for {n} items, got {yy.size}")
    out = np.empty(n, dtype=np.float32)
    fp = lambda a: a.ctypes.data_as(C.POINTER(F.f32))
    api.call("debug_math", ctx, op, fp(x), None if yy is None else fp(yy), fp(out), n)
    return out


class FrameCounter:
    def __init__(self, value=0):
        self.value = value

    def tick(self):
        self.value += 1
        return self.value


def frame_uniform(settings: HikariSettings, frame_number: int):
    f = F.HkFrame()
    s = settings.to_c()
    F.api().call("frame_from_settings", C.byref(s), frame_number, C.byref(f))
    return f


class _Node:
    IN_VIEW = "view"

    def __init__(self, engine: Engine):
        self.engine = engine


class PrepassNode(_Node):
    def run(self, settings: HikariSettings):
        self.engine.set_view_options(settings.taa, settings.upscale.kind, settings.upscale.sharpness_)
        self.engine.pass_run(F.PASS_PREPASS)


class LightNode(_Node):
    def run(self, settings: HikariSettings):
        e = self.engine
        e.pass_run(F.PASS_FULL_SCREEN_ALBEDO)
        e.pass_run(F.PASS_DIRECT_LIT)
        e.pass_run(F.PASS_DIRECT_EMISSIVE)
        if settings.emissive_spatial_reuse:
            e.pass_run(F.PASS_EMISSIVE_SPATIAL_REUSE)
        e.pass_run(F.PASS_INDIRECT)
        if settings.indirect_spatial_reuse:
            e.pass_run(F.PASS_INDIRECT_SPATIAL_REUSE)
# ... 88 lines not shown
```

### include/hikari_hip_debug.h

```cpp
#ifndef HIKARI_HIP_DEBUG_H
#define HIKARI_HIP_DEBUG_H

#include "hikari_hip.h"

#ifdef __cplusplus
extern "C" {
#endif
#if defined(__GNUC__)
#pragma GCC visibility push(default)
#endif

int hk_debug_read_trees(hk_ctx* ctx, HkNode* instance_nodes, uint32_t instance_cap, HkNode* emissive_nodes, uint32_t emissive_cap);
int hk_debug_read_mesh_nodes(hk_ctx* ctx, HkNode* out, uint32_t cap, uint32_t* count, uint32_t* orderings);
int hk_debug_last_load(hk_ctx* ctx, uint32_t out[4]);
int hk_debug_last_load_times(hk_ctx* ctx, double out[5]);
int hk_debug_read_mesh_geometry(hk_ctx* ctx, const HkMeshIndex* mesh, float* positions, float* normals, uint32_t vertex_cap, float* triangles,
                                uint32_t triangle_cap, float box[6], uint32_t* n_vertices, uint32_t* n_triangles);
int hk_debug_read_emitters(hk_ctx* ctx, float* records, uint32_t records_cap, uint32_t* n_records, float* alias, uint32_t alias_cap, uint32_t* n_alias);

int hk_measure_hbm(hk_ctx* ctx, size_t bytes_per_array, uint32_t reps, double* copy_gbs, double* triad_gbs);
int hk_measure_valu(hk_ctx* ctx, uint32_t iters, double ginstr_s[4]);

int hk_debug_math(hk_ctx* ctx, uint32_t op, const float* x, const float* y, float* out, size_t n);

int hk_measure_gather(hk_ctx* ctx, size_t footprint_bytes, uint32_t bytes_per_step, uint32_t waves_per_simd, uint32_t steps,
                      uint32_t workgroups , double* gloads_s, double* gbytes_s);

int hk_debug_read_wf_timeline(hk_ctx* ctx, unsigned long long* out, uint32_t n );

int hk_debug_comm_loopback(hk_ctx* ctx, uint32_t src_buffer, uint32_t dst_buffer, uint32_t row_begin, uint32_t row_end,
                           uint32_t mode );

int hk_debug_spatial_windowed_launches(hk_ctx* ctx, uint64_t* out);

int hk_debug_main_stream_priority(hk_ctx* ctx, uint32_t* out);

int hk_debug_comm_lanes(hk_ctx* ctx, uint32_t* lanes);

#define HK_DEBUG_OPT_SPATIAL_WINDOW 0u
#define HK_DEBUG_OPT_FRAME_PIPELINE 1u
#define HK_DEBUG_OPT_WF_TIMELINE 2u
#define HK_DEBUG_OPT_FLAT_WALK 3u
#define HK_DEBUG_OPT_FLAT_ORDERINGS 4u
#define HK_DEBUG_OPT_TRACE_UPDATE 5u
#define HK_DEBUG_OPT_MAIN_PRIORITY 9u
#define HK_DEBUG_OPT_PREPASS_PIPELINE 10u
#define HK_DEBUG_OPT_LOAD_DEVICE_LIMIT 12u
#define HK_DEBUG_OPT_MESH_REBUILD_ONE_WORKGROUP 11u
int hk_debug_set_option(hk_ctx* ctx, uint32_t option, int64_t value);
int hk_debug_multi_serial(int on);

#if defined(__GNUC__)
#pragma GCC visibility pop
#endif
#ifdef __cplusplus
}
#endif
#endif
```

Measured before the change: 7253.

## Skip lighting and denoise work on 8x8 tiles where all primary rays missed

The prepass now writes a per-8x8-tile flag plane that records when every primary ray in a wave missed geometry. The direct, emissive, indirect and spatial-reuse passes read this flag per wave and skip the G-buffer position fetch. Demodulation and the denoise levels write known constant outputs (zeros or the clear colour) for tiles whose neighbourhood is all empty. The plane is used only under conditions the host checks: full-resolution single band, no host writes, and a certified pixel-to-UV identity. The cost is extra bookkeeping and invalidation logic, with a risk of stale planes if a case is missed.

```diff
diff --git a/bevy-hikari_amd/_ffi.py b/bevy-hikari_amd/_ffi.py
--- a/bevy-hikari_amd/_ffi.py
+++ b/bevy-hikari_amd/_ffi.py
@@ -31,6 +31,7 @@
 DEBUG_OPT_SPATIAL_WINDOW, DEBUG_OPT_FRAME_PIPELINE, DEBUG_OPT_WF_TIMELINE, DEBUG_OPT_FLAT_WALK, DEBUG_OPT_FLAT_ORDERINGS, DEBUG_OPT_TRACE_UPDATE = 0, 1, 2, 3, 4, 5
 DEBUG_OPT_MAIN_PRIORITY, DEBUG_OPT_PREPASS_PIPELINE, DEBUG_OPT_MESH_REBUILD_ONE_WORKGROUP = 9, 10, 11
 DEBUG_OPT_LOAD_DEVICE_LIMIT = 12
+DEBUG_OPT_KNOWN_RESULTS = 13
 TIMING_TRACE_STAGES = 18
 TRAVERSAL_WIDE = 0x100
 FRAME_EXTERNAL_GBUFFER, FRAME_ANTIALIAS, FRAME_BALANCE_BANDS, FRAME_GATHER, FRAME_TIME_BAND = 1, 2, 4, 8, 16
@@ -216,6 +217,7 @@
     "debug_comm_lanes": [_vp, P(u32)],
     "debug_multi_serial": [C.c_int],
     "debug_spatial_windowed_launches": [_vp, P(C.c_uint64)],
+    "debug_empty_tiles": [_vp, P(C.c_uint8), C.c_size_t, P(C.c_uint64)],
     "debug_main_stream_priority": [_vp, P(u32)],
     "measure_hbm": [_vp, C.c_size_t, u32, P(C.c_double), P(C.c_double)],
     "measure_valu": [_vp, u32, P(C.c_double)],
diff --git a/bevy-hikari_amd/csrc/context.hip b/bevy-hikari_amd/csrc/context.hip
--- a/bevy-hikari_amd/csrc/context.hip
+++ b/bevy-hikari_amd/csrc/context.hip
@@ -23,6 +23,27 @@
   for (int k = -64; k < size + 64; ++k) {
     const float x = (float)k + 0.5f, want = x / b, q = x * c, got = fmaf(fmaf(-q, b, x), c, q);
     if (memcmp(&want, &got, 4) != 0) return false;
+  }
+  return true;
+}
+
+bool certify_pixel_identity(int size, bool fast) {
+  const float b = (float)size, c = 1.0f / b;
+  for (int k = 0; k < size; ++k) {
+    const float x = (float)k + 0.5f, q = x * c;
+    const float uv = fast ? fmaf(fmaf(-q, b, x), c, q) : x / b;
+    for (int s = 0; s < 4; ++s) {
+      const float sgn = (s & 1) ? 0.25f : 0.5f, amount = (s & 2) ? -sgn : sgn;
+      const float duv = uv + amount * c * 0.0f;
+      if ((int)(duv * b) != k) return false;
+      if (std::min(std::max((int)floorf(duv * b), 0), size - 1) != k) return false;
+    }
+    for (int o = -1; o <= 1; ++o) {
+      const float su = uv + (float)o * c;
+      if (su < 0.0f || su > 1.0f) continue;
+      const int sx = std::min(std::max((int)floorf(su * b), 0), size - 1);
+      if (sx < k - 1 || sx > k + 1) return false;
+    }
   }
   return true;
 }
@@ -92,6 +113,12 @@
     c->tile_meta[k] = nullptr;
     c->tile_meta_zero[k] = false;
   }
+  for (int k = 0; k < 2; ++k) {
+    if (c->empty_tiles[k]) (void)hipFree(c->empty_tiles[k]);
+    c->empty_tiles[k] = nullptr;
+    c->empty_ok[k] = c->lights_ok[k] = false;
+  }
+  c->pixel_identity = false;
   if (c->wf_mem) (void)hipFree(c->wf_mem);
   c->wf_mem = nullptr;
   if (c->wf.timeline) (void)hipFree(c->wf.timeline);
@@ -211,8 +238,26 @@
   g.depth = c->depth_plane;
   g.dn_g = (float4*)c->dn_g;
   g.albedo_out = nullptr;
+  g.empty_out = nullptr;
+  g.empty_in = nullptr;
+  g.tiles_x = c->tiles_x;
   return g;
 }
+const uint8_t* known_empty_plane(hk_ctx* c, int y0, int y1, bool demodulation = false) {
+  const uint32_t p = c->mapped_parity & 1u;
+  if (!c->known_results || !c->in_frame_stage || !c->empty_tiles[p] || !c->pixel_identity || c->W != c->RW || c->H != c->RH || c->frame.upscale_ratio != 1.0f) return nullptr;
+  if (c->band_count != 1 || (y0 % 8) != 0 || !((y1 % 8) == 0 || y1 == c->RH)) return nullptr;
+  if (!c->empty_ok[p] || c->empty_frame[p] != c->frame.number || c->derived_dirty || c->host_wrote) return nullptr;
+  if (demodulation) {
+    if (!c->lights_ok[p] || c->lights_frame[p] != c->frame.number) return nullptr;
+    for (int col = 0; col < 3; ++col)
+      for (int row = 0; row < 3; ++row)
+        if (!std::isfinite(c->frame.kernel[col][row])) return nullptr;
+  }
+  c->empty_plane_launches += 1;
+  return c->empty_tiles[p];
+}
+void forget_empty_tiles(hk_ctx* c) { c->empty_ok[0] = c->empty_ok[1] = c->lights_ok[0] = c->lights_ok[1] = false; }
 bool parks_across_bands(const hk_ctx* c) { return c->band_count > 1 && c->history_now > 0; }
 bool scatter_lite(const hk_ctx* c, int channel) {
   if (c->band_count > 1 || (c->flags & HK_CTX_RACING_SCATTER)) return false;
@@ -381,6 +426,8 @@
     d.output[ch] = (uint2*)dn_internal(c, nch, ch, 0);
     d.internal_variance[ch] = dn_variance(c, nch, ch);
   }
+  d.empty_tiles = known_empty_plane(c, y0, y1, true);
+  d.tiles_x = c->tiles_x;
   launch_demodulation(c->stream, (int)nch, fr, d, y0, y1);
   HK_HIP(hipGetLastError());
   return HK_OK;
@@ -403,6 +450,8 @@
     d.tone_mapped = (uint2*)c->buf[HK_BUF_TONE_MAPPED];
     memcpy(d.clear_color, c->frame.clear_color, sizeof(d.clear_color));
   }
+  d.empty_tiles = known_empty_plane(c, y0, y1);
+  d.tiles_x = c->tiles_x;
   launch_denoise(c->stream, level, (int)nch, 0, fr, d, y0, y1);
   HK_HIP(hipGetLastError());
   return HK_OK;
@@ -620,12 +669,15 @@
 
 int run_pass(hk_ctx* c, uint32_t pass, uint32_t arg, int y0, int y1) {
   const DFrame fr = make_dframe(c);
-  const GBuffer g = make_gbuffer(c);
+  GBuffer g = make_gbuffer(c);
   unsigned long long* counters = (c->flags & HK_CTX_COUNT_RAYS) ? c->d_counters : nullptr;
   if (c->derived_dirty && pass != HK_PASS_PREPASS) {
     launch_derive_planes(c->stream, g, c->depth_plane, c->dn_g, c->W, 0, c->H);
     c->derived_dirty = false;
   }
+  const bool fused_light = pass == HK_PASS_DIRECT_LIT || pass == HK_PASS_DIRECT_EMISSIVE || (pass == HK_PASS_INDIRECT && !use_wavefront(c)) ||
+                           pass == HK_PASS_EMISSIVE_SPATIAL_REUSE || pass == HK_PASS_INDIRECT_SPATIAL_REUSE;
+  if (fused_light) g.empty_in = known_empty_plane(c, y0, y1);
   ScopedTimer timer(c, pass, pass == HK_PASS_INDIRECT || pass == HK_PASS_INDIRECT_SPATIAL_REUSE || pass == HK_PASS_EMISSIVE_SPATIAL_REUSE);
   switch (pass) {
     case HK_PASS_PREPASS: {
@@ -926,6 +978,7 @@
     case HK_DEBUG_OPT_MESH_REBUILD_ONE_WORKGROUP: c->mesh_rebuild_one_workgroup = value != 0; break;
     case HK_DEBUG_OPT_LOAD_DEVICE_LIMIT: c->load_device_limit = value <= 0 ? HK_MESH_REBUILD_MAX_TRIANGLES : (uint32_t)std::min<int64_t>(value, HK_MESH_REBUILD_MAX_TRIANGLES); break;
     case HK_DEBUG_OPT_PREPASS_PIPELINE: c->prepass_pipeline = value < 0 ? -1 : (value ? 1 : 0); break;
+    case HK_DEBUG_OPT_KNOWN_RESULTS: c->known_results = value != 0; forget_empty_tiles(c); break;
     case HK_DEBUG_OPT_MAIN_PRIORITY: c->main_priority = value < 0 ? -1 : (value ? 1 : 0); return pick_main_stream(c, true);
     default: HK_REQUIRE(false, HK_E_INVALID, "unknown option %u", option);
   }
@@ -935,6 +988,16 @@
 int hk_debug_main_stream_priority(hk_ctx* c, uint32_t* out) {
   HK_REQUIRE(c && out, HK_E_INVALID, "bad argument");
   *out = (c->own_stream_high ? 1u : 0u) | (c->main_priority_decided ? 2u : 0u) | (c->pre_stream ? 4u : 0u) | ((uint32_t)std::min<uint64_t>(c->prepasses_pipelined, 0xFFFFFu) << 8);
+  return HK_OK;
+}
+
+int hk_debug_empty_tiles(hk_ctx* c, uint8_t* out_bytes, size_t n, uint64_t* launches_given_the_plane) {
+  HK_REQUIRE(c && out_bytes && launches_given_the_plane, HK_E_INVALID, "bad argument");
+  HK_REQUIRE(c->empty_tiles[0] && n == (size_t)c->tiles_x * c->tiles_y, HK_E_INVALID, "the plane has %d x %d tiles", c->tiles_x, c->tiles_y);
+  HK_HIP(hipSetDevice(c->device));
+  { const int rc = sync_all(c); if (rc) return rc; }
+  HK_HIP(hipMemcpy(out_bytes, c->empty_tiles[c->mapped_parity & 1u], n, hipMemcpyDeviceToHost));
+  *launches_given_the_plane = c->empty_plane_launches;
   return HK_OK;
 }
 
@@ -992,6 +1055,10 @@
       HK_HIP(hipMalloc((void**)&c->tile_meta[k], mb));
       HK_HIP(hipMemset(c->tile_meta[k], 0, mb));
       c->tile_meta_zero[k] = true;
+    }
+    for (int k = 0; k < 2; ++k) {
+      HK_HIP(hipMalloc((void**)&c->empty_tiles[k], (size_t)c->tiles_x * c->tiles_y));
+      HK_HIP(hipMemset(c->empty_tiles[k], 0, (size_t)c->tiles_x * c->tiles_y));
     }
   }
   HK_HIP(hipMalloc((void**)&c->depth_plane, nf * 4));
@@ -1028,6 +1095,8 @@
   }
   c->derived_dirty = false;
   c->uv_fast = !(c->flags & HK_CTX_PLAIN_DIVISION) && certify_uv_division(c->W) && certify_uv_division(c->H) && certify_uv_division(c->RW) && certify_uv_division(c->RH);
+  c->pixel_identity = c->W == c->RW && c->H == c->RH && certify_pixel_identity(c->RW, c->uv_fast) && certify_pixel_identity(c->RH, c->uv_fast);
+  c->host_wrote = false;
   HK_HIP(hipDeviceSynchronize());
   return HK_OK;
 }
@@ -1109,6 +1178,7 @@
   if (pass == HK_PASS_FSR_EASU || pass == HK_PASS_FSR_RCAS) rows = c->H;
   const int y0 = (int)row_begin, y1 = row_end == 0 ? rows : (int)row_end;
   HK_REQUIRE(y0 >= 0 && y1 <= rows && y0 <= y1, HK_E_INVALID, "row range [%d,%d) outside 0..%d", y0, y1, rows);
+  forget_empty_tiles(c);
   return run_pass(c, pass, arg, y0, y1);
 }
 
@@ -1251,6 +1321,8 @@
   auto clampr = [&](int v) { return std::min(std::max(v, 0), c->RH); };
   const Aprons ap = band_aprons(st);
   const int den = (int)ap.denoise, sp = (int)ap.spatial;
+  struct InStage { hk_ctx* c; ~InStage() { c->in_frame_stage = false; } } in_stage_{c};
+  c->in_frame_stage = true;
 #define HK_RUN(pass, arg, y0, y1)                    \
   do {                                               \
     int a_ = (y0), b_ = (y1);                        \
@@ -1282,11 +1354,20 @@
     }
     bool albedo_done = false;
     if (c->timing_mask) (void)hipEventRecord(c->frame_start, c->stream);
+    c->empty_ok[parity] = c->lights_ok[parity] = false;
+    const bool write_plane = c->known_results && c->empty_tiles[parity] && c->pixel_identity && c->frame.upscale_ratio == 1.0f && c->band_count == 1 &&
+                             !(flags & HK_FRAME_EXTERNAL_GBUFFER) && !c->derived_dirty && !c->host_wrote && f0 == 0 && f1 == c->H;
+    c->host_wrote = false;
     if (!(flags & HK_FRAME_EXTERNAL_GBUFFER)) {
       if (f1 > f0) {
         const DFrame fr = make_dframe(c);
         GBuffer g = make_gbuffer(c);
         g.albedo_out = (uint2*)c->buf[HK_BUF_ALBEDO];
+        if (write_plane) {
+          g.empty_out = c->empty_tiles[parity];
+          c->empty_ok[parity] = true;
+          c->empty_frame[parity] = c->frame.number;
+        }
         unsigned long long* counters = (c->flags & HK_CTX_COUNT_RAYS) ? c->d_counters : nullptr;
         const Jitter j = prepass_jitter(c);
         hkd::WideTrees wide{};
@@ -1327,6 +1408,10 @@
       HK_RUN(HK_PASS_DIRECT_LIT, 0, b0, b1);
       HK_RUN(HK_PASS_DIRECT_EMISSIVE, 0, b0, b1);
       HK_RUN(HK_PASS_INDIRECT, 0, b0, b1);
+    }
+    if (c->band_count == 1 && b0 == 0 && b1 == c->RH) {
+      c->lights_ok[parity] = true;
+      c->lights_frame[parity] = c->frame.number;
     }
     c->pre_chain_ok = !(flags & (HK_FRAME_EXTERNAL_GBUFFER | HK_FRAME_ANTIALIAS));
     c->pre_last_parity = parity;
@@ -1606,11 +1691,18 @@
     c->tile_meta_zero[k] = true;
   }
   if (buffer == HK_BUF_POSITION || buffer == HK_BUF_NORMAL || buffer == HK_BUF_INSTANCE_MATERIAL) c->derived_dirty = true;
+  forget_empty_tiles(c);
+  c->host_wrote = true;
   return HK_OK;
 }
 int hk_device_ptr(hk_ctx* c, uint32_t buffer, void** ptr, size_t* bytes) {
   HK_REQUIRE(c && ptr && buffer < HK_BUF_COUNT && c->buf[buffer], HK_E_INVALID, "bad argument");
   *ptr = c->buf[buffer];
+  if (buffer == HK_BUF_POSITION || buffer == HK_BUF_NORMAL || buffer == HK_BUF_DEPTH_GRADIENT || buffer == HK_BUF_INSTANCE_MATERIAL || buffer == HK_BUF_VELOCITY_UV ||
+      buffer == HK_BUF_ALBEDO || (buffer >= HK_BUF_VARIANCE0 && buffer < HK_BUF_VARIANCE0 + 3) || (buffer >= HK_BUF_RENDER0 && buffer < HK_BUF_RENDER0 + 3)) {
+    forget_empty_tiles(c);
+    c->host_wrote = true;
+  }
   if (bytes) *bytes = c->buf_bytes[buffer];
   return HK_OK;
 }
diff --git a/bevy-hikari_amd/csrc/hk_context.hpp b/bevy-hikari_amd/csrc/hk_context.hpp
--- a/bevy-hikari_amd/csrc/hk_context.hpp
+++ b/bevy-hikari_amd/csrc/hk_context.hpp
@@ -174,6 +174,14 @@
   bool tile_meta_zero[10] = {};
   int tiles_x = 0, tiles_y = 0;
   uint32_t elide_serial = 0;
+  uint8_t* empty_tiles[2] = {nullptr, nullptr};
+  bool empty_ok[2] = {false, false}, lights_ok[2] = {false, false};
+  uint32_t empty_frame[2] = {0, 0}, lights_frame[2] = {0, 0};
+  bool pixel_identity = false;
+  bool host_wrote = false;
+  bool in_frame_stage = false;
+  bool known_results = true;
+  uint64_t empty_plane_launches = 0;
   DynOffsets dyn_off{};
   float4 *rf_inst_lo = nullptr, *rf_inst_hi = nullptr, *rf_prev_models = nullptr;
   uint32_t* rf_emissive_of_instance = nullptr;
diff --git a/bevy-hikari_amd/csrc/hk_kernels.hpp b/bevy-hikari_amd/csrc/hk_kernels.hpp
--- a/bevy-hikari_amd/csrc/hk_kernels.hpp
+++ b/bevy-hikari_amd/csrc/hk_kernels.hpp
@@ -15,6 +15,9 @@
   float* __restrict__ depth;
   float4* __restrict__ dn_g;
   uint2* __restrict__ albedo_out;
+  uint8_t* empty_out;
+  const uint8_t* empty_in;
+  int tiles_x;
 };
 struct TileMeta {
   unsigned long long id, src;
@@ -100,6 +103,8 @@
   const uint2* render[3];
   uint2* output[3];
   float* internal_variance[3];
+  const uint8_t* empty_tiles;
+  int tiles_x;
 };
 struct DenoiseTargets {
   const uint2* __restrict__ albedo;
@@ -111,6 +116,8 @@
   const float* internal_variance[3];
   uint2* tone_mapped;
   float clear_color[4];
+  const uint8_t* empty_tiles;
+  int tiles_x;
 };
 
 __device__ __forceinline__ float4 denoise_geometry(uint32_t packed_normal, float instance) {
@@ -137,6 +144,19 @@
 __device__ __forceinline__ int wave_tile(const Pixel& px, int tiles_x) {
   const int lane = threadIdx.x & 63;
   return ((px.y - (lane >> 3)) >> 3) * tiles_x + ((px.x - (lane & 7)) >> 3);
+}
+__device__ __forceinline__ bool wave_tile_known_empty(const uint8_t* __restrict__ plane, const Pixel& px, int tiles_x) {
+  if (!plane) return false;
+  const int tile = __builtin_amdgcn_readfirstlane(wave_tile(px, tiles_x));
+  return __builtin_amdgcn_readfirstlane((int)plane[tile]) != 0;
+}
+__device__ __forceinline__ bool pixel_known_empty(const uint8_t* __restrict__ plane, int tiles_x, int x, int y, int reach, int width, int height) {
+  const int yu = __builtin_amdgcn_readfirstlane(y);
+  const uint8_t* __restrict__ row0 = plane + (max(yu - reach, 0) >> 3) * tiles_x;
+  const uint8_t* __restrict__ row1 = plane + (min(yu + reach, height - 1) >> 3) * tiles_x;
+  if (reach == 0) return row0[(uint32_t)x >> 3] != 0;
+  const uint32_t x0 = (uint32_t)max(x - reach, 0) >> 3, x1 = (uint32_t)min(x + reach, width - 1) >> 3;
+  return (row0[x0] & row0[x1] & row1[x0] & row1[x1]) != 0;
 }
 __device__ __forceinline__ bool tile_holds(const TileMeta* m, int tile, unsigned long long id) {
   const TileMeta v = m[tile];
diff --git a/bevy-hikari_amd/csrc/kernels.hip b/bevy-hikari_amd/csrc/kernels.hip
--- a/bevy-hikari_amd/csrc/kernels.hip
+++ b/bevy-hikari_amd/csrc/kernels.hip
@@ -80,6 +80,10 @@
     rc.tlas = 0;
     primary = 1;
     rc.hits += hit.instance_index != HK_U32_MAX ? 1u : 0u;
+    if (g.empty_out) {
+      const bool all_missed = __ballot(hit.instance_index != HK_U32_MAX) == 0ull;
+      if (wave_leader()) g.empty_out[wave_tile(px, g.tiles_x)] = all_missed ? (uint8_t)1 : (uint8_t)0;
+    }
     prepass_store(sc, fr, pp, g, px.x, px.y, ray, hit);
   }
   flush_counters<COUNT>(rc, primary, counters);
@@ -120,13 +124,16 @@
   if (px.valid) {
     const int x = px.x, y = px.y;
     const int index = x + fr.rw * y;
-    const f2 uv = coords_to_uv(fr, x, y);
     Sample s = zero_sample();
-    int dcx, dcy;
-    jittered_deferred_coords(fr, uv, &dcx, &dcy);
-    const bool din = in_bounds(dcx, dcy, fr.dw, fr.dh);
+    f2 uv = F2(0.0f, 0.0f);
+    int dcx = 0, dcy = 0;
+    float4 position_depth = make_float4(0, 0, 0, 0);
+    if (!wave_tile_known_empty(g.empty_in, px, g.tiles_x)) {
+      uv = coords_to_uv(fr, x, y);
+      jittered_deferred_coords(fr, uv, &dcx, &dcy);
+      if (in_bounds(dcx, dcy, fr.dw, fr.dh)) position_depth = g.position[dcx + fr.dw * dcy];
+    }
     const int didx = dcx + fr.dw * dcy;
-    const float4 position_depth = din ? g.position[didx] : make_float4(0, 0, 0, 0);
     const f3 position = xyz(position_depth);
     const float depth = position_depth.w;
 
@@ -401,11 +408,13 @@
     const int x = px.x, y = px.y;
     const int index = x + fr.rw * y;
     const f2 uv = coords_to_uv(fr, x, y);
-    int dcx, dcy;
-    jittered_deferred_coords(fr, uv, &dcx, &dcy);
-    const bool din = in_bounds(dcx, dcy, fr.dw, fr.dh);
+    int dcx = 0, dcy = 0;
+    float4 position_depth = make_float4(0, 0, 0, 0);
+    if (LDS != 2 || !wave_tile_known_empty(g.empty_in, px, g.tiles_x)) {
+      jittered_deferred_coords(fr, uv, &dcx, &dcy);
+      if (in_bounds(dcx, dcy, fr.dw, fr.dh)) position_depth = g.position[dcx + fr.dw * dcy];
+    }
     const int didx = dcx + fr.dw * dcy;
-    const float4 position_depth = din ? g.position[didx] : make_float4(0, 0, 0, 0);
     const f3 position = xyz(position_depth);
     const float depth = position_depth.w;
 
@@ -633,12 +642,15 @@
   constexpr uint32_t SPATIAL_REUSE_COUNT = EMISSIVE_LIT ? 8u : 16u;
   const int x = px.x, y = px.y;
   const int index = x + fr.rw * y;
-  const f2 uv = coords_to_uv(fr, x, y);
-  int dcx, dcy;
-  jittered_deferred_coords(fr, uv, &dcx, &dcy);
-  const bool din = in_bounds(dcx, dcy, fr.dw, fr.dh) && px.valid;
+  f2 uv = F2(0.0f, 0.0f);
+  int dcx = 0, dcy = 0;
+  float4 position_depth = make_float4(0, 0, 0, 0);
+  if (WINDOWED || !wave_tile_known_empty(g.empty_in, px, g.tiles_x)) {
+    uv = coords_to_uv(fr, x, y);
+    jittered_deferred_coords(fr, uv, &dcx, &dcy);
+    if (in_bounds(dcx, dcy, fr.dw, fr.dh) && px.valid) position_depth = g.position[dcx + fr.dw * dcy];
+  }
   const int didx = dcx + fr.dw * dcy;
-  const float4 position_depth = din ? g.position[didx] : make_float4(0, 0, 0, 0);
   const f3 position = xyz(position_depth);
   const float depth = position_depth.w;
   __shared__ float depth_tile[WINDOWED ? HK_SPATIAL_TILE_W * HK_SPATIAL_TILE_W : 1];
diff --git a/bevy-hikari_amd/csrc/kernels_denoise.hip b/bevy-hikari_amd/csrc/kernels_denoise.hip
--- a/bevy-hikari_amd/csrc/kernels_denoise.hip
+++ b/bevy-hikari_amd/csrc/kernels_denoise.hip
@@ -6,6 +6,7 @@
 #ifndef HK_DENOISE_W
 #define HK_DENOISE_W 64
 #endif
+static_assert(HK_DENOISE_W == 64, "pixel_known_empty (hk_kernels.hpp) takes a wave for one row of pixels");
 
 namespace hkd {
 
@@ -35,6 +36,15 @@
   const Pixel px = pixel_of_thread_rows<64, true>(fr.rw, row_begin, row_end);
   if (!px.valid) return;
   const int x = px.x, y = px.y, index = x + fr.rw * y;
+  if (d.empty_tiles && __ballot(!pixel_known_empty(d.empty_tiles, d.tiles_x, x, y, 1, fr.rw, fr.rh)) == 0ull) {
+    const uint32_t at8 = (uint32_t)index * 8u, at4 = (uint32_t)index * 4u;
+#pragma unroll
+    for (int ch = 0; ch < NCH; ++ch) {
+      *reinterpret_cast<uint2*>(reinterpret_cast<char*>(d.output[ch]) + at8) = make_uint2(0u, 0x3C000000u);
+      *reinterpret_cast<float*>(reinterpret_cast<char*>(d.internal_variance[ch]) + at4) = 0.0f;
+    }
+    return;
+  }
   const f2 uv = coords_to_uv(fr, x, y);
   const f2 deferred_uv = jittered_deferred_uv(fr, uv, 0.5f);
   int ax, ay, rx, ry;
@@ -98,6 +108,12 @@
   if (!px.valid) return;
   constexpr int STEP = 8 >> LEVEL;
   const int x = px.x, y = px.y, index = x + fr.rw * y;
+  if (d.empty_tiles && __ballot(!pixel_known_empty(d.empty_tiles, d.tiles_x, x, y, 0, fr.rw, fr.rh)) == 0ull) {
+#pragma unroll
+    for (int ch = 0; ch < NCH; ++ch) d.output[ch][index] = make_uint2(0u, 0u);
+    if (LEVEL == 3 && d.tone_mapped) d.tone_mapped[index] = pack_f16x4(F4(d.clear_color[0], d.clear_color[1], d.clear_color[2], d.clear_color[3]));
+    return;
+  }
   int col_texel[3], row_texel[3];
   bool col_inside[3], row_inside[3];
 #pragma unroll
diff --git a/bevy-hikari_amd/plugin.py b/bevy-hikari_amd/plugin.py
--- a/bevy-hikari_amd/plugin.py
+++ b/bevy-hikari_amd/plugin.py
@@ -846,6 +846,13 @@
         self.api.call("debug_main_stream_priority", self.ctx, C.byref(v))
         return int(v.value >> 8)
 
+    def empty_tiles(self):
+        w, h, _ = self.buffer_info(F.BUF_TONE_MAPPED)
+        tiles = np.zeros(((h + 7) // 8, (w + 7) // 8), dtype=np.uint8)
+        n = C.c_uint64()
+        self.api.call("debug_empty_tiles", self.ctx, tiles.ctypes.data_as(C.POINTER(C.c_uint8)), tiles.size, C.byref(n))
+        return tiles, int(n.value)
+
     def spatial_windowed_launches(self):
         n = C.c_uint64()
         self.api.call("debug_spatial_windowed_launches", self.ctx, C.byref(n))
diff --git a/include/hikari_hip_debug.h b/include/hikari_hip_debug.h
--- a/include/hikari_hip_debug.h
+++ b/include/hikari_hip_debug.h
@@ -47,7 +47,9 @@
 #define HK_DEBUG_OPT_PREPASS_PIPELINE 10u
 #define HK_DEBUG_OPT_LOAD_DEVICE_LIMIT 12u
 #define HK_DEBUG_OPT_MESH_REBUILD_ONE_WORKGROUP 11u
+#define HK_DEBUG_OPT_KNOWN_RESULTS 13u
 int hk_debug_set_option(hk_ctx* ctx, uint32_t option, int64_t value);
+int hk_debug_empty_tiles(hk_ctx* ctx, uint8_t* out_bytes, size_t n, uint64_t* launches_given_the_plane);
 int hk_debug_multi_serial(int on);
 
 #if defined(__GNUC__)
```

Measured after the change: 7408 (median of 6 runs). +2.1%, better.
